# YichengDWu/tinyedm

Measured on AMD Instinct MI355X. Metric: train imgs/sec CIFAR-10 32x32 bf16, higher is better.
Workload: dtype bf16; 1 GPU; CIFAR-10 32x32 unconditional EDM2 U-Net (conf/cifar10.yaml, 35.6M params) full training step: diffuse+embed+denoiser fwd/bwd+loss+grad all-reduce+Adam+EMA; per_gpu_batch=128, global_batch=128, parallelism=dp1, conditional=False, step_launch=hipGraph replay, collective=none

## Files before the change

### include/tinyedm_hip.h

```cpp
#ifndef TINYEDM_HIP_H
#define TINYEDM_HIP_H
#ifdef __cplusplus
extern "C" {
#endif

typedef struct ihipStream_t* edm_stream_t;

int edm_version(void);
const char* edm_last_error(void);
int edm_init(int device);
int edm_graph_replay_safe(void);
typedef struct {
  unsigned step, seed_lo, seed_hi, reserved;
  float lr, ema_beta, grad_scale, bc1, bc2sqrt, pad[3];
} edm_step_params;

int edm_conv_igemm(const void* X, const void* Wp, void* Y, const void* R, float alpha, float beta, int B, int H,
                   int W, int Cin, int Cout, int taps, edm_stream_t stream);
int edm_conv_igemm_v2(const void* X, const void* Wp, void* Y, const void* R, float alpha, float beta, int B, int H,
                      int W, int Cin, int Cout, int taps, edm_stream_t stream);
int edm_conv_igemm_v6(const void* X, const void* Wp, void* Y, const void* R, float alpha, float beta, int B, int H,
                      int W, int Cin, int Cout, int taps, edm_stream_t stream);
int edm_conv_igemm_s(const void* X, const void* Wp, void* Y, const void* R, float alpha, float beta, int B, int H,
                     int W, int Cin, int Cout, int taps, edm_stream_t stream);
int edm_conv_plan(int B, int H, int W, int Cin, int Cout, int taps, int force);
int edm_conv_igemm_o(const void* X, const void* Wp, void* Y, long ldY, void* Ysilu, void* Yb, long ldYb, int split,
                     const void* R, float alpha, float beta, int B, int H, int W, int Cin, int Cout, int taps, int kernel,
                     int wfrag, edm_stream_t stream);
int edm_conv3x3_fold_supported(int B, int H, int W, int Cin, int Cout, int C2);
int edm_conv3x3_fold(const void* X, const void* Wp, const void* X2, long ldX2, const void* W2p, int C2, void* Y, long ldY,
                     void* Ysilu, float alpha3, float alpha1, int B, int H, int W, int Cin, int Cout, edm_stream_t stream);
int edm_conv3x3_mod(const void* X, const void* Wp, void* Y, void* Y2, const float* lin, long lin_stride,
                    const float* gain, float pdrop, unsigned long long seed, unsigned sub, unsigned step, int mark_dropped,
                    int B, int H, int W, int Cin, int Cout, const void* dyn, int wfrag, edm_stream_t stream);
int edm_conv3x3_modbwd(const void* dY, const void* Wd, float alpha, const void* U, const float* lin, long lin_stride,
                       const float* gain, void* GR, float* gm, long gm_stride, float pdrop, unsigned long long seed,
                       unsigned sub, unsigned step, int u_marked, int B, int H, int W, int Cin, int Cout, const void* dyn,
                       int wfrag, edm_stream_t stream);
int edm_conv3x3_silubwd(const void* dY, const void* Wd, const void* Xpre, const void* ADD, float add_scale, void* GX,
                        int B, int H, int W, int Cin, int Cout, int wfrag, edm_stream_t stream);
int edm_mod_finish(const float* gm, const float* lin, long lin_stride, const float* gain, float* glin, long glin_stride,
                   float* ggain, int B, int C, edm_stream_t stream);
int edm_mod_finish_multi(const float* gm_all, const float* lin_all, float* glin_all, long stride, const void* items_dev,
                         int n_items, int B, edm_stream_t stream);
int edm_conv_wgrad_nsplit(int B, int H, int W, int Cin, int Cout, int taps);
int edm_conv_wgrad_v2(const void* X, const void* dY, float* slabs, int B, int H, int W, int Cin, int Cout, int taps,
                      int nsplit, edm_stream_t stream);
int edm_conv_wgrad_1x1_nsplit(long npix, int Cin, int Cout);
int edm_conv_wgrad_1x1(const void* X, const void* dY, float* slabs, long npix, int Cin, int Cout, int nsplit,
                       edm_stream_t stream);
typedef struct {
  const void* X;
  const void* dY;
  float* slabs;
  long npix;
  int Cin, Cout, nsplit, pad;
} edm_wgrad1_item;
int edm_conv_wgrad_1x1_nsplit_grouped(long npix, int Cin, int Cout);
long edm_conv_wgrad_1x1_group_table_bytes(void);
int edm_conv_wgrad_1x1_group(const edm_wgrad1_item* items, int n, void* table_host, void* table_dev, int defer_upload,
                             edm_stream_t stream);
typedef struct {
  const void* X;
  const void* dY;
  const float* w;
  float* grad;
  const int* perm;
  int B, H, W, Cin, Cout, I;
  float scale;
  int accumulate;
} edm_wgrad3_item;
long edm_wgrad3_workspace(const edm_wgrad3_item* items, int n);
long edm_wgrad3_table_bytes(void);
int edm_wgrad3_max_layers(void);
int edm_wgrad3_group(const edm_wgrad3_item* items, int n, void* workspace, long workspace_bytes, void* table_host,
                     void* table_dev, int defer_upload, edm_stream_t stream);

int edm_weight_prep(float* w, int O, int I, int taps, int Ipad, void* wp_fwd, void* wp_dgrad, float* w_hat,
                    const int* perm, int normalize_inplace, edm_stream_t stream);
int edm_weight_prep_multi(const void* descs, const int* groups, int n_groups, int lds_bytes, int normalize_inplace,
                          edm_stream_t stream);
int edm_wgrad_finish(const float* slabs, int S, const float* w, float* grad, const int* perm, int O, int I, int Ipad,
                     int taps, float scale, int accumulate, edm_stream_t stream);

typedef struct {
  const float* slabs;
  const float* w;
  float* grad;
  const int* perm;
  int S, O, I, Ipad, taps;
  float scale;
  int accumulate;
} edm_finish_item;
long edm_wgrad_finish_multi_table_bytes(void);
int edm_wgrad_finish_multi(const edm_finish_item* items, int n, void* table_host, void* table_dev, int defer_upload,
                           edm_stream_t stream);

int edm_attention_fwd(const void* qkv, void* y, int B, int N, int C, int heads, edm_stream_t stream);
int edm_attention_bwd(const void* qkv, const void* y, const void* gy, void* gqkv, int B, int N, int C, int heads,
                      edm_stream_t stream);

int edm_attention_qkv_supported(int N, int C, int heads);
int edm_attention_qkv_fwd(const void* x, const void* Wqkv, void* y, void* stat, int B, int N, int C, int heads,
                          int heads_per_wg, edm_stream_t stream);
int edm_attention_qkv_bwd(const void* x, const void* y, const void* gout, const void* stat, const void* Wqkv,
                          const void* Wd_out, void* gqkv, float alpha, int B, int N, int C, int heads, int heads_per_wg,
                          edm_stream_t stream);

int edm_pixelnorm_silu_fwd(const void* x, void* xn, void* a, float* dsave, long P, int C, edm_stream_t stream);
int edm_pixelnorm_silu_bwd(const void* xn, const float* dsave, const void* gxn, float gxn_scale, const void* ga,
                           const void* gadd, void* gx, long P, int C, edm_stream_t stream);
int edm_pool_pixelnorm_silu_fwd(const void* x, void* xn, void* a, float* dsave, int B, int Hp, int Wp, int C,
                                edm_stream_t stream);
int edm_pool_pixelnorm_silu_bwd(const void* xn, const float* dsave, const void* gxn, float gxn_scale, const void* ga,
                                const void* gadd, void* gx, int B, int Hp, int Wp, int C, edm_stream_t stream);
int edm_silu_fwd(const void* x, void* a, long n, edm_stream_t stream);
int edm_silu_bwd(const void* x, const void* ga, const void* gextra, float extra_scale, void* gx, long n,
                 edm_stream_t stream);
int edm_axpby(const void* a, float alpha, const void* b, float beta, void* out, long n, edm_stream_t stream);
int edm_mod_silu_drop_fwd(const void* r, const float* lin, long lin_stride, const float* gain, void* a, int B, int HW,
                          int C, float pdrop, unsigned long long seed, unsigned sub, unsigned step, const void* dyn,
                          edm_stream_t stream);
int edm_mod_silu_drop_bwd(const void* r, const float* lin, long lin_stride, const float* gain, const void* ga, void* gr,
                          float* gm, float* glin, long glin_stride, float* ggain, int B, int HW, int C, float pdrop,
                          unsigned long long seed, unsigned sub, unsigned step, const void* dyn, edm_stream_t stream);
int edm_mod_silu_drop_bwd_raw(const void* r, const float* lin, long lin_stride, const float* gain, const void* ga, void* gr,
                              float* gm, long gm_stride, int B, int HW, int C, float pdrop, unsigned long long seed,
                              unsigned sub, unsigned step, const void* dyn, edm_stream_t stream);
int edm_dropout_mask(unsigned char* mask, long n, float pdrop, unsigned long long seed, unsigned sub, unsigned step,
                     edm_stream_t stream);
int edm_pool2(const void* x, void* y, int B, int Hout, int Wout, int C, float scale, edm_stream_t stream);
int edm_up2(const void* x, const void* add, void* y, int B, int Hout, int Wout, int C, float scale, edm_stream_t stream);
int edm_up2_silu(const void* x, void* y, void* a, int B, int Hout, int Wout, int C, edm_stream_t stream);
int edm_reduce_hw(const void* x, long x_stride, const void* y, long y_stride, float* out, int B, int HW, int C,
                  float scale, edm_stream_t stream);
int edm_scalelong_fwd(const float* mean, const float* W1h, const float* W2h, float* gate, float* z1save, int B, int C,
                      int R, edm_stream_t stream);
int edm_scalelong_bwd(const float* mean, const float* W1h, const float* W2h, const float* gate, const float* z1save,
                      const float* ggate, float* gmean, float* gW1h, float* gW2h, int B, int C, int R,
                      edm_stream_t stream);
int edm_skip_gate_fwd(const void* skip, const float* W1h, const float* W2h, float* mean, float* gate, float* z1save,
                      int B, int HW, int C, int R, edm_stream_t stream);
int edm_skip_gate_bwd(const void* gcat, long gcat_stride, int c_off, const void* skip, const float* mean,
                      const float* W1h, const float* W2h, const float* gate, const float* z1save, float* gmean,
                      float* gW1h, float* gW2h, float* ws, int B, int HW, int C, int R, edm_stream_t stream);
typedef struct {
  const float* ws;
  const float* mean;
  float* gW1h;
  float* gW2h;
  int B, C, R, pad;
} edm_skip_gate_wgrad_item;
long edm_skip_gate_wgrad_multi_table_bytes(void);
int edm_skip_gate_wgrad_multi(const edm_skip_gate_wgrad_item* items, int n, void* table_host, void* table_dev,
                              int defer_upload, edm_stream_t stream);
typedef struct {
  const void* skip;
  const float* W1h;
  const float* W2h;
  float* mean;
  float* gate;
  float* z1save;
  void* cat;
  void* silu_out;
  int B, HW, C, R, Ci, pad;
} edm_skip_gate_fwd_item;
long edm_skip_gate_fwd_multi_table_bytes(void);
int edm_skip_gate_fwd_multi(const edm_skip_gate_fwd_item* items, int n, void* table_host, void* table_dev, int defer_upload,
                            edm_stream_t stream);
typedef struct {
  const void* gcat;
  long gcat_stride;
  const void* skip;
  const float* W1h;
  const float* W2h;
  const float* gate;
  const float* z1save;
  float* gmean;
  float* ws;
  void* gskip;
  int c_off, B, HW, C, R, pad;
} edm_skip_gate_bwd_item;
typedef struct {
  const void* gcs;
  const float* gate;
  const float* gmean;
  void* gskip;
  int B, HW, Cs, pad;
} edm_skip_half_bwd_item;
long edm_skip_gate_bwd_multi_table_bytes(void);
int edm_skip_gate_bwd_multi(const edm_skip_gate_bwd_item* items, int n, void* table_host, void* table_dev, int defer_upload,
                            edm_stream_t stream);
int edm_skip_half_bwd_multi(const edm_skip_half_bwd_item* items, int n, void* table_host, void* table_dev, int defer_upload,
                            edm_stream_t stream);
int edm_concat_gate_fwd(const void* inp, const void* skip, const float* gate, void* cat, void* silu_out, int B, int HW,
                        int Ci, int Cs, edm_stream_t stream);
int edm_concat_gate_bwd(const void* gcat, const float* gate, const float* gmean, void* ginp, void* gskip, int B,
                        int HW, int Ci, int Cs, edm_stream_t stream);
int edm_skip_half_fwd(const void* skip, const float* gate, void* cat, void* silu_out, int B, int HW, int Ci, int Cs,
                      edm_stream_t stream);
int edm_skip_half_bwd(const void* gcs, const float* gate, const float* gmean, void* gskip, int B, int HW, int Cs,
                      edm_stream_t stream);

int edm_precond_in(const float* noisy, const float* sigma, int sigma_stride, float sigma_data, void* out, int B,
                   int Cimg, int HW, int CP, edm_stream_t stream);
int edm_conv_out_fwd(const void* x, const float* w_hat, const float* gain_out, const float* noisy, const float* sigma,
                     int sigma_stride, float sigma_data, float* D, float* Fraw, int B, int HW, int C, int Co,
                     edm_stream_t stream);
int edm_conv_out_bwd(const void* x, const float* w_hat, const float* gain_out, const float* Fraw, const float* dD,
                     const float* sigma, int sigma_stride, float sigma_data, void* gx, float* gw_hat, float* ggain,
                     int B, int HW, int C, int Co, edm_stream_t stream);

int edm_lowrank_df(const float* dD, const float* Fraw, const float* gain_out, const float* sigma, int sigma_stride,
                   float sigma_data, float* dF, float* aux, int B, int Co, int HW, edm_stream_t stream);
int edm_lowrank_dgrad3x3(const float* dF, const float* Wc, float scale, void* ga2, const void* r1, const float* lin,
                         long lin_stride, const float* gain, void* gr, float* gm, long gm_stride, float pdrop,
                         unsigned long long seed, unsigned sub, unsigned step, int u_marked, int B, int H, int W, int C,
                         int Co, const void* dyn, edm_stream_t stream);
long edm_lowrank_wgrad_workspace(int C, int Co, int taps);
int edm_lowrank_supported(int C, int Co, int W, int taps);
int edm_lowrank_wgrad(const float* dF, const void* X, int taps, const float* aux, float* G, float* aux_out, float* ws,
                      long ws_floats, int B, int H, int W, int C, int Co, edm_stream_t stream);
int edm_lowrank_expand_wc(const float* wout_hat, const void* wd, float* Wc, int Co, int O, int I, int taps,
                          edm_stream_t stream);
int edm_lowrank_expand_slab(const float* wout_hat, const float* G, float* slab, float scale, int Co, int O, int I,
                            int Ipad, int taps, edm_stream_t stream);

int edm_nchw_to_nhwc_bf16(const float* x, void* y, int B, int C, int HW, edm_stream_t stream);
int edm_nhwc_bf16_to_nchw(const void* x, float* y, int B, int C, int HW, edm_stream_t stream);

int edm_linear_fwd(const float* X, const float* W, float* Y, int M, int N, int K, edm_stream_t stream);
int edm_linear_plan(int M, int N, int K, int accumulate, int* tile_rows, int* splits);
int edm_linear_dgrad(const float* dY, const float* W, float* dX, int M, int N, int K, int accumulate,
                     edm_stream_t stream);
int edm_linear_wgrad(const float* dY, const float* X, float* dW, int M, int N, int K, int accumulate,
                     edm_stream_t stream);
int edm_fourier_fwd(const float* sigma, int sigma_stride, const float* freqs, const float* phases, float* out, int B,
                    int Fd, edm_stream_t stream);
int edm_embed_combine_fwd(const float* emb_sigma, const float* wcls_hat, const long long* labels, float add_factor,
                          int K, float* pre, float* out, int B, int E, unsigned long long drop_thr,
                          unsigned long long seed, unsigned step, const void* dyn, const int* drop_in, int* drop_out,
                          edm_stream_t stream);
int edm_embed_combine_bwd(const float* gout, const float* pre, const long long* labels, float add_factor, int K,
                          float* gemb_sigma, float* gwcls_hat, int B, int E, const int* drop, edm_stream_t stream);
int edm_aug_embed_fwd(float* emb_sigma, const float* aug, const float* w_hat, int B, int E, int K, edm_stream_t stream);
int edm_aug_embed_wgrad(const float* gemb_sigma, const float* aug, float* gw_hat, int B, int E, int K,
                        edm_stream_t stream);

int edm_diffuse(const float* clean, float* noisy, float* sigma, float P_mean, float P_std, int B, long CHW,
                unsigned long long seed, unsigned step, const void* dyn, edm_stream_t stream);
int edm_diffuse_given(const float* clean, const float* eps, const float* noise, float* noisy, float* sigma,
                      float P_mean, float P_std, int B, long CHW, edm_stream_t stream);
int edm_weighted_mse(const float* D, const float* clean, const float* sigma, const float* weight_override,
                     float sigma_data, float* loss, float* dD, int B, long CHW, float* acc_sum, long long* acc_total,
                     edm_stream_t stream);
int edm_adam_ema(float* theta, float* grad, float* m, float* v, float* ema, long n, float lr, float b1, float b2,
                 float eps, int step, float ema_beta, float grad_scale, const void* dyn, int zero_grad,
                 unsigned* health, edm_stream_t stream);
int edm_adam_ema_phema(float* theta, float* grad, float* m, float* v, float* ema, float* const* profiles, int K,
                       const float* betas, long n, float lr, float b1, float b2, float eps, int step, float ema_beta,
                       float grad_scale, const void* dyn, int zero_grad, unsigned* health, edm_stream_t stream);
int edm_phema_accumulate(double* acc, const float* snap, const double* w, int L, long n, edm_stream_t stream);
int edm_phema_finish(const double* acc, float* out, long n, edm_stream_t stream);
int edm_heun_euler(const float* x, const float* D, float t0, float t1, float* dx, float* x1, long n, unsigned* health,
                   edm_stream_t stream);
int edm_heun_correct(const float* x, const float* dx, const float* x1, const float* D1, float t0, float t1, float* out,
                     long n, unsigned* health, edm_stream_t stream);
int edm_heun_euler_guided(const float* x, const float* Dm, const float* Dg, const float* w, float t0, float t1,
                          float* dx, float* x1, long n, unsigned* health, edm_stream_t stream);
int edm_heun_correct_guided(const float* x, const float* dx, const float* x1, const float* Dm1, const float* Dg1,
                            const float* w, float t0, float t1, float* out, long n, unsigned* health,
                            edm_stream_t stream);
int edm_heun_churn(const float* x, float c, const void* rec, int step, int B, long CHW, float* x_hat,
                   unsigned* health, edm_stream_t stream);
int edm_dpm_multistep(const float* x, const float* Dm, const float* Dg, const float* w, const float* m1,
                      const float* m2, float a, float c0, float c1, float c2, float* x_out, float* m_out, long n,
                      unsigned* health, edm_stream_t stream);
int edm_state_init(const float* image, const float* x0, float t, float* out, long n, unsigned* health,
                   edm_stream_t stream);
int edm_inpaint_blend(const float* x, const float* image, const unsigned char* mask, float t, const void* rec, int step,
                      int B, int C, long HW, int mask_B, float* out, unsigned* health, edm_stream_t stream);
int edm_degrade(const float* x, float* y, int B, int C, int H, int W, int scale, int gray, edm_stream_t stream);
int edm_project_denoised(const float* Dm, const float* Dg, const float* w, const float* y, float* out, int B, int C,
                         int H, int W, int scale, int gray, unsigned* health, edm_stream_t stream);
#define EDM_NLL_MAX_CHUNKS 64
int edm_nll_probe(const float* x, float h, const void* rec, int step, int ev, int K, int B, long CHW, float* E,
                  unsigned* health, edm_stream_t stream);
int edm_heun_euler_div(const float* E, const float* D, float t0, float t1, float h0, float h1, const void* rec, int step,
                       int K, int B, long CHW, float* dx, float* E1, double* part, double* L, unsigned* health,
                       edm_stream_t stream);
int edm_heun_correct_div(const float* E, const float* dx, const float* E1, const float* D1, float t0, float t1, float h1,
                         float hn, const void* rec, int step, int K, int probes_out, int B, long CHW, float* out,
                         double* part, double* L, unsigned* health, edm_stream_t stream);
int edm_nll_prior(const float* x, float t, int B, long CHW, double* part, double* L, unsigned* health,
                  edm_stream_t stream);
int edm_eval_diffuse(const float* clean, const unsigned* ids, const int* level, const float* sigmas, int L,
                     const void* rec, int B, long CHW, float* noisy, float* sigma_out, unsigned* health,
                     edm_stream_t stream);
int edm_eval_sqerr(const float* D, const float* clean, int B, long CHW, double* part, double* se, unsigned* health,
                   edm_stream_t stream);
int edm_scale_f32(const float* x, float s, float* y, long n, edm_stream_t stream);

int edm_f32_conv(const float* X, const float* w_hat, float* Y, const float* R, float alpha, float beta, const float* lin,
                 long lin_stride, const float* gain, int B, int H, int W, int Cin, int I, int Cout, int taps,
                 edm_stream_t stream);
int edm_f32_to_pairs(const float* x, void* pairs, long rows, int C, edm_stream_t stream);
int edm_split_pack(const float* w_hat, void* pack, int O, int I, int taps, int Ip, edm_stream_t stream);
int edm_split_conv(const void* Xp, const void* Wp3, float* Y, void* Ypairs, const float* R, float alpha, float beta,
                   const float* lin, long lin_stride, const float* gain, int B, int H, int W, int C, int Cout, int taps,
                   edm_stream_t stream);
int edm_split_conv_o(const void* Xp, const void* Wp3, float* Y, void* Ypairs, long ld_pairs, long lo_off, void* Ysilu_pairs,
                     const float* R, float alpha, float beta, const float* lin, long lin_stride, const float* gain, int B,
                     int H, int W, int C, int Cout, int taps, edm_stream_t stream);
int edm_split_conv_fold(const void* Xp, const void* Wp3, const void* X2p, const void* W2p3, int C2, float* Y, void* Ypairs,
                        long ld_pairs, long lo_off, void* Ysilu_pairs, float alpha3, float alpha1, int B, int H, int W, int C,
                        int Cout, edm_stream_t stream);
int edm_f32_skip_half(const float* skip, const float* gate, void* cat_pairs, void* silu_pairs, int B, int HW, int Ci, int Cs,
                      edm_stream_t stream);
int edm_f32_attention(const float* qkv, float* y, int B, int N, int C, int heads, edm_stream_t stream);
int edm_split_attention(const float* qkv, float* y, void* ypairs, int B, int N, int C, int heads, edm_stream_t stream);
int edm_f32_pixelnorm_silu(const float* x, float* xn, float* s, long P, int C, int s_pairs, edm_stream_t stream);
int edm_f32_silu(const float* x, float* s, long n, int pairs_row, edm_stream_t stream);
int edm_f32_pool2(const float* x, float* y, int B, int Hout, int Wout, int C, edm_stream_t stream);
int edm_f32_up2(const float* x, float* y, int B, int Hout, int Wout, int C, edm_stream_t stream);
int edm_f32_pool_pixelnorm_silu(const float* x, float* xn, float* s, int B, int Hout, int Wout, int C, int s_pairs,
                                edm_stream_t stream);
int edm_f32_up2_silu(const float* x, float* y, float* s, int B, int Hout, int Wout, int C, int s_pairs, edm_stream_t stream);
int edm_f32_skip_gate(const float* skip, const float* W1h, const float* W2h, float* gate, int B, int HW, int C, int R,
                      edm_stream_t stream);
int edm_f32_concat_gate(const float* inp, const float* skip, const float* gate, float* cat, float* silu_out, int B,
                        int HW, int Ci, int Cs, int pairs, edm_stream_t stream);
int edm_f32_precond_in(const float* noisy, const float* sigma, int sigma_stride, float sigma_data, float* out, int B,
                       int Cimg, int HW, int CP, edm_stream_t stream);
int edm_f32_conv_out(const float* x, const float* w_hat, const float* gain_out, const float* noisy, const float* sigma,
                     int sigma_stride, float sigma_data, float* D, int B, int HW, int C, int Co, edm_stream_t stream);
int edm_f32_nchw_to_nhwc(const float* x, float* y, int B, int C, int HW, edm_stream_t stream);
int edm_f32_nhwc_to_nchw(const float* x, float* y, int B, int C, int HW, edm_stream_t stream);

int edm_u8_gather_normalize(const void* data, const long* index, float* out, int B, int C, int H, int W, long n_images,
                            float mean, float stdv, int flip, unsigned long long seed, unsigned epoch,
                            edm_stream_t stream);
int edm_u8_gather_augment_normalize(const void* data, const long* index, float* out, int B, int C, int H, int W,
                                    long n_images, float mean, float stdv, int flip, unsigned long long seed,
                                    unsigned epoch, unsigned long long aug_thr, int aug_ops, float* aug,
                                    edm_stream_t stream);
int edm_u8_gather_augment_warp_normalize(const void* data, const long* index, float* out, int B, int C, int H, int W,
                                         long n_images, float mean, float stdv, int flip, unsigned long long seed,
                                         unsigned epoch, unsigned long long aug_thr, int aug_ops, int warp_ops,
                                         float* aug, float* theta, edm_stream_t stream);
int edm_denormalize_u8(const float* x, void* out, long n, float scale, float offset, edm_stream_t stream);
int edm_prediction_to_u8_nhwc(const float* pred, void* out, int B, int C, int H, int W, const float* mean,
                              const float* stdv, edm_stream_t stream);

int edm_u8_knn_splits(long Q, long R);
int edm_u8_norms(const void* x, long n_rows, int D, int* norms, edm_stream_t stream);
int edm_u8_knn_partial(const void* queries, const void* refs, long Q, long R, int D, int k, int exclude_self, long ref_base,
                       int partial, int splits, const int* qnorms, const int* rnorms, unsigned long long* keys,
                       edm_stream_t stream);
int edm_knn_merge(const unsigned long long* keys, int n_lists, long Q, int k, unsigned* dist, int* idx,
                  edm_stream_t stream);

#ifdef __cplusplus
}
#endif
#endif
```

### tinyedm_amd/_lib.py

```python
import ctypes
import os

_HERE = os.path.dirname(os.path.abspath(__file__))
LIB_PATH = os.environ.get("EDM_LIB_PATH") or os.path.join(_HERE, "libtinyedm_hip.so")

P, I, L, F = ctypes.c_void_p, ctypes.c_int, ctypes.c_long, ctypes.c_float
U, U64 = ctypes.c_uint, ctypes.c_ulonglong

SIGNATURES = {
    "edm_version": [],
    "edm_last_error": [],
    "edm_init": [I],
    "edm_graph_replay_safe": [],
    "edm_pixelnorm_silu_fwd": [P, P, P, P, L, I, P],
    "edm_pixelnorm_silu_bwd": [P, P, P, F, P, P, P, L, I, P],
    "edm_pool_pixelnorm_silu_fwd": [P, P, P, P, I, I, I, I, P],
    "edm_pool_pixelnorm_silu_bwd": [P, P, P, F, P, P, P, I, I, I, I, P],
    "edm_up2_silu": [P, P, P, I, I, I, I, P],
    "edm_silu_fwd": [P, P, L, P],
    "edm_silu_bwd": [P, P, P, F, P, L, P],
    "edm_axpby": [P, F, P, F, P, L, P],
    "edm_mod_silu_drop_fwd": [P, P, L, P, P, I, I, I, F, U64, U, U, P, P],
    "edm_mod_silu_drop_bwd": [P, P, L, P, P, P, P, P, L, P, I, I, I, F, U64, U, U, P, P],
    "edm_mod_silu_drop_bwd_raw": [P, P, L, P, P, P, P, L, I, I, I, F, U64, U, U, P, P],
    "edm_dropout_mask": [P, L, F, U64, U, U, P],
    "edm_pool2": [P, P, I, I, I, I, F, P],
    "edm_up2": [P, P, P, I, I, I, I, F, P],
    "edm_reduce_hw": [P, L, P, L, P, I, I, I, F, P],
    "edm_scalelong_fwd": [P, P, P, P, P, I, I, I, P],
    "edm_scalelong_bwd": [P, P, P, P, P, P, P, P, P, I, I, I, P],
    "edm_skip_gate_fwd": [P, P, P, P, P, P, I, I, I, I, P],
    "edm_skip_gate_bwd": [P, L, I, P, P, P, P, P, P, P, P, P, P, I, I, I, I, P],
    "edm_skip_gate_wgrad_multi": [P, I, P, P, I, P],
    "edm_skip_gate_wgrad_multi_table_bytes": [],
    "edm_skip_gate_fwd_multi": [P, I, P, P, I, P],
    "edm_skip_gate_fwd_multi_table_bytes": [],
    "edm_skip_gate_bwd_multi": [P, I, P, P, I, P],
    "edm_skip_half_bwd_multi": [P, I, P, P, I, P],
    "edm_skip_gate_bwd_multi_table_bytes": [],
    "edm_concat_gate_fwd": [P, P, P, P, P, I, I, I, I, P],
    "edm_concat_gate_bwd": [P, P, P, P, P, I, I, I, I, P],
    "edm_skip_half_fwd": [P, P, P, P, I, I, I, I, P],
    "edm_skip_half_bwd": [P, P, P, P, I, I, I, P],
    "edm_precond_in": [P, P, I, F, P, I, I, I, I, P],
    "edm_conv_out_fwd": [P, P, P, P, P, I, F, P, P, I, I, I, I, P],
    "edm_conv_out_bwd": [P, P, P, P, P, P, I, F, P, P, P, I, I, I, I, P],
    "edm_nchw_to_nhwc_bf16": [P, P, I, I, I, P],
    "edm_nhwc_bf16_to_nchw": [P, P, I, I, I, P],
    "edm_lowrank_df": [P, P, P, P, I, F, P, P, I, I, I, P],
    "edm_lowrank_dgrad3x3": [P, P, F, P, P, P, L, P, P, P, L, F, U64, U, U, I, I, I, I, I, I, P, P],
    "edm_lowrank_wgrad_workspace": [I, I, I],
    "edm_lowrank_supported": [I, I, I, I],
    "edm_lowrank_wgrad": [P, P, I, P, P, P, P, L, I, I, I, I, I, P],
    "edm_lowrank_expand_wc": [P, P, P, I, I, I, I, P],
    "edm_lowrank_expand_slab": [P, P, P, F, I, I, I, I, I, P],
    "edm_conv_igemm": [P, P, P, P, F, F, I, I, I, I, I, I, P],
    "edm_conv_igemm_v2": [P, P, P, P, F, F, I, I, I, I, I, I, P],
    "edm_conv_plan": [I, I, I, I, I, I, I],
    "edm_conv_igemm_o": [P, P, P, L, P, P, L, I, P, F, F, I, I, I, I, I, I, I, I, P],
    "edm_conv3x3_fold_supported": [I, I, I, I, I, I],
    "edm_conv3x3_fold": [P, P, P, L, P, I, P, L, P, F, F, I, I, I, I, I, P],
    "edm_conv_igemm_v6": [P, P, P, P, F, F, I, I, I, I, I, I, P],
    "edm_conv_igemm_s": [P, P, P, P, F, F, I, I, I, I, I, I, P],
    "edm_conv3x3_mod": [P, P, P, P, P, L, P, F, U64, U, U, I, I, I, I, I, I, P, I, P],
    "edm_conv3x3_modbwd": [P, P, F, P, P, L, P, P, P, L, F, U64, U, U, I, I, I, I, I, I, P, I, P],
    "edm_mod_finish_multi": [P, P, P, L, P, I, I, P],
    "edm_conv3x3_silubwd": [P, P, P, P, F, P, I, I, I, I, I, I, P],
    "edm_mod_finish": [P, P, L, P, P, L, P, I, I, P],
    "edm_conv_wgrad_nsplit": [I, I, I, I, I, I],
    "edm_conv_wgrad_v2": [P, P, P, I, I, I, I, I, I, I, P],
    "edm_conv_wgrad_1x1_nsplit": [L, I, I],
    "edm_conv_wgrad_1x1_nsplit_grouped": [L, I, I],
    "edm_conv_wgrad_1x1": [P, P, P, L, I, I, I, P],
    "edm_conv_wgrad_1x1_group": [P, I, P, P, I, P],
    "edm_conv_wgrad_1x1_group_table_bytes": [],
    "edm_wgrad3_workspace": [P, I],
    "edm_wgrad3_group": [P, I, P, L, P, P, I, P],
    "edm_wgrad3_table_bytes": [],
    "edm_wgrad3_max_layers": [],
    "edm_attention_fwd": [P, P, I, I, I, I, P],
    "edm_attention_bwd": [P, P, P, P, I, I, I, I, P],
    "edm_attention_qkv_supported": [I, I, I],
    "edm_attention_qkv_fwd": [P, P, P, P, I, I, I, I, I, P],
    "edm_attention_qkv_bwd": [P, P, P, P, P, P, P, F, I, I, I, I, I, P],
    "edm_linear_plan": [I, I, I, I, P, P],
    "edm_linear_fwd": [P, P, P, I, I, I, P],
    "edm_linear_dgrad": [P, P, P, I, I, I, I, P],
    "edm_linear_wgrad": [P, P, P, I, I, I, I, P],
    "edm_fourier_fwd": [P, I, P, P, P, I, I, P],
    "edm_embed_combine_fwd": [P, P, P, F, I, P, P, I, I, U64, U64, U, P, P, P, P],
    "edm_embed_combine_bwd": [P, P, P, F, I, P, P, I, I, P, P],
    "edm_aug_embed_fwd": [P, P, P, I, I, I, P],
    "edm_aug_embed_wgrad": [P, P, P, I, I, I, P],
    "edm_diffuse": [P, P, P, F, F, I, L, U64, U, P, P],
    "edm_diffuse_given": [P, P, P, P, P, F, F, I, L, P],
    "edm_weighted_mse": [P, P, P, P, F, P, P, I, L, P, P, P],
    "edm_adam_ema": [P, P, P, P, P, L, F, F, F, F, I, F, F, P, I, P, P],
    "edm_adam_ema_phema": [P, P, P, P, P, P, I, P, L, F, F, F, F, I, F, F, P, I, P, P],
    "edm_phema_accumulate": [P, P, P, I, L, P],
    "edm_phema_finish": [P, P, L, P],
    "edm_heun_euler": [P, P, F, F, P, P, L, P, P],
    "edm_heun_correct": [P, P, P, P, F, F, P, L, P, P],
    "edm_heun_euler_guided": [P, P, P, P, F, F, P, P, L, P, P],
    "edm_heun_correct_guided": [P, P, P, P, P, P, F, F, P, L, P, P],
    "edm_heun_churn": [P, F, P, I, I, L, P, P, P],
    "edm_dpm_multistep": [P, P, P, P, P, P, F, F, F, F, P, P, L, P, P],
    "edm_state_init": [P, P, F, P, L, P, P],
    "edm_inpaint_blend": [P, P, P, F, P, I, I, I, L, I, P, P, P],
    "edm_nll_probe": [P, F, P, I, I, I, I, L, P, P, P],
    "edm_heun_euler_div": [P, P, F, F, F, F, P, I, I, I, L, P, P, P, P, P, P],
    "edm_heun_correct_div": [P, P, P, P, F, F, F, F, P, I, I, I, I, L, P, P, P, P, P],
    "edm_nll_prior": [P, F, I, L, P, P, P, P],
    "edm_eval_diffuse": [P, P, P, P, I, P, I, L, P, P, P, P],
    "edm_eval_sqerr": [P, P, I, L, P, P, P, P],
    "edm_scale_f32": [P, F, P, L, P],
    "edm_degrade": [P, P, I, I, I, I, I, I, P],
    "edm_project_denoised": [P, P, P, P, P, I, I, I, I, I, I, P, P],
    "edm_weight_prep": [P, I, I, I, I, P, P, P, P, I, P],
    "edm_weight_prep_multi": [P, P, I, I, I, P],
    "edm_wgrad_finish": [P, I, P, P, P, I, I, I, I, F, I, P],
    "edm_wgrad_finish_multi": [P, I, P, P, I, P],
    "edm_wgrad_finish_multi_table_bytes": [],
    "edm_f32_conv": [P, P, P, P, F, F, P, L, P, I, I, I, I, I, I, I, P],
    "edm_f32_attention": [P, P, I, I, I, I, P],
    "edm_split_attention": [P, P, P, I, I, I, I, P],
    "edm_f32_to_pairs": [P, P, L, I, P],
    "edm_split_pack": [P, P, I, I, I, I, P],
    "edm_split_conv": [P, P, P, P, P, F, F, P, L, P, I, I, I, I, I, I, P],
    "edm_split_conv_o": [P, P, P, P, L, L, P, P, F, F, P, L, P, I, I, I, I, I, I, P],
    "edm_split_conv_fold": [P, P, P, P, I, P, P, L, L, P, F, F, I, I, I, I, I, P],
    "edm_f32_skip_half": [P, P, P, P, I, I, I, I, P],
    "edm_f32_pool_pixelnorm_silu": [P, P, P, I, I, I, I, I, P],
    "edm_f32_up2_silu": [P, P, P, I, I, I, I, I, P],
    "edm_f32_pixelnorm_silu": [P, P, P, L, I, I, P],
    "edm_f32_silu": [P, P, L, I, P],
    "edm_f32_pool2": [P, P, I, I, I, I, P],
    "edm_f32_up2": [P, P, I, I, I, I, P],
    "edm_f32_skip_gate": [P, P, P, P, I, I, I, I, P],
    "edm_f32_concat_gate": [P, P, P, P, P, I, I, I, I, I, P],
    "edm_f32_precond_in": [P, P, I, F, P, I, I, I, I, P],
    "edm_f32_conv_out": [P, P, P, P, P, I, F, P, I, I, I, I, P],
    "edm_f32_nchw_to_nhwc": [P, P, I, I, I, P],
    "edm_f32_nhwc_to_nchw": [P, P, I, I, I, P],
    "edm_u8_gather_normalize": [P, P, P, I, I, I, I, L, F, F, I, U64, U, P],
    "edm_u8_gather_augment_normalize": [P, P, P, I, I, I, I, L, F, F, I, U64, U, U64, I, P, P],
    "edm_u8_gather_augment_warp_normalize": [P, P, P, I, I, I, I, L, F, F, I, U64, U, U64, I, I, P, P, P],
    "edm_denormalize_u8": [P, P, L, F, F, P],
    "edm_prediction_to_u8_nhwc": [P, P, I, I, I, I, P, P, P],
    "edm_u8_knn_splits": [L, L],
    "edm_u8_norms": [P, L, I, P, P],
    "edm_u8_knn_partial": [P, P, L, L, I, I, I, L, I, I, P, P, P, P],
    "edm_knn_merge": [P, I, L, I, P, P, P],
}
DIAG_SIGNATURES = {
    "edm_conv_igemm_v2_stamp": [P, P, P, I, I, I, I, I, P, P],
    "edm_conv_igemm_v2_ablate": [P, P, P, I, I, I, I, I, I, P],
    "edm_wgrad3_probe": [P, P],
    "edm_wgrad3_plan_ksplit": [P, I, P],
    "edm_v6_persistent_launches": [],
}
_RET = {"edm_last_error": ctypes.c_char_p, "edm_lowrank_wgrad_workspace": ctypes.c_long, "edm_v6_persistent_launches": ctypes.c_long, "edm_wgrad3_workspace": ctypes.c_long, "edm_wgrad3_table_bytes": ctypes.c_long,
        "edm_skip_gate_wgrad_multi_table_bytes": ctypes.c_long, "edm_skip_gate_fwd_multi_table_bytes": ctypes.c_long, "edm_skip_gate_bwd_multi_table_bytes": ctypes.c_long,
        "edm_conv_wgrad_1x1_group_table_bytes": ctypes.c_long, "edm_wgrad_finish_multi_table_bytes": ctypes.c_long}
_NO_STATUS = {"edm_lowrank_wgrad_workspace", "edm_lowrank_supported", "edm_skip_gate_bwd_multi_table_bytes", "edm_skip_gate_fwd_multi_table_bytes", "edm_v6_persistent_launches", "edm_conv3x3_fold_supported", "edm_conv_plan", "edm_skip_gate_wgrad_multi_table_bytes", "edm_version", "edm_graph_replay_safe", "edm_last_error", "edm_conv_wgrad_nsplit", "edm_conv_wgrad_1x1_nsplit", "edm_conv_wgrad_1x1_nsplit_grouped", "edm_wgrad3_workspace", "edm_wgrad3_table_bytes", "edm_wgrad3_max_layers",
              "edm_conv_wgrad_1x1_group_table_bytes", "edm_wgrad_finish_multi_table_bytes", "edm_attention_qkv_supported",
              "edm_u8_knn_splits"}

_lib = None


class HipKernelError(RuntimeError):
    pass


class FinishItem(ctypes.Structure):
    _fields_ = [("slabs", P), ("w", P), ("grad", P), ("perm", P), ("S", I), ("O", I), ("I", I), ("Ipad", I), ("taps", I),
                ("scale", F), ("accumulate", I)]


class SkipGateWgradItem(ctypes.Structure):
    _fields_ = [("ws", P), ("mean", P), ("gW1h", P), ("gW2h", P), ("B", I), ("C", I), ("R", I), ("pad", I)]


class SkipGateFwdItem(ctypes.Structure):
    _fields_ = [("skip", P), ("W1h", P), ("W2h", P), ("mean", P), ("gate", P), ("z1save", P), ("cat", P), ("silu_out", P),
                ("B", I), ("HW", I), ("C", I), ("R", I), ("Ci", I), ("pad", I)]


class SkipGateBwdItem(ctypes.Structure):
    _fields_ = [("gcat", P), ("gcat_stride", L), ("skip", P), ("W1h", P), ("W2h", P), ("gate", P), ("z1save", P), ("gmean", P),
                ("ws", P), ("gskip", P), ("c_off", I), ("B", I), ("HW", I), ("C", I), ("R", I), ("pad", I)]


class SkipHalfBwdItem(ctypes.Structure):
    _fields_ = [("gcs", P), ("gate", P), ("gmean", P), ("gskip", P), ("B", I), ("HW", I), ("Cs", I), ("pad", I)]


class WGrad1Item(ctypes.Structure):
    _fields_ = [("X", P), ("dY", P), ("slabs", P), ("npix", L), ("Cin", I), ("Cout", I), ("nsplit", I), ("pad", I)]


class WGrad3Item(ctypes.Structure):
    _fields_ = [("X", P), ("dY", P), ("w", P), ("grad", P), ("perm", P), ("B", I), ("H", I), ("W", I), ("Cin", I),
                ("Cout", I), ("I", I), ("scale", F), ("accumulate", I)]


def lib() -> ctypes.CDLL:
    global _lib
    if _lib is None:
        if not os.path.exists(LIB_PATH):
            raise RuntimeError(
                f"tinyedm_amd: {LIB_PATH} is missing -- build it with `python -m tinyedm_amd.build` "
                "(there is no CPU fallback for the HIP hot path)")
        h = ctypes.CDLL(LIB_PATH)
        for name, args in {**SIGNATURES, **DIAG_SIGNATURES}.items():
            fn = getattr(h, name)
            fn.argtypes = args
            fn.restype = _RET.get(name, ctypes.c_int)
        _lib = h
    return _lib


N_CALLS = 0


def call(name: str, *args):
    global N_CALLS
    N_CALLS += 1
    h = lib()
    rc = getattr(h, name)(*args)
    if name in _NO_STATUS:
        return rc
    if rc != 0:
        msg = h.edm_last_error()
        raise HipKernelError(f"{name} failed (status {rc}): {msg.decode() if msg else '?'}")
    return rc


_inited_devices = set()


def init_device(index: int) -> None:
    if index not in _inited_devices:
        call("edm_init", int(index))
        _inited_devices.add(index)
```

### tinyedm_amd/csrc/tail_lowrank.hip

```cpp
#include "common.h"

typedef __attribute__((ext_vector_type(2))) float f32x2;

constexpr size_t LOWRANK_LDS_MAX = 60 * 1024;
static size_t dgrad_lds(int Co, int C, int W, int R, bool fused) {
  const int CL = C / 8, PS = ((256 / CL) * CL) / CL, TP = (W + 3) / 4 * 4 + 4;
  return ((size_t)Co * 9 * C + (size_t)Co * (R + 2) * TP + (fused ? (size_t)PS * C : 0)) * sizeof(float);
}
static size_t wgrad_lds(int Co, int taps, int C, int W, int R) {
  const int halo = taps == 9 ? 1 : 0;
  return ((size_t)Co * taps * C + (size_t)Co * (R + 2 * halo) * (W + 2 * halo)) * sizeof(float);
}
extern "C" int edm_lowrank_supported(int C, int Co, int W, int taps) {
  if (C <= 0 || C % 8 || C > 1024 || Co < 1 || Co > 8 || W <= 0 || (taps != 1 && taps != 9)) return 0;
  if (wgrad_lds(Co, taps, C, W, 1) > LOWRANK_LDS_MAX) return 0;
  return taps == 1 || dgrad_lds(Co, C, W, 1, true) <= LOWRANK_LDS_MAX;
}

__global__ void k_lowrank_df(const float* __restrict__ dD, const float* __restrict__ Fraw,
                             const float* __restrict__ gain_out, const float* __restrict__ sigma, int sstride, float sd,
                             float* __restrict__ dF, float* __restrict__ aux, int CoHW, long n) {
  const float go = *gain_out;
  for (long i = (long)blockIdx.x * blockDim.x + threadIdx.x; i < n; i += (long)gridDim.x * blockDim.x) {
    const int b = (int)(i / CoHW);
// ... 132 lines not shown
    }
  }
}

template <int CO>
static int launch_dgrad(const float* dF, const float* Wc, float scale, void* ga, const void* U, const float* lin,
                        long lin_stride, const float* gain, void* gr, float* gm, long gm_stride, float pdrop,
                        unsigned long long seed, unsigned sub, unsigned step, int u_marked, int B, int H, int W, int C,
                        const void* dyn, hipStream_t st) {
  const int CL = C / 8, block = (256 / CL) * CL, PS = block / CL;
  const int NSX = (W + 3) / 4, TP = NSX * 4 + 4;
  int R = 128 / W;
  R = R < 1 ? 1 : (R > H ? H : R);
  auto lds = [&](int r) { return dgrad_lds(CO, C, W, r, U != nullptr); };
  while (R > 1 && lds(R) > LOWRANK_LDS_MAX) --R;
  EDM_REQUIRE(lds(R) <= LOWRANK_LDS_MAX, "lowrank_dgrad3x3: Co=%d, C=%d, W=%d need %zu bytes of LDS (60 KB at most)", CO, C, W,
              lds(R));
  const dim3 grid((H + R - 1) / R, B);
  if (U)
    hipLaunchKernelGGL((k_lowrank_dgrad3x3<CO, true>), grid, dim3(block), lds(R), st, dF, Wc, scale, (bf16*)ga,
                       (const bf16*)U, lin, lin_stride, gain, (bf16*)gr, gm, gm_stride, pdrop, (uint32_t)seed,
                       (uint32_t)(seed >> 32), sub, step, u_marked, (const StepParams*)dyn, H, W, C, R, TP);
  else
    hipLaunchKernelGGL((k_lowrank_dgrad3x3<CO, false>), grid, dim3(block), lds(R), st, dF, Wc, scale, (bf16*)ga,
                       (const bf16*)nullptr, (const float*)nullptr, 0L, (const float*)nullptr, (bf16*)nullptr,
                       (float*)nullptr, 0L, 0.f, 0u, 0u, 0u, 0u, 0, (const StepParams*)nullptr, H, W, C, R, TP);
  EDM_CHECK_LAUNCH("lowrank_dgrad3x3");
  return EDM_OK;
}

#define EDM_CO_SWITCH(Co, CALL)      \
  switch (Co) {                      \
    case 1: return CALL(1);          \
    case 2: return CALL(2);          \
    case 3: return CALL(3);          \
    case 4: return CALL(4);          \
    case 5: return CALL(5);          \
    case 6: return CALL(6);          \
    case 7: return CALL(7);          \
    default: return CALL(8);         \
  }

extern "C" int edm_lowrank_dgrad3x3(const float* dF, const float* Wc, float scale, void* ga, const void* r1,
                                    const float* lin, long lin_stride, const float* gain, void* gr, float* gm,
                                    long gm_stride, float pdrop, unsigned long long seed, unsigned sub, unsigned step,
                                    int u_marked, int B, int H, int W, int C, int Co, const void* dyn, hipStream_t st) {
  EDM_REQUIRE(dF && Wc && (ga || r1), "lowrank_dgrad3x3: null pointer");
  EDM_REQUIRE(B > 0 && B <= 65535 && H > 0 && W > 0 && C > 0 && C % 8 == 0 && C <= 2048 && Co >= 1 && Co <= 8,
              "lowrank_dgrad3x3: bad args (C %% 8 == 0, Co <= 8 required)");
  EDM_REQUIRE(((uintptr_t)Wc & 15) == 0, "lowrank_dgrad3x3: Wc must be 16-byte aligned");
  if (r1)
    EDM_REQUIRE(lin && gain && gr && gm && lin_stride >= C && gm_stride >= C && pdrop >= 0.f && pdrop < 1.f,
                "lowrank_dgrad3x3: bad modulation-backward args");
#define CALL(CO_) launch_dgrad<CO_>(dF, Wc, scale, ga, r1, lin, lin_stride, gain, gr, gm, gm_stride, pdrop, seed, sub, step, \
                                    u_marked, B, H, W, C, dyn, st)
  EDM_CO_SWITCH(Co, CALL)
#undef CALL
}

template <int CO, int TAPS, int VEC>
__global__ __launch_bounds__(512) void k_lowrank_wgrad(const float* __restrict__ dF, const bf16* __restrict__ X,
                                                       const float* __restrict__ aux, float* __restrict__ ws, int H,
                                                       int W, int C, int R, int upb, int nunits) {
  constexpr int HALO = TAPS == 9 ? 1 : 0, K = TAPS == 9 ? 3 : 1, NB = 8;
  extern __shared__ __attribute__((aligned(16))) float sm[];
  __shared__ float asums[512];
  const int N = CO * TAPS * C, TPW = W + 2 * HALO, TR = R + 2 * HALO;
  float* accl = sm;
  float* tl = sm + N;
  typedef __attribute__((ext_vector_type(VEC / 2))) unsigned int uraw;
  const int CLV = C / VEC;
  const int PS = blockDim.x / CLV;
  const int cv = threadIdx.x % CLV, ps = threadIdx.x / CLV;
  f32x2 acc[CO * TAPS][VEC / 2];
#pragma unroll
  for (int e = 0; e < CO * TAPS; ++e)
#pragma unroll
    for (int h = 0; h < VEC / 2; ++h) acc[e][h] = f32x2{0.f, 0.f};
  float asum = 0.f;
  for (int u = blockIdx.x; u < nunits; u += gridDim.x) {
    const int b = u / upb, y0 = (u - b * upb) * R;
    const int rows = min(R, H - y0);
    __syncthreads();
    for (int i = threadIdx.x; i < CO * TR * TPW; i += blockDim.x) {
      const int o = i / (TR * TPW), rem = i - o * TR * TPW;
      const int ry = rem / TPW, cx = rem - ry * TPW;
      const int y = y0 + ry - HALO, x = cx - HALO;
      float v = 0.f;
      if (y >= 0 && y < H && x >= 0 && x < W)
        v = dF[(((long)b * CO + o) * H + y) * W + x];
      tl[i] = v;
    }
    if (aux) {
      for (int o = 0; o < CO; ++o) {
        const float* ap = aux + (((long)b * CO + o) * H + y0) * W;
        for (int i = threadIdx.x; i < rows * W; i += blockDim.x) asum += ap[i];
      }
    }
    __syncthreads();
    const int np = rows * W;
    const bf16* xp = X + (((long)b * H + y0) * W) * C + cv * VEC;
    int ry = ps / W, x = ps - (ps / W) * W;
    uraw nx[NB];
    auto fetch = [&](int q0) {
#pragma unroll
      for (int i = 0; i < NB; ++i) {
        const int q = q0 + i * PS;
        nx[i] = uraw{};
        if (q < np) nx[i] = *reinterpret_cast<const uraw*>(xp + (long)q * C);
      }
    };
    fetch(ps);
    for (int q0 = ps; q0 < np; q0 += NB * PS) {
      uraw cur[NB];
#pragma unroll
      for (int i = 0; i < NB; ++i) cur[i] = nx[i];
      if (q0 + NB * PS < np) fetch(q0 + NB * PS);
#pragma unroll
      for (int i = 0; i < NB; ++i) {
        if (q0 + i * PS < np) {
          typedef __attribute__((ext_vector_type(VEC))) __bf16 bfv;
          const bfv xv = __builtin_bit_cast(bfv, cur[i]);
          f32x2 xf[VEC / 2];
#pragma unroll
          for (int h = 0; h < VEC / 2; ++h) xf[h] = f32x2{(float)xv[2 * h], (float)xv[2 * h + 1]};
#pragma unroll
          for (int o = 0; o < CO; ++o)
#pragma unroll
            for (int ky = 0; ky < K; ++ky)
#pragma unroll
              for (int kx = 0; kx < K; ++kx) {
                const float d = tl[(o * TR + ry + 2 * HALO - ky) * TPW + x + 2 * HALO - kx];
                const f32x2 d2 = {d, d};
#pragma unroll
                for (int h = 0; h < VEC / 2; ++h) acc[o * TAPS + ky * K + kx][h] += d2 * xf[h];
              }
        }
        x += PS;
        while (x >= W) {
          x -= W;
          ++ry;
        }
      }
    }
  }
  for (int r = 0; r < PS; ++r) {
    __syncthreads();
    if (ps == r) {
#pragma unroll
      for (int e = 0; e < CO * TAPS; ++e) {
#pragma unroll
        for (int h = 0; h < VEC / 2; ++h) {
          f32x2* ap = reinterpret_cast<f32x2*>(accl + e * C + cv * VEC + 2 * h);
          f32x2 v = acc[e][h];
          if (r) v += *ap;
          *ap = v;
        }
      }
    }
  }
  asums[threadIdx.x] = asum;
  __syncthreads();
  float* row = ws + (long)blockIdx.x * (N + 4);
  for (int i = threadIdx.x; i < N; i += blockDim.x) row[i] = accl[i];
  if (threadIdx.x == 0) {
    float s = 0.f;
    for (int i = 0; i < (int)blockDim.x; ++i) s += asums[i];
    row[N] = s;
  }
}

__global__ __launch_bounds__(1024) void k_lowrank_reduce(const float* __restrict__ ws, int nwg, int N, float* __restrict__ G,
                                                         float* __restrict__ aux_out) {
  __shared__ float part[16][64];
  const int l = threadIdx.x & 63, seg = threadIdx.x >> 6;
  const int e = blockIdx.x * 64 + l;
  const int per = (nwg + 15) / 16;
  const int r0 = seg * per;
  float v[16];
#pragma unroll
  for (int k = 0; k < 16; ++k) {
    const int r = r0 + k;
    v[k] = (e <= N && k < per && r < nwg) ? ws[(long)r * (N + 4) + e] : 0.f;
  }
  float s = 0.f;
#pragma unroll
  for (int k = 0; k < 16; ++k) s += v[k];
  part[seg][l] = s;
  __syncthreads();
  if (seg == 0 && e <= N) {
    float t = 0.f;
#pragma unroll
    for (int k = 0; k < 16; ++k) t += part[k][l];
    if (e < N) G[e] = t;
    else if (aux_out) *aux_out += t;
  }
}

template <int CO>
static int launch_wgrad(const float* dF, const void* X, int taps, const float* aux, float* G, float* aux_out, float* ws,
                        long ws_floats, int B, int H, int W, int C, int nwg, hipStream_t st) {
  constexpr int VEC = CO <= 4 ? 4 : 2;
  const int CLV = C / VEC;
  int PS = 512 / CLV;
  PS = PS > 16 ? 16 : PS;
  const int block = PS * CLV, halo = taps == 9 ? 1 : 0;
  const int N = CO * taps * C;
  int R = 512 / W;
  R = R < 1 ? 1 : (R > H ? H : R);
  auto lds = [&](int r) { return wgrad_lds(CO, taps, C, W, r); };
  while (R > 1 && lds(R) > LOWRANK_LDS_MAX) --R;
  EDM_REQUIRE(lds(R) <= LOWRANK_LDS_MAX, "lowrank_wgrad: Co=%d, taps=%d, C=%d, W=%d need %zu bytes of LDS (60 KB at most)", CO,
              taps, C, W, lds(R));
  const int upb = (H + R - 1) / R;
  EDM_REQUIRE((long)B * upb < (1L << 31), "lowrank_wgrad: too many units");
  const int nunits = B * upb;
  const int grid = nunits < nwg ? nunits : nwg;
  EDM_REQUIRE(ws_floats >= (long)grid * (N + 4), "lowrank_wgrad: workspace of %ld floats, %ld needed", ws_floats,
              (long)grid * (N + 4));
  if (taps == 9)
    hipLaunchKernelGGL((k_lowrank_wgrad<CO, 9, VEC>), dim3(grid), dim3(block), lds(R), st, dF, (const bf16*)X, aux, ws, H, W, C,
                       R, upb, nunits);
  else
    hipLaunchKernelGGL((k_lowrank_wgrad<CO, 1, VEC>), dim3(grid), dim3(block), lds(R), st, dF, (const bf16*)X, aux, ws, H, W, C,
                       R, upb, nunits);
  EDM_CHECK_LAUNCH("lowrank_wgrad");
  hipLaunchKernelGGL(k_lowrank_reduce, dim3((N + 1 + 63) / 64), dim3(1024), 0, st, ws, grid, N, G, aux_out);
  EDM_CHECK_LAUNCH("lowrank_reduce");
  return EDM_OK;
}

constexpr int LOWRANK_WGRAD_NWG = 256;
extern "C" long edm_lowrank_wgrad_workspace(int C, int Co, int taps) {
  return (long)LOWRANK_WGRAD_NWG * ((long)Co * taps * C + 4);
}

extern "C" int edm_lowrank_wgrad(const float* dF, const void* X, int taps, const float* aux, float* G, float* aux_out,
                                 float* ws, long ws_floats, int B, int H, int W, int C, int Co, hipStream_t st) {
  EDM_REQUIRE(dF && X && G && ws && (!aux || aux_out), "lowrank_wgrad: null pointer");
  EDM_REQUIRE(B > 0 && H > 0 && W > 0 && C > 0 && C % 8 == 0 && C <= 1024 && Co >= 1 && Co <= 8 && (taps == 1 || taps == 9),
              "lowrank_wgrad: bad args (C %% 8 == 0, Co <= 8, taps 1 or 9 required)");
#define CALL(CO_) launch_wgrad<CO_>(dF, X, taps, aux, G, aux_out, ws, ws_floats, B, H, W, C, LOWRANK_WGRAD_NWG, st)
  EDM_CO_SWITCH(Co, CALL)
#undef CALL
}

__global__ void k_lowrank_expand_wc(const float* __restrict__ wout, const bf16* __restrict__ wd, float* __restrict__ Wc,
                                    int Co, int O, int I, int taps) {
  const int lane = threadIdx.x & 63;
  const int row = blockIdx.x * (blockDim.x >> 6) + (threadIdx.x >> 6);
  if (row >= taps * I) return;
  const int tt = row / I, ci = row - tt * I;
  float acc[8] = {0, 0, 0, 0, 0, 0, 0, 0};
  for (int c = lane * 8; c < O; c += 64 * 8) {
    float v[8];
    load8(wd + (long)row * O + c, v);
#pragma unroll
    for (int o = 0; o < 8; ++o)
      if (o < Co) {
#pragma unroll
        for (int j = 0; j < 8; ++j) acc[o] += wout[(long)o * O + c + j] * v[j];
      }
  }
#pragma unroll
  for (int o = 0; o < 8; ++o)
    if (o < Co) {
      const float s = wave_sum(acc[o]);
      if (lane == 0) Wc[((long)o * taps + (taps - 1 - tt)) * I + ci] = s;
    }
}
extern "C" int edm_lowrank_expand_wc(const float* wout_hat, const void* wd, float* Wc, int Co, int O, int I, int taps,
                                     hipStream_t st) {
  EDM_REQUIRE(wout_hat && wd && Wc, "lowrank_expand_wc: null pointer");
  EDM_REQUIRE(Co >= 1 && Co <= 8 && O > 0 && O % 8 == 0 && I > 0 && taps >= 1, "lowrank_expand_wc: bad args");
  hipLaunchKernelGGL(k_lowrank_expand_wc, dim3((taps * I + 3) / 4), dim3(256), 0, st, wout_hat, (const bf16*)wd, Wc, Co, O,
                     I, taps);
  EDM_CHECK_LAUNCH("lowrank_expand_wc");
  return EDM_OK;
}

__global__ void k_lowrank_expand_slab(const float* __restrict__ wout, const float* __restrict__ G, float* __restrict__ slab,
                                      float scale, int Co, int O, int I, int Ipad, int taps, long n) {
  for (long e = (long)blockIdx.x * blockDim.x + threadIdx.x; e < n; e += (long)gridDim.x * blockDim.x) {
    const int i = (int)(e % Ipad);
    const long tc = e / Ipad;
    const int c = (int)(tc % O), t = (int)(tc / O);
    float s = 0.f;
    if (i < I)
      for (int o = 0; o < Co; ++o) s += wout[(long)o * O + c] * G[((long)o * taps + t) * I + i];
    slab[e] = scale * s;
  }
}
extern "C" int edm_lowrank_expand_slab(const float* wout_hat, const float* G, float* slab, float scale, int Co, int O, int I,
                                       int Ipad, int taps, hipStream_t st) {
  EDM_REQUIRE(wout_hat && G && slab, "lowrank_expand_slab: null pointer");
  EDM_REQUIRE(Co >= 1 && Co <= 8 && O > 0 && I > 0 && Ipad >= I && taps >= 1, "lowrank_expand_slab: bad args");
  const long n = (long)taps * O * Ipad;
  const long blocks = (n + 255) / 256;
  hipLaunchKernelGGL(k_lowrank_expand_slab, dim3((unsigned)(blocks < 4096 ? blocks : 4096)), dim3(256), 0, st, wout_hat, G,
                     slab, scale, Co, O, I, Ipad, taps, n);
  EDM_CHECK_LAUNCH("lowrank_expand_slab");
  return EDM_OK;
}
```

### tinyedm_amd/networks.py

```python
from __future__ import annotations

import math
import os
from typing import Optional

import numpy as np
import torch
import torch.nn as nn
from torch import Tensor

from . import ops

bf16, f32 = torch.bfloat16, torch.float32


class _Rng:
    seed: int = 42
    step: int = 0
    dyn = None


rng = _Rng()


def manual_seed(seed: int) -> None:
    rng.seed = int(seed) & 0xFFFFFFFFFFFFFFFF
    rng.step = 0


_WEIGHT_EPOCH = 0


_IN_DENOISER = [False]
FORWARD_EPOCH = 0


def bump_weight_epoch() -> None:
    global _WEIGHT_EPOCH
    _WEIGHT_EPOCH += 1


def _mp_coeffs(t: float):
    c = math.sqrt((1 - t) ** 2 + t ** 2)
    return (1 - t) / c, t / c


class _WNBase(nn.Module):

    weight: nn.Parameter

    def _init_cache(self):
        self._cache = None
        self._cache_key = None
        self._perm: Optional[Tensor] = None
        self._ipad: Optional[int] = None
        self._want = ("fwd", "dgrad")
        self._split_pack = None
        self._split_key = None
        self._plain = None

    def _taps(self) -> int:
        return self.weight[0, 0].numel() if self.weight.dim() == 4 else 1

    def packs(self):
        w = self.weight
        if not w.is_cuda:
            raise RuntimeError("tinyedm_amd: parameters must live on the GPU (there is no CPU path)")
        if self.training and getattr(self, "_fresh", False):
            self._fresh = False
            return self._cache
        key = (w.data_ptr(), w._version, _WEIGHT_EPOCH)
        if not self.training and not _IN_DENOISER[0] and self._cache is not None and self._cache_key == key and any(
                getattr(t, "_edm_frag", False) for t in self._cache[:2] if t is not None):
            if self._plain is None or self._plain[0] != key:
                with torch.no_grad():
                    self._plain = (key, ops.weight_prep(w.data, self._taps(), Ipad=self._ipad, want_fwd="fwd" in self._want,
                                                        want_dgrad="dgrad" in self._want, want_hat="hat" in self._want,
                                                        perm=self._perm, normalize_inplace=False))
            return self._plain[1]
        if self.training or self._cache is None or self._cache_key != key:
            perm = self._perm
            if perm is not None and perm.device != w.device:
                perm = self._perm = perm.to(w.device)
            with torch.no_grad():
                self._cache = ops.weight_prep(
                    w.data, self._taps(), Ipad=self._ipad, want_fwd="fwd" in self._want,
                    want_dgrad="dgrad" in self._want, want_hat="hat" in self._want, perm=perm,
                    normalize_inplace=self.training)
            self._cache_key = (w.data_ptr(), w._version, _WEIGHT_EPOCH)
        return self._cache

    def finish_grad(self, slabs: Tensor, scale: float = 1.0) -> Tensor:
        w = self.weight
        I = w.shape[1]
        if w.grad is not None and getattr(w, "_edm_direct", False):
            key = w.device.index
            pend = _fin_pending.setdefault(key, [])
            pend.append((slabs, w, self._perm, self._taps(), I, scale))
            w._edm_deferred = True
            if len(pend) >= FIN_GROUP:
                _flush_fin(key)
            _queue_backward_end(w.device)
            return None
        g = ops.wgrad_finish(slabs, w.data, self._taps(), I, perm=self._perm, scale=scale)
        return g.view_as(w)


WGRAD_STREAM = os.environ.get("EDM_WGRAD_STREAM", "1") != "0"
W3_GROUP = max(0, min(ops.W3_MAX_LAYERS, int(os.environ.get("EDM_W3_GROUP", "16"))))
W3_TAIL = max(0, int(os.environ.get("EDM_W3_TAIL", "0")))
_w3_seen = {}
_w3_total = {}
W3_MAXPIX = int(os.environ.get("EDM_W3_MAXPIX", str(1 << 18)))
FIN_GROUP = 40
W1_GROUP = max(0, min(16, int(os.environ.get("EDM_W1_GROUP", "16"))))
_w1_pending = {}
_bwd_end_queued = set()
MOD_DEFER_UNFUSED = os.environ.get("EDM_MOD_DEFER_UNFUSED", "1") != "0"
SG_MULTI = os.environ.get("EDM_SG_MULTI", "1") != "0"
SG_HALVES = os.environ.get("EDM_SG_HALVES", "1") != "0"
SG_BWD_MULTI = os.environ.get("EDM_SG_BWD_MULTI", "1") != "0"
SG_DEFER = os.environ.get("EDM_SG_DEFER", "1") != "0"
_sg_pending = {}
_w3_pending = {}
TAIL_LOWRANK = os.environ.get("EDM_TAIL_LOWRANK", "1") != "0"
_tail_slot = {}
_fin_pending = {}


def _run_on_side(device, fn, tensors=()):
    if WGRAD_STREAM:
        side = ops.side_stream(device)
        side.wait_stream(torch.cuda.current_stream())
        with torch.cuda.stream(side):
            fn()
        for t in tensors:
            t.record_stream(side)
    else:
        fn()


def _flush_w3(key):
    items = _w3_pending.pop(key, None)
    if not items:
        return
    dev = items[0][0].weight.device
    args = [(x, dy, m.weight.data, m.weight.grad, m._perm, scale, True) for m, x, dy, scale in items]
    keep = [t for _, x, dy, _ in items for t in (x, dy)]
    _run_on_side(dev, lambda: ops.wgrad3_group(args), keep)
    _flush_fin(key)
    for m, _, _, _ in items:
        m.weight._edm_deferred = False
        for hook in getattr(m.weight, "_edm_hooks", ()):
            hook(m.weight)


def _flush_w1(key):
    items = _w1_pending.pop(key, None)
    if not items:
        return
    dev = items[0][0].weight.device
    box = []
    _run_on_side(dev, lambda: box.extend(ops.conv_wgrad_1x1_group([(x, dy) for _, x, dy, _ in items])),
                 [t for _, x, dy, _ in items for t in (x, dy)])
    pend = _fin_pending.setdefault(key, [])
    for (m, _, _, scale), slabs in zip(items, box):
        w = m.weight
        pend.append((slabs, w, m._perm, 1, w.shape[1], scale))


def _flush_fin(key):
    _flush_w1(key)
    items = _fin_pending.pop(key, None)
    if not items:
        return
    dev = items[0][1].device
    args = [(slabs, w.data, w.grad, perm, taps, I, scale, True) for slabs, w, perm, taps, I, scale in items]
    _run_on_side(dev, lambda: ops.wgrad_finish_multi(args), [a[0] for a in args])
    for _, w, *_rest in items:
        w._edm_deferred = False
        for hook in getattr(w, "_edm_hooks", ()):
            hook(w)


def _flush_sg(key):
    items = _sg_pending.pop(key, None)
    if not items:
        return
    outs = ops.skip_gate_wgrad_multi([(ws, mean, R) for _, ws, mean, R in items])
    for (sl, _, _, _), (gw1h, gw2h) in zip(items, outs):
        sl.layer1.finish_grad(gw1h.view(1, 1, *gw1h.shape))
        sl.layer2.finish_grad(gw2h.view(1, 1, *gw2h.shape))


def _backward_end(key):
    _bwd_end_queued.discard(key)
    _tail_slot.pop(key, None)
    if key in _w3_seen:
        _w3_total[key] = _w3_seen.pop(key)
    _flush_sg(key)
    _flush_w3(key)
    _flush_fin(key)
    if WGRAD_STREAM:
        torch.cuda.current_stream(key).wait_stream(ops.side_stream(key))


def _queue_backward_end(device):
    key = torch.device(device).index
    if key in _bwd_end_queued:
        return
    try:
        torch.autograd.Variable._execution_engine.queue_callback(lambda: _backward_end(key))
        _bwd_end_queued.add(key)
    except RuntimeError:
        _backward_end(key)


def reset_backward_state():
    _tail_slot.clear()
    if _bwd_end_queued or _w3_pending or _fin_pending or _w1_pending or _sg_pending:
        _bwd_end_queued.clear()
        for items in _sg_pending.values():
            for sl, *_rest in items:
                sl.layer1.weight._edm_deferred = sl.layer2.weight._edm_deferred = False
        _sg_pending.clear()
        for items in _w1_pending.values():
            for m, _, _, _ in items:
                m.weight._edm_deferred = False
        _w1_pending.clear()
        for items in _fin_pending.values():
            for _, w, *_rest in items:
                w._edm_deferred = False
        _fin_pending.clear()
        for items in _w3_pending.values():
            for m, _, _, _ in items:
                m.weight._edm_deferred = False
        _w3_pending.clear()
        _w3_seen.clear()
        if WGRAD_STREAM:
            for s in ops.side_streams():
                torch.cuda.current_stream(s.device).wait_stream(s)


def _wgrad(mod, x, dy, taps, scale=1.0):
    w = mod.weight
    direct = w.grad is not None and getattr(w, "_edm_direct", False)
    if (taps == 9 and W3_GROUP and w.dim() == 4 and ops.wgrad3_supported(x, dy, w.shape[1])
            and (not WGRAD_STREAM or x.shape[0] * x.shape[1] * x.shape[2] <= W3_MAXPIX)):
        if direct:
            key = w.device.index
            pend = _w3_pending.setdefault(key, [])
            if pend and (pend[0][1].shape[2] + 2 > 64) != (x.shape[2] + 2 > 64):
                _flush_w3(key)
                pend = _w3_pending.setdefault(key, [])
            pend.append((mod, x, dy, scale))
            w._edm_deferred = True
            seen = _w3_seen[key] = _w3_seen.get(key, 0) + 1
            if len(pend) >= W3_GROUP or (W3_TAIL and seen == _w3_total.get(key, 0) - W3_TAIL):
                _flush_w3(key)
            _queue_backward_end(w.device)
            return None
        g = torch.empty_like(w.data)
        ops.wgrad3_group([(x, dy, w.data, g, mod._perm, scale, False)])
        return g
    if direct and taps == 1 and W1_GROUP and w.dim() == 4 and ops.wgrad1x1_group_supported(x, dy):
        key = w.device.index
        pend = _w1_pending.setdefault(key, [])
        pend.append((mod, x, dy, scale))
        w._edm_deferred = True
        if len(pend) >= W1_GROUP:
            _flush_fin(key)
        _queue_backward_end(w.device)
        return None
    if direct:
        _run_on_side(w.device, lambda: mod.finish_grad(ops.conv_wgrad(x, dy, taps), scale=scale), (x, dy))
        _queue_backward_end(w.device)
        return None
    return mod.finish_grad(ops.conv_wgrad(x, dy, taps), scale=scale)


def _wgrad_lowrank(mod, x, dF, wout_hat, scale):
    w = mod.weight
    box = []
    _run_on_side(w.device, lambda: box.append(ops.lowrank_expand_slab(wout_hat, ops.lowrank_wgrad(dF, x, 9)[0], scale)),
                 (x, dF, wout_hat))
    return mod.finish_grad(box[0])


PREP_TILE_BYTES = int(os.environ.get("EDM_PREP_TILE_KB", "96")) * 1024


class _PrepPlan:

    def __init__(self, mods, frag=None, wants=None, cat=None):
        self.mods = mods
        frag = frag or {}
        wants = [tuple(m._want) for m in mods] if wants is None else list(wants)
        self.wants = wants
        self.pins = 0
        self._pinned_forever = False
        self.splits = []
        dev = mods[0].weight.device
        self.ptr_key = tuple(m.weight.data_ptr() for m in mods)
        desc = np.zeros(len(mods), dtype=np.dtype([
            ("w", "<u8"), ("fwd", "<u8"), ("dgrad", "<u8"), ("hat", "<u8"), ("perm", "<u8"),
            ("O", "<i4"), ("I", "<i4"), ("taps", "<i4"), ("Ipad", "<i4"), ("row0", "<i4"), ("pad", "<i4")]))
        assert desc.dtype.itemsize == 64
        groups, row0, lds = [], 0, 0
        self.caches = []
        self.wcat, cat_rows = None, {}
        if cat:
            kin = cat[0].weight.shape[1]
            if all(c.weight.dim() == 2 and c.weight.shape[1] == kin for c in cat):
                self.wcat = torch.empty(sum(c.weight.shape[0] for c in cat), kin, device=dev, dtype=f32)
                r = 0
                for c in cat:
                    cat_rows[c] = r
                    r += c.weight.shape[0]
        for k, m in enumerate(mods):
            w = m.weight
            O, I, taps = w.shape[0], w.shape[1], m._taps()
            ipad = I if m._ipad is None else m._ipad
            want = wants[k]
            wf = torch.empty(taps, O, ipad, device=dev, dtype=bf16) if "fwd" in want else None
            wd = torch.empty(taps, I, O, device=dev, dtype=bf16) if "dgrad" in want else None
            if m in cat_rows:
                wh = self.wcat[cat_rows[m]:cat_rows[m] + O]
            else:
                wh = torch.empty(O, I * taps, device=dev, dtype=f32) if ("hat" in want or "split" in want) else None
            self.splits.append(torch.empty(taps, O, 3 * ((I + 31) // 32 * 32), device=dev, dtype=bf16)
                               if "split" in want else None)
            if m._perm is not None and m._perm.device != dev:
                m._perm = m._perm.to(dev)
            rb = 32
            while rb > 1 and (rb * I * taps * 2 > PREP_TILE_BYTES or rb > O):
                rb //= 2
            lds = max(lds, rb * I * taps * 2)
            ff, fd = frag.get(m, (False, False))
            if not (taps == 9 and I % 32 == 0 and O % 32 == 0 and ipad == I and rb % 8 == 0 and m._perm is None):
                ff = fd = False
            if ff and wf is not None:
                wf._edm_frag = True
            if fd and wd is not None:
                wd._edm_frag = True
            desc[k] = (w.data_ptr(), wf.data_ptr() if wf is not None else 0, wd.data_ptr() if wd is not None else 0,
                       wh.data_ptr() if wh is not None else 0, m._perm.data_ptr() if m._perm is not None else 0,
                       O, I, taps | (0x100 if ff and wf is not None else 0) | (0x200 if fd and wd is not None else 0), ipad,
                       row0, rb)
            groups += [(k, r) for r in range(0, O, rb)]
            row0 += O
            self.caches.append((wf, wd, wh))
        self.total_rows = row0
        self.desc = torch.from_numpy(desc.view(np.uint8).copy()).to(dev)
        self.groups = torch.tensor(groups, dtype=torch.int32).to(dev)
        self.lds_bytes = lds
        self.eval_key = None

    @property
    def pinned(self) -> bool:
        return self.pins > 0 or self._pinned_forever

    def valid_for(self, mods):
        return tuple(m.weight.data_ptr() for m in mods) == self.ptr_key

    def run(self, training: bool):
        key = (tuple(m.weight._version for m in self.mods), _WEIGHT_EPOCH)
        if training or key != self.eval_key:
            ops.weight_prep_multi(self.desc, self.groups, self.lds_bytes, training)
            for m, c, sp in zip(self.mods, self.caches, self.splits):
                if sp is not None:
                    ops.split_pack(c[2], m._taps(), out=sp)
            self.eval_key = None if training else key
        if torch.cuda.is_current_stream_capturing() and not ops.note_capture_pin(self):
            self._pinned_forever = True
        for m, c, sp in zip(self.mods, self.caches, self.splits):
            m._cache = c
            m._cache_key = (m.weight.data_ptr(), m.weight._version, _WEIGHT_EPOCH)
            m._fresh = training
            m._split_pack = sp
            m._split_key = m._cache_key if sp is not None else None


class Conv2d(_WNBase):

    def __init__(self, in_channels, out_channels, kernel_size):
        super().__init__()
        self.in_channels = in_channels
        self.out_channels = out_channels
        self.kernel_size = kernel_size
        self.weight = nn.Parameter(torch.randn(out_channels, in_channels, kernel_size, kernel_size))
        self._init_cache()

    def forward(self, x: Tensor) -> Tensor:
        xh = ops.nchw_to_nhwc_bf16(x.float().contiguous())
        y = _ConvFn.apply(xh, self.weight, self)
        return ops.nhwc_bf16_to_nchw(y).to(x.dtype)

    def extra_repr(self) -> str:
        return f"{self.in_channels}, {self.out_channels}, kernel_size={self.kernel_size}"


class Linear(_WNBase):

    def __init__(self, in_features: int, out_features: int):
        super().__init__()
        self.in_features = in_features
        self.out_features = out_features
        self.weight = nn.Parameter(torch.randn(out_features, in_features))
        self._init_cache()
        self._want = ("hat",)

    def forward(self, x: Tensor) -> Tensor:
        return _LinearFn.apply(x.float().contiguous(), self.weight, self)

    def extra_repr(self) -> str:
        return f"{self.in_features}, {self.out_features}"


class _ConvFn(torch.autograd.Function):
    @staticmethod
    def forward(ctx, x, weight, mod: Conv2d):
        wf, wd, _ = mod.packs()
        ctx.mod, ctx.wd = mod, wd
        ctx.save_for_backward(x)
        return ops.conv_igemm(x, wf, mod._taps())

    @staticmethod
    def backward(ctx, gy):
        (x,) = ctx.saved_tensors
        gy = gy.contiguous()
        taps = ctx.mod._taps()
        gx = ops.conv_igemm(gy, ctx.wd, taps) if ctx.needs_input_grad[0] else None
        gw = _wgrad(ctx.mod, x, gy, taps) if ctx.needs_input_grad[1] else None
        return gx, gw, None


class _LinearFn(torch.autograd.Function):
    @staticmethod
    def forward(ctx, x, weight, mod: Linear):
        _, _, wh = mod.packs()
        ctx.mod, ctx.wh = mod, wh
        ctx.save_for_backward(x)
        return ops.linear_fwd(x, wh)

    @staticmethod
    def backward(ctx, gy):
        (x,) = ctx.saved_tensors
        gy = gy.contiguous()
        gx = ops.linear_dgrad(gy, ctx.wh) if ctx.needs_input_grad[0] else None
        gw = None
        if ctx.needs_input_grad[1]:
            dwh = ops.linear_wgrad(gy, x)
            gw = ctx.mod.finish_grad(dwh.view(1, 1, *dwh.shape))
        return gx, gw, None


def pixel_norm(x: Tensor, eps: float = 1e-4, dim=1) -> Tensor:
    if dim != 1 or x.dim() != 4 or eps != 1e-4:
        raise NotImplementedError("tinyedm_amd.pixel_norm implements the (B,C,H,W), dim=1, eps=1e-4 hot-path case")
    xn, _, _ = ops.pixelnorm_silu_fwd(ops.nchw_to_nhwc_bf16(x.float().contiguous()))
    return ops.nhwc_bf16_to_nchw(xn).to(x.dtype)


def mp_silu(x: Tensor) -> Tensor:
    return torch.nn.functional.silu(x) / 0.596


def mp_add(a: Tensor, b: Tensor, t: float = 0.5) -> Tensor:
    return a.lerp(b, t) / np.sqrt((1 - t) ** 2 + t ** 2)


class UpSample(nn.Module):

    def forward(self, x):
        return ops.nhwc_bf16_to_nchw(ops.up2(ops.nchw_to_nhwc_bf16(x.float().contiguous()))).to(x.dtype)


class DownSample(nn.Module):

    def forward(self, x):
        return ops.nhwc_bf16_to_nchw(ops.pool2(ops.nchw_to_nhwc_bf16(x.float().contiguous()))).to(x.dtype)


class _ResampleFn(torch.autograd.Function):

    @staticmethod
    def forward(ctx, x, up: bool, alias: bool = False, want_silu: bool = False):
        ctx.up = up
        ctx.set_materialize_grads(False)
        if up and want_silu:
            y, s = ops.up2_silu(x)
            ctx.mark_non_differentiable(s)
            return y, s
        y = ops.up2(x) if up else ops.pool2(x, 0.25)
        return (y, x) if alias else y

    @staticmethod
    def backward(ctx, g, g_alias=None):
        if g is None:
            return g_alias, None, None, None
        g = g.contiguous()
        if ctx.up:
            gx = ops.pool2(g, 1.0)
            if g_alias is not None:
                gx = ops.axpby(gx, 1.0, g_alias.contiguous(), 1.0)
            return gx, None, None, None
        return ops.up2(g, 0.25, add=None if g_alias is None else g_alias.contiguous()), None, None, None


class UncertaintyNet(nn.Module):

    def __init__(self, in_features: int, hidden_features: int):
        super().__init__()
        self.linear1 = Linear(in_features + 1, hidden_features)
        self.linear2 = Linear(hidden_features, 1)
        self.gain = nn.Parameter(torch.zeros(()))

    def forward(self, x: Tensor):
        x = torch.cat((x, torch.ones_like(x[:, 0:1])), dim=1)
        x = mp_silu(self.linear1(x))
        return self.gain * self.linear2(x)


class ScaleLong(nn.Module):
    def __init__(self, dim, r=16):
        super().__init__()
        self.layer1 = Conv2d(dim + 1, int(dim // r), 1)
        self.layer2 = Conv2d(int(dim // r), dim, 1)
        self.layer1._want = ("hat",)
        self.layer2._want = ("hat",)
        if SG_DEFER:
            self.layer1.weight._edm_late = True
            self.layer2.weight._edm_late = True

    def forward(self, inp: Tensor) -> Tensor:
        xh = ops.nchw_to_nhwc_bf16(inp.float().contiguous())
        B, H, W, C = xh.shape
        w1h, w2h = self.layer1.packs()[2], self.layer2.packs()[2]
        _, gate, _ = ops.skip_gate_fwd(xh, w1h, w2h)
        return gate.view(B, C, 1, 1)


SKIP_GATE_FUSED = os.environ.get("EDM_SKIP_GATE_FUSED", "1") != "0"
U_MARKS = os.environ.get("EDM_U_MARKS", "1") != "0"


FUSE_CAT = os.environ.get("EDM_FUSE_CAT", "1") != "0"
FUSE_RESAMPLE = os.environ.get("EDM_FUSE_RESAMPLE", "1") != "0"
FRAG_PACKS = os.environ.get("EDM_FRAG_PACKS", "1") != "0"


def _col_block(buf: Tensor, C: int) -> Tensor:
    B, H, W, Ct = buf.shape
    return torch.empty(0, device=buf.device, dtype=buf.dtype).set_(buf.untyped_storage(), buf.storage_offset(),
                                                                   (B, H, W, C), (H * W * Ct, W * Ct, Ct, 1))


def _dest_ok(dest, x: Tensor) -> bool:
    return dest is not None and dest[0].shape[:3] == x.shape[:3]


class _ConcatGateFn(torch.autograd.Function):
    @staticmethod
    def forward(ctx, inp, skip, w1, w2, sl: ScaleLong, want_silu: bool = False):
        ctx.set_materialize_grads(False)
        B, H, W, Cs = skip.shape
        w1h, w2h = sl.layer1.packs()[2], sl.layer2.packs()[2]
        if SKIP_GATE_FUSED:
            mean, gate, z1 = ops.skip_gate_fwd(skip, w1h, w2h)
        else:
            mean = ops.reduce_hw(skip, scale=1.0 / (H * W))
            gate, z1 = ops.scalelong_fwd(mean, w1h, w2h)
        cat, sil = ops.concat_gate_fwd(inp, skip, gate, want_silu)
        ctx.sl, ctx.Ci = sl, inp.shape[-1]
        ctx.save_for_backward(skip, mean, gate, z1, w1h, w2h)
        if want_silu:
            ctx.mark_non_differentiable(sil)
            return cat, sil
        return cat

    @staticmethod
    def backward(ctx, gcat, _gsil=None):
        skip, mean, gate, z1, w1h, w2h = ctx.saved_tensors
        gcat = gcat.contiguous()
        Ci, Cs = ctx.Ci, skip.shape[-1]
        if SKIP_GATE_FUSED:
            gmean, gw1h, gw2h = ops.skip_gate_bwd(gcat, Ci, skip, mean, w1h, w2h, gate, z1)
        else:
            ggate = ops.reduce_hw(gcat, C=Cs, c_off=Ci, y=skip)
            gmean, gw1h, gw2h = ops.scalelong_bwd(mean, w1h, w2h, gate, z1, ggate)
        ginp, gskip = ops.concat_gate_bwd(gcat, gate, gmean, Ci)
        gw1 = ctx.sl.layer1.finish_grad(gw1h.view(1, 1, *gw1h.shape))
        gw2 = ctx.sl.layer2.finish_grad(gw2h.view(1, 1, *gw2h.shape))
        return ginp, gskip, gw1, gw2, None, None


class ClassEmbedding(nn.Module):
    def __init__(self, num_embeddings, embedding_dim):
        super().__init__()
        self.num_embeddings = num_embeddings
        self.linear = Linear(num_embeddings, embedding_dim)

    def forward(self, class_labels: Tensor):
        onehot = torch.nn.functional.one_hot(class_labels.flatten(), self.num_embeddings).float()
        return self.linear(onehot * np.sqrt(self.num_embeddings, dtype=np.float32))


class FourierEmbedding(nn.Module):
    def __init__(self, embedding_dim: int):
        super().__init__()
        self.register_buffer("freqs", 2 * np.pi * torch.randn(embedding_dim))
        self.register_buffer("phases", 2 * np.pi * torch.rand(embedding_dim))

    def forward(self, x):
        s = (x.float() * 4).exp().flatten().contiguous()
        return ops.fourier_fwd(s, self.freqs, self.phases, s.numel())


class _EmbeddingFn(torch.autograd.Function):
    @staticmethod
    def forward(ctx, sigma, labels, w_sigma, w_cls, mod: "Embedding", aug=None, w_aug=None):
        ctx.set_materialize_grads(False)
        B = max(sigma.numel(), labels.numel() if labels is not None else 1, aug.shape[0] if aug is not None else 1)
        four = ops.fourier_fwd(sigma, mod.fourier_embed.freqs, mod.fourier_embed.phases, B)
        wsh = mod.sigma_embed.packs()[2]
        wch = mod.class_embed.linear.packs()[2] if labels is not None else None
        es = ops.linear_fwd(four, wsh)
        if aug is not None:
            ops.aug_embed_fwd(es, aug, mod.aug_embed.packs()[2])
        drop = None
        if labels is not None and mod.training and mod.label_dropout > 0:
            pre, out, drop = ops.embed_combine_fwd(es, wch, labels, mod.add_factor, drop_p=mod.label_dropout,
                                                   seed=rng.seed, step=rng.step, dyn=rng.dyn)
        else:
            pre, out = ops.embed_combine_fwd(es, wch, labels, mod.add_factor)
        ctx.mod, ctx.labels, ctx.drop, ctx.aug = mod, labels, drop, aug
        mod.last_label_drop = drop
        ctx.save_for_backward(four, pre)
        ctx.mark_non_differentiable(four)
        return four, out

    @staticmethod
    def backward(ctx, _gfour, gout):
        four, pre = ctx.saved_tensors
        mod = ctx.mod
        wshape = tuple(mod.class_embed.linear.weight.shape) if ctx.labels is not None else None
        ges, gwch = ops.embed_combine_bwd(gout.contiguous(), pre, ctx.labels, mod.add_factor, wshape, drop=ctx.drop)
        dws = ops.linear_wgrad(ges, four)
        gws = mod.sigma_embed.finish_grad(dws.view(1, 1, *dws.shape))
        gwc = mod.class_embed.linear.finish_grad(gwch.view(1, 1, *gwch.shape)) if gwch is not None else None
        gwa = None
        if ctx.aug is not None and ctx.needs_input_grad[6]:
            dwa = ops.aug_embed_wgrad(ges, ctx.aug)
            gwa = mod.aug_embed.finish_grad(dwa.view(1, 1, *dwa.shape))
        return None, None, gws, gwc, None, None, gwa


class Embedding(nn.Module):

    _local_extensions = ("label_dropout", "augment_dim")

    def __init__(self, fourier_dim: int, embedding_dim: int, num_classes: int | None = None, add_factor: float = 0.5,
                 label_dropout: float = 0.0, augment_dim: int = 0):
        super().__init__()
        augment_dim = int(augment_dim)
        if augment_dim < 0:
            raise ValueError(f"Embedding: augment_dim must be >= 0, got {augment_dim}")
        self.augment_dim = augment_dim
        label_dropout = float(label_dropout)
        if not 0.0 <= label_dropout <= 1.0:
            raise ValueError(f"Embedding: label_dropout must be in [0, 1], got {label_dropout}")
        if label_dropout > 0 and (num_classes is None or num_classes == -1):
            raise ValueError("Embedding: label_dropout > 0 needs a class-conditional embedding (num_classes)")
        self.label_dropout = label_dropout
        self.last_label_drop = None
        self.fourier_dim = fourier_dim
        self.add_factor = add_factor
        self.embedding_dim = embedding_dim
        self.num_classes = num_classes
        self.fourier_embed = FourierEmbedding(fourier_dim)
        self.sigma_embed = Linear(fourier_dim, embedding_dim)
        self.sigma_embed.weight._edm_late = True
        self.class_embed = None
        if num_classes is not None and num_classes != -1:
            self.class_embed = ClassEmbedding(num_classes, embedding_dim)
            self.class_embed.linear.weight._edm_late = True
        self.aug_embed = None
        if augment_dim > 0:
            self.aug_embed = Linear(augment_dim, embedding_dim)
            self.aug_embed.weight._edm_late = True

    def forward(self, sigmas: Tensor, class_labels: Tensor | None = None, augment_labels: Tensor | None = None):
        if augment_labels is not None and self.aug_embed is None:
            raise ValueError("augment_labels is not None, but augment_dim is 0. ")
        if class_labels is not None and self.class_embed is None:
            raise ValueError("class_labels is not None, but num_classes is None. ")
        if not sigmas.is_cuda:
            raise RuntimeError("tinyedm_amd.Embedding: sigma must be a GPU tensor (there is no CPU path)")
        sigma = sigmas.detach().float().flatten().contiguous()
        labels = None
        if class_labels is not None:
            labels = class_labels.detach().to(sigma.device).flatten().to(torch.int64).contiguous()
            if sigma.numel() not in (1, labels.numel()):
                raise ValueError("sigma and class_labels batch sizes differ")
        w_cls = self.class_embed.linear.weight if labels is not None else None
        aug = w_aug = None
        if augment_labels is not None:
            aug = augment_labels.detach().to(sigma.device).float().contiguous()
            if aug.dim() != 2 or aug.shape[1] != self.augment_dim:
                raise ValueError(f"augment_labels must have shape (B, {self.augment_dim}), got {tuple(aug.shape)}")
            if sigma.numel() not in (1, aug.shape[0]) or (labels is not None and labels.numel() != aug.shape[0]):
                raise ValueError("sigma / class_labels and augment_labels batch sizes differ")
            w_aug = self.aug_embed.weight
        four, out = _EmbeddingFn.apply(sigma, labels, self.sigma_embed.weight, w_cls, self, aug, w_aug)
        if sigmas.numel() == 1:
            four = four[:1]
        return four, out


def _qkv_perm(C: int, heads: int) -> Tensor:
    d = C // heads
    h = torch.arange(heads).view(heads, 1, 1)
    w = torch.arange(3).view(1, 3, 1)
    dd = torch.arange(d).view(1, 1, d)
    return (h * 3 * d + dd * 3 + w).reshape(-1).to(torch.int32)


class CosineAttention(nn.Module):
    def __init__(self, embedding_dim: int, num_heads):
        super().__init__()
        assert embedding_dim % num_heads == 0
        self.num_heads = num_heads
        self.head_dim = embedding_dim // num_heads
        self.embedding_dim = embedding_dim
        self.qkv_conv = Conv2d(embedding_dim, 3 * embedding_dim, 1)
        self.out_conv = Conv2d(embedding_dim, embedding_dim, 1)
        self.qkv_conv._perm = _qkv_perm(embedding_dim, num_heads)

    def forward_nhwc(self, x: Tensor, dest=None) -> Tensor:
        out = _AttnFn.apply(x, self.qkv_conv.weight, self.out_conv.weight, self, dest, torch.is_grad_enabled())
        if dest is not None and out.data_ptr() == dest[0].data_ptr():
            out._edm_cat = dest
        return out

    def forward(self, x: Tensor) -> Tensor:
        y = self.forward_nhwc(ops.nchw_to_nhwc_bf16(x.float().contiguous()))
        return ops.nhwc_bf16_to_nchw(y).to(x.dtype)

    def forward_f32(self, x: Tensor, xp: Tensor | None = None, want=None):
        qkv = _conv_f32(self.qkv_conv, xp if (xp is not None and _split_ok(self.qkv_conv)) else x, 1)
        B, H, W, _ = qkv.shape
        if _split_ok(self.out_conv) and ops.split_attention_ok(self.embedding_dim, self.num_heads, H * W):
            y = ops.split_attention(qkv, self.num_heads, pairs=True)
        else:
            y = ops.f32_attention(qkv, self.num_heads)
        a, b = _mp_coeffs(0.5)
        return _conv_f32(self.out_conv, y, 1, residual=x, alpha=b, beta=a, want=want)


class _AttnFn(torch.autograd.Function):

    @staticmethod
    def forward(ctx, x, w_qkv, w_out, mod: CosineAttention, dest=None, grad_mode: bool = True):
        wf_qkv, wd_qkv, _ = mod.qkv_conv.packs()
        wf_out, wd_out, _ = mod.out_conv.packs()
        fused = ops.attention_qkv_supported(x, mod.num_heads)
        stat = qkv = None
        if fused:
            y, stat = ops.attention_qkv_fwd(x, wf_qkv, mod.num_heads, want_stat=grad_mode and any(ctx.needs_input_grad[:3]))
        else:
            qkv = ops.conv_igemm(x, wf_qkv, 1)
            y = ops.attention_fwd(qkv, mod.num_heads)
        a, b = _mp_coeffs(0.5)
        C = wf_out.shape[1]
        if _dest_ok(dest, y):
            out = ops.conv_igemm(y, wf_out, 1, residual=x, alpha=b, beta=a, out=_col_block(dest[0], C),
                                 silu_out=_col_block(dest[1], C))
            out._edm_cat = dest
        else:
            out = ops.conv_igemm(y, wf_out, 1, residual=x, alpha=b, beta=a)
        ctx.mod, ctx.fused = mod, fused
        if fused:
            ctx.save_for_backward(x, stat, y, wd_qkv, wd_out, wf_qkv)
        else:
            ctx.save_for_backward(x, qkv, y, wd_qkv, wd_out)
        return out

    @staticmethod
    def backward(ctx, gout):
        mod = ctx.mod
        gout = gout.contiguous()
        a, b = _mp_coeffs(0.5)
        if ctx.fused:
            x, stat, y, wd_qkv, wd_out, wf_qkv = ctx.saved_tensors
            if stat is None:
                raise RuntimeError("tinyedm_amd: attention backward without the forward's softmax statistics (the forward ran "
                                   "under torch.no_grad())")
            gqkv = ops.attention_qkv_bwd(x, y, gout, stat, wf_qkv, wd_out, mod.num_heads, alpha=b)
        else:
            x, qkv, y, wd_qkv, wd_out = ctx.saved_tensors
            gy = ops.conv_igemm(gout, wd_out, 1, alpha=b)
            gqkv = ops.attention_bwd(qkv, y, gy, mod.num_heads)
        gw_out = _wgrad(mod.out_conv, y, gout, 1, b)
        gx = ops.conv_igemm(gqkv, wd_qkv, 1, residual=gout, alpha=1.0, beta=a)
        gw_qkv = _wgrad(mod.qkv_conv, x, gqkv, 1)
        return gx, gw_qkv, gw_out, None, None, None


class _ResBlockFn(torch.autograd.Function):

    @staticmethod
    def forward(ctx, u, emb, w1x1, w1, w2, wemb, gain, blk, lin_view, glin_view, token, s_pre=None, alias=False,
                gm_view=None, skip=None, w_sl1=None, w_sl2=None, pre=None, dest=None, pool=False, gate_pre=None):
        enc = blk.is_encoder
        ctx.set_materialize_grads(False)
        has1 = w1x1 is not None
        taps = 9
        wf1, wd1, _ = blk.conv_3x3_1.packs()
        wf2, wd2, _ = blk.conv_3x3_2.packs()
        batched = lin_view is not None
        weh = None if batched else blk.embed.packs()[2]
        wd11 = None
        ctx.has_skip = skip is not None
        if skip is not None:
            sl = blk.cat_factor
            ctx.sgb = None
            if gate_pre is not None:
                mean, gate, z1, w1h, w2h, ctx.sgb, halves = gate_pre
            else:
                w1h, w2h = sl.layer1.packs()[2], sl.layer2.packs()[2]
                mean, gate, z1 = ops.skip_gate_fwd(skip, w1h, w2h)
            ctx.Ci = u.shape[-1]
            if pre is not None and pre[0].shape[-1] == u.shape[-1] + skip.shape[-1] and pre[0].data_ptr() == u.data_ptr():
                cat, s_pre = pre
                if not (gate_pre is not None and halves == cat.data_ptr()):
                    ops.skip_half_fwd(skip, gate, cat, s_pre)
            else:
                cat, s_pre = ops.concat_gate_fwd(u.contiguous(), skip, gate, True)
            u = cat
            ctx.skip_saved = (skip, mean, gate, z1, w1h, w2h)
        ctx.pool = bool(pool)
        if enc and pool:
            assert not has1
            xres, s, dsave = ops.pool_pixelnorm_silu_fwd(u)
        elif enc:
            x = u
            if has1:
                wf11, wd11, _ = blk.conv_1x1.packs()
                x = ops.conv_igemm(u, wf11, 1)
            xres, s, dsave = ops.pixelnorm_silu_fwd(x)
        else:
            xres = u
            fold = False
            if has1:
                wf11, wd11, _ = blk.conv_1x1.packs()
                fold = u.is_contiguous() and ops.conv3x3_fold_supported((*u.shape[:3], wf1.shape[1]), wf2.shape[1], u.shape[-1])
                if not fold:
                    xres = ops.conv_igemm(u, wf11, 1)
            s = s_pre if s_pre is not None else ops.silu_fwd(u)
            dsave = None
        lin = lin_view if batched else ops.linear_fwd(emb, weh)
        pdrop = blk.dropout_rate if blk.training else 0.0
        seed, sub, step = rng.seed, blk.rng_sub, rng.step
        if ops.FUSE_MOD and ops.IGEMM_VERSION == 0:
            r1, a2 = ops.conv3x3_mod(s, wf1, lin, gain, pdrop, seed, sub, step, want_u=any(ctx.needs_input_grad),
                                     dyn=rng.dyn, mark_dropped=U_MARKS)
        else:
            r1 = ops.conv_igemm(s, wf1, taps)
            a2 = ops.mod_silu_drop_fwd(r1, lin, gain, pdrop, seed, sub, step, dyn=rng.dyn)
        a, b = _mp_coeffs(blk.add_factor)
        Co = wf2.shape[1]
        if (not enc) and fold:
            if _dest_ok(dest, a2):
                out = ops.conv3x3_fold(a2, wf2, u, wf11, b, a, out=_col_block(dest[0], Co), silu_out=_col_block(dest[1], Co))
                out._edm_cat = dest
            else:
                out = ops.conv3x3_fold(a2, wf2, u, wf11, b, a)
        elif _dest_ok(dest, a2):
            out = ops.conv_igemm(a2, wf2, taps, residual=xres, alpha=b, beta=a, out=_col_block(dest[0], Co),
                                 silu_out=_col_block(dest[1], Co))
            out._edm_cat = dest
        else:
            out = ops.conv_igemm(a2, wf2, taps, residual=xres, alpha=b, beta=a)
        ctx.blk, ctx.enc, ctx.has1 = blk, enc, has1
        ctx.drop = (pdrop, seed, sub, step, rng.dyn)
        ctx.u_marked = U_MARKS and ops.FUSE_MOD and ops.IGEMM_VERSION == 0
        ctx.batched, ctx.glin_view, ctx.gm_view = batched, glin_view, gm_view
        ctx.has_token = token is not None
        ctx.save_for_backward(u if (not enc or has1) else None, xres if enc else None, dsave, s, r1, lin, a2,
                              None if batched else emb, gain, wd1, wd2, wd11, weh)
        return (out, u) if alias else out

    @staticmethod
    def backward(ctx, gout, g_alias=None):
        u, xn, dsave, s, r1, lin, a2, emb, gain, wd1, wd2, wd11, weh = ctx.saved_tensors
        if g_alias is not None:
            g_alias = g_alias.contiguous()
        blk, enc, has1 = ctx.blk, ctx.enc, ctx.has1
        pdrop, seed, sub, step, dyn = ctx.drop
        gout = gout.contiguous()
        a, b = _mp_coeffs(blk.add_factor)
        glin_out = ctx.glin_view if ctx.batched else None
        gp = blk.gain
        gdirect = gp.grad is not None and getattr(gp, "_edm_direct", False) and gp.grad.is_contiguous()
        ggain_out = gp.grad if gdirect else None
        deferred = False
        fused = ops.FUSE_MOD and ops.IGEMM_VERSION == 0 and (gout.shape[1] * gout.shape[2]) % 32 == 0
        tail = None
        if blk._tail_last:
            slot = _tail_slot.pop(gout.device.index, None)
            w2 = blk.conv_3x3_2.weight
            if (slot is not None and slot[2].data_ptr() == gout.data_ptr() and slot[2].shape == gout.shape
                    and w2.grad is not None and getattr(w2, "_edm_direct", False) and r1 is not None
                    and wd2.dim() == 3 and not getattr(wd2, "_edm_frag", False)
                    and ops.lowrank_supported(r1.shape[-1], slot[0].shape[1], r1.shape[2], 9)):
                tail = slot[:2]
        if tail is not None:
            deferred = ctx.gm_view is not None and gdirect and (fused or MOD_DEFER_UNFUSED)
            gr1, glin, ggain = ops.lowrank_dgrad3x3_modbwd(tail[0], ops.lowrank_expand_wc(tail[1], wd2), b, r1, lin, gain, pdrop,
                                                             seed, sub, step, glin_out=glin_out, ggain_out=ggain_out, dyn=dyn,
                                                             gm_out=ctx.gm_view if deferred else None, u_marked=ctx.u_marked)
            if deferred:
                gp._edm_deferred = True
        elif fused:
            deferred = ctx.gm_view is not None and gdirect
            gr1, glin, ggain = ops.conv3x3_modbwd(gout, wd2, b, r1, lin, gain, pdrop, seed, sub, step, glin_out=glin_out,
                                                     ggain_out=ggain_out, dyn=dyn, gm_out=ctx.gm_view if deferred else None,
                                                     u_marked=ctx.u_marked)
            if deferred:
                gp._edm_deferred = True
        else:
            deferred = MOD_DEFER_UNFUSED and ctx.gm_view is not None and gdirect
            ga2 = ops.conv_igemm(gout, wd2, 9, alpha=b)
            gr1, glin, ggain = ops.mod_silu_drop_bwd(r1, lin, gain, ga2, pdrop, seed, sub, step, glin_out=glin_out,
                                                        ggain_out=ggain_out, dyn=dyn, gm_out=ctx.gm_view if deferred else None)
            if deferred:
                gp._edm_deferred = True
        if gdirect:
            ggain = None
            if not deferred:
                for hook in getattr(gp, "_edm_hooks", ()):
                    hook(gp)
        if tail is not None:
            gw2 = _wgrad_lowrank(blk.conv_3x3_2, a2, tail[0], tail[1], b)
        else:
            gw2 = _wgrad(blk.conv_3x3_2, a2, gout, 9, b)
        gwemb = gemb = gtoken = None
        if ctx.batched:
            gtoken = ops.zeros_f32((1,), gout.device) if ctx.has_token else None
        else:
            dweh = ops.linear_wgrad(glin, emb)
            gwemb = blk.embed.finish_grad(dweh.view(1, 1, *dweh.shape))
            gemb = ops.linear_dgrad(glin, weh) if ctx.needs_input_grad[1] else None
        fuse = ops.FUSE_MOD and ops.IGEMM_VERSION == 0 and not enc
        gs = None if fuse else ops.conv_igemm(gr1, wd1, 9)
        gw1 = _wgrad(blk.conv_3x3_1, s, gr1, 9)
        gw11 = None
        if enc and ctx.pool:
            gu = ops.pool_pixelnorm_silu_bwd(xn, dsave, gout, a, gs, gadd=g_alias)
            g_alias = None
        elif enc:
            gx = ops.pixelnorm_silu_bwd(xn, dsave, gout, a, gs, gadd=None if has1 else g_alias)
            if has1:
                gw11 = _wgrad(blk.conv_1x1, u, gx, 1)
                gu = ops.conv_igemm(gx, wd11, 1, residual=g_alias, alpha=1.0, beta=1.0 if g_alias is not None else 0.0)
            else:
                gu = gx
            g_alias = None
        else:
            if has1:
                t = ops.conv3x3_silubwd(gr1, wd1, u) if fuse else ops.silu_bwd(u, gs)
                if ctx.has_skip:
                    Ci = ctx.Ci
                    B_, H_, W_, Ct = u.shape
                    gu = torch.empty(B_, H_, W_, Ci, device=u.device, dtype=bf16)
                    gcs = torch.empty(B_, H_, W_, Ct - Ci, device=u.device, dtype=bf16)
                    ops.conv_igemm(gout, wd11, 1, residual=t, alpha=a, beta=1.0, split=(Ci, gu, gcs))
                else:
                    gu = ops.conv_igemm(gout, wd11, 1, residual=t, alpha=a, beta=1.0)
                    gcs = None
                gw11 = _wgrad(blk.conv_1x1, u, gout, 1, a)
            else:
                gu = ops.conv3x3_silubwd(gr1, wd1, u, gout, a) if fuse else ops.silu_bwd(u, gs, gout, a)
                gcs = None
        gskip = gwsl1 = gwsl2 = None
        if ctx.has_skip:
            skip, mean, gate, z1, w1h, w2h = ctx.skip_saved
            Ci = ctx.Ci
            sl = blk.cat_factor
            wsl = (sl.layer1.weight, sl.layer2.weight)
            defer = SG_DEFER and all(w.grad is not None and getattr(w, "_edm_direct", False) for w in wsl)
            sgb = getattr(ctx, "sgb", None)
            queued = False
            if gcs is None:
                gmean, *gws = ops.skip_gate_bwd(gu, Ci, skip, mean, w1h, w2h, gate, z1, defer_wgrad=defer)
                gu, gskip = ops.concat_gate_bwd(gu, gate, gmean, Ci)
            elif defer and sgb is not None and SG_BWD_MULTI:
                gskip = torch.empty_like(gcs)
                sgb.pending.append((gcs, skip, w1h, w2h, gate, z1, gskip, sl, mean))
                queued = True
            else:
                gmean, *gws = ops.skip_gate_bwd(gcs, 0, skip, mean, w1h, w2h, gate, z1, defer_wgrad=defer)
                gskip = ops.skip_half_bwd(gcs, gate, gmean)
            if defer:
                if not queued:
                    _sg_pending.setdefault(wsl[0].device.index, []).append((sl, gws[0], mean, w1h.shape[0]))
                wsl[0]._edm_deferred = wsl[1]._edm_deferred = True
                _queue_backward_end(wsl[0].device)
            else:
                gw1h, gw2h = gws
                gwsl1 = sl.layer1.finish_grad(gw1h.view(1, 1, *gw1h.shape))
                gwsl2 = sl.layer2.finish_grad(gw2h.view(1, 1, *gw2h.shape))
            if sgb is not None:
                sgb.arrived += 1
                if sgb.arrived == sgb.expected:
                    sgb.flush()
        if g_alias is not None:
            gu = ops.axpby(gu, 1.0, g_alias, 1.0)
        return (gu, gemb, gw11, gw1, gw2, gwemb, ggain, None, None, None, gtoken, None, None, None, gskip, gwsl1, gwsl2,
                None, None, None, None)


_rng_sub_counter = [0]


class _BlockBase(nn.Module):
    is_encoder = True

    def _common(self, out_channels, embedding_dim, attention, num_heads, dropout_rate):
        self.conv_3x3_2 = Conv2d(out_channels, out_channels, 3)
        self.dropout = nn.Dropout(dropout_rate)
        self.attention = CosineAttention(out_channels, num_heads) if attention else nn.Identity()
        self.embed = Linear(embedding_dim, out_channels)
        self.embed.weight._edm_late = True
        self.gain = nn.Parameter(torch.ones(()))
        self._tail_last = False
        _rng_sub_counter[0] += 1
        self.rng_sub = _rng_sub_counter[0]

    def _res(self, u: Tensor, embedding: Tensor, lin=None, s_pre=None, alias=False, skip=None, dest=None, pool=False,
             gate=None):
        w11 = self.conv_1x1.weight if isinstance(self.conv_1x1, Conv2d) else None
        has_attn = isinstance(self.attention, CosineAttention)
        sk = ()
        if skip is not None or dest is not None or pool:
            cf = self.cat_factor if skip is not None else None
            sk = (skip, cf.layer1.weight if cf is not None else None, cf.layer2.weight if cf is not None else None,
                  getattr(u, "_edm_cat", None) if skip is not None else None, None if has_attn else dest, bool(pool),
                  gate if skip is not None else None)
        if lin is None:
            out = _ResBlockFn.apply(u, embedding, w11, self.conv_3x3_1.weight, self.conv_3x3_2.weight,
                                    self.embed.weight, self.gain, self, None, None, None, s_pre, alias, None, *sk)
        else:
            lin_view, glin_view, token, gm_view = lin
            out = _ResBlockFn.apply(u, None, w11, self.conv_3x3_1.weight, self.conv_3x3_2.weight, None, self.gain,
                                    self, lin_view, glin_view, token, s_pre, alias, gm_view, *sk)
        ualias = None
        if alias:
            out, ualias = out
        if has_attn:
            out = self.attention.forward_nhwc(out, dest)
        elif dest is not None and out.data_ptr() == dest[0].data_ptr():
            out._edm_cat = dest
        return (out, ualias) if alias else out


_SPLIT_EVAL = [False]
F32_FUSE_OUT = os.environ.get("EDM_F32_FUSE_OUT", "1") != "0"


def _split_ok(mod) -> bool:
    return bool(_SPLIT_EVAL[0]) and isinstance(mod, _WNBase) and mod.weight.shape[1] % 32 == 0 and mod.weight.shape[0] % 8 == 0


class _CatPre:
    __slots__ = ("cat", "sil")

    def __init__(self, cat, sil):
        self.cat, self.sil = cat, sil


def _conv_f32(mod: "_WNBase", x: Tensor, taps: int, pairs_out: bool = False, want=None, **kw):
    w_hat = mod.packs()[2]
    if _split_ok(mod):
        key = (mod.weight.data_ptr(), mod.weight._version, _WEIGHT_EPOCH)
        if mod._split_pack is None or mod._split_key != key:
            if torch.cuda.is_current_stream_capturing():
                raise RuntimeError("tinyedm_amd: split-bf16 weight pack is stale under stream capture (the plan refreshes "
                                   "it before the capture: Denoiser._prep_all)")
            mod._split_pack, mod._split_key = ops.split_pack(w_hat, taps), key
        xp = x if x.dtype == bf16 else ops.f32_to_pairs(x)
        if want == "pairs":
            return ops.split_conv(xp, mod._split_pack, taps, also_pairs=True, **kw)
        if want == "silu":
            return ops.split_conv(xp, mod._split_pack, taps, silu_pairs=True, **kw)
        if want is not None:
            _, cat, sil = want
            ops.split_conv(xp, mod._split_pack, taps, dest=(cat, sil), **kw)
            return _CatPre(cat, sil)
        return ops.split_conv(xp, mod._split_pack, taps, pairs_out=pairs_out, **kw)
    if x.dtype == bf16 or pairs_out or want is not None:
        raise RuntimeError("tinyedm_amd: split-bf16 pairs reached a conv that runs on the exact-fp32 kernel")
    return ops.f32_conv(x, w_hat, taps, **kw)


def _res_f32(blk, xres, s: Tensor, lin: Tensor, want=None):
    a2 = _conv_f32(blk.conv_3x3_1, s, 9, lin=lin, gain=blk.gain.detach(),
                   pairs_out=_split_ok(blk.conv_3x3_1) and _split_ok(blk.conv_3x3_2))
    a, b = _mp_coeffs(blk.add_factor)
    kw = dict(residual=xres)
    if isinstance(xres, tuple):
        m1 = blk.conv_1x1
        kw = dict(fold=(xres[1], m1._split_pack))
    if isinstance(blk.attention, CosineAttention):
        both = _split_ok(blk.conv_3x3_2) and _split_ok(blk.attention.qkv_conv)
        out = _conv_f32(blk.conv_3x3_2, a2, 9, alpha=b, beta=a, want="pairs" if both else None, **kw)
        out, outp = out if both else (out, None)
        return blk.attention.forward_f32(out, outp, want)
    return _conv_f32(blk.conv_3x3_2, a2, 9, alpha=b, beta=a, want=want, **kw)


def _out_conv_split(blk) -> bool:
    return _split_ok(blk.attention.out_conv if isinstance(blk.attention, CosineAttention) else blk.conv_3x3_2)


def _as_nhwc(x: Tensor):
    if x.dtype == bf16 and getattr(x, "_edm_nhwc", False):
        return x, False
    return ops.nchw_to_nhwc_bf16(x.float().contiguous()), True


def _tag(x: Tensor) -> Tensor:
    x._edm_nhwc = True
    return x


class EncoderBlock(_BlockBase):
    is_encoder = True

    def __init__(self, in_channels: int, out_channels: int, embedding_dim: int, down: bool, attention: bool,
                 num_heads: int = 4, dropout_rate: float = 0.0, add_factor: float = 0.3):
        super().__init__()
        self.dropout_rate = dropout_rate
        self.add_factor = add_factor
        self.resample = DownSample() if down else nn.Identity()
        self.conv_1x1 = Conv2d(in_channels, out_channels, 1) if in_channels != out_channels else nn.Identity()
        self.conv_3x3_1 = Conv2d(out_channels, out_channels, 3)
        self._common(out_channels, embedding_dim, attention, num_heads, dropout_rate)

    def forward(self, input: Tensor, embedding: Tensor, _lin=None, _alias: bool = False, _dest=None):
        x, conv = _as_nhwc(input)
        ualias = None
        emb = None if _lin is not None else _emb32(embedding, x.shape[0])
        if (isinstance(self.resample, DownSample) and FUSE_RESAMPLE and not isinstance(self.conv_1x1, Conv2d)
                and x.shape[-1] <= 1024 and x.shape[1] % 2 == 0 and x.shape[2] % 2 == 0):
            out = self._res(x, emb, _lin, alias=_alias, pool=True, dest=_dest)
            if _alias:
                out, ualias = out
        else:
            if isinstance(self.resample, DownSample):
                if _alias:
                    x, ualias = _ResampleFn.apply(x, False, True)
                else:
                    x = _ResampleFn.apply(x, False)
            if _alias and ualias is None:
                out, ualias = self._res(x, emb, _lin, alias=True, dest=_dest)
            else:
                out = self._res(x, emb, _lin, dest=_dest)
        if conv:
            out = ops.nhwc_bf16_to_nchw(out).to(input.dtype)
        else:
            cat_pre = getattr(out, "_edm_cat", None)
            out = _tag(out)
            if cat_pre is not None:
                out._edm_cat = cat_pre
        return (out, _tag(ualias)) if _alias else out

    def forward_f32(self, x: Tensor, lin: Tensor, want=None):
        pairs = _split_ok(self.conv_3x3_1)
        if (F32_FUSE_OUT and isinstance(self.resample, DownSample) and not isinstance(self.conv_1x1, Conv2d)
                and x.shape[-1] <= 1024):
            xn, s = ops.f32_pool_pixelnorm_silu(x, pairs=pairs)
        else:
            if isinstance(self.resample, DownSample):
                x = ops.f32_pool2(x)
            if isinstance(self.conv_1x1, Conv2d):
                x = _conv_f32(self.conv_1x1, x, 1)
            xn, s = ops.f32_pixelnorm_silu(x, pairs=pairs)
        return _res_f32(self, xn, s, lin, want)


class DecoderBlock(_BlockBase):
    is_encoder = False

    def __init__(self, in_channels: int, out_channels: int, embedding_dim: int, up: bool, attention: bool,
                 num_heads: int = 4, skip_channels: int = 0, dropout_rate: float = 0.0, add_factor: float = 0.3):
        super().__init__()
        self.add_factor = add_factor
        self.dropout_rate = dropout_rate
        self.cat_factor = ScaleLong(skip_channels) if skip_channels > 0 else None
        self.resample = UpSample() if up else nn.Identity()
        total = in_channels + skip_channels
        self.conv_1x1 = Conv2d(total, out_channels, 1) if total != out_channels else nn.Identity()
        self.conv_3x3_1 = Conv2d(total, out_channels, 3)
        self._common(out_channels, embedding_dim, attention, num_heads, dropout_rate)

    def _gate_in_block(self) -> bool:
        return (FUSE_CAT and SKIP_GATE_FUSED and not isinstance(self.resample, UpSample)
                and isinstance(self.conv_1x1, Conv2d) and self.cat_factor is not None)

    def forward(self, input: Tensor, embedding: Tensor, skip: Tensor | None = None, _lin=None, _dest=None, _gate=None) -> Tensor:
        x, conv = _as_nhwc(input)
        s_pre = None
        if skip is not None and FUSE_CAT and SKIP_GATE_FUSED and not isinstance(self.resample, UpSample) \
                and isinstance(self.conv_1x1, Conv2d):
            assert self.cat_factor is not None
            sk, _ = _as_nhwc(skip)
            out = self._res(x, None if _lin is not None else _emb32(embedding, x.shape[0]), _lin, skip=sk, dest=_dest,
                            gate=_gate)
            return ops.nhwc_bf16_to_nchw(out).to(input.dtype) if conv else _tag(out)
        if skip is not None:
            assert self.cat_factor is not None
            sk, _ = _as_nhwc(skip)
            fuse_silu = not isinstance(self.resample, UpSample)
            x = _ConcatGateFn.apply(x, sk, self.cat_factor.layer1.weight, self.cat_factor.layer2.weight, self.cat_factor,
                                    fuse_silu)
            if fuse_silu:
                x, s_pre = x
        if skip is None and not isinstance(self.resample, UpSample):
            pre = getattr(x, "_edm_cat", None)
            if pre is not None and pre[0].data_ptr() == x.data_ptr() and pre[0].shape == x.shape:
                s_pre = pre[1]
        if isinstance(self.resample, UpSample):
            if FUSE_RESAMPLE:
                x, s_pre = _ResampleFn.apply(x, True, False, True)
            else:
                x = _ResampleFn.apply(x, True)
                s_pre = None
        out = self._res(x, None if _lin is not None else _emb32(embedding, x.shape[0]), _lin, s_pre, dest=_dest)
        return ops.nhwc_bf16_to_nchw(out).to(input.dtype) if conv else _tag(out)

    @staticmethod
    def _split_pack_ready(mod) -> bool:
        key = (mod.weight.data_ptr(), mod.weight._version, _WEIGHT_EPOCH)
        return mod._split_pack is not None and mod._split_key == key

    def forward_f32(self, x, lin: Tensor, skip: Tensor | None = None, want=None):
        s = silp = pre = None
        if isinstance(x, _CatPre):
            pre = x
        elif isinstance(x, tuple):
            x, silp = x
        up = isinstance(self.resample, UpSample)
        if skip is not None:
            cf = self.cat_factor
            gate = ops.f32_skip_gate(skip, cf.layer1.packs()[2], cf.layer2.packs()[2])
            if pre is not None:
                ops.f32_skip_half(skip, gate, pre.cat, pre.sil)
                x, s = pre.cat, pre.sil
            else:
                pairs = (not up) and isinstance(self.conv_1x1, Conv2d) and _split_ok(self.conv_1x1) and _split_ok(self.conv_3x3_1)
                x, s = ops.f32_concat_gate(x, skip, gate, not up, pairs=pairs)
        elif pre is not None:
            raise RuntimeError("tinyedm_amd: a pre-concatenated input reached a decoder block without a skip")
        if up and F32_FUSE_OUT:
            x, s = ops.f32_up2_silu(x, pairs=_split_ok(self.conv_3x3_1))
        elif up:
            x, s = ops.f32_up2(x), None
        if (isinstance(self.conv_1x1, Conv2d) and F32_FUSE_OUT and x.dtype == bf16 and _split_ok(self.conv_1x1)
                and _split_ok(self.conv_3x3_1) and _split_ok(self.conv_3x3_2) and self._split_pack_ready(self.conv_1x1)
                and ops.split_conv_fold_supported((*x.shape[:3], 2 * self.conv_3x3_2.weight.shape[1]),
                                                  self.conv_3x3_2.weight.shape[0], x.shape[-1] // 2)):
            xres = ("fold", x)
        else:
            xres = _conv_f32(self.conv_1x1, x, 1) if isinstance(self.conv_1x1, Conv2d) else x
        if s is None:
            s = silp if (silp is not None and _split_ok(self.conv_3x3_1)) else ops.f32_silu(x, pairs=_split_ok(self.conv_3x3_1))
        return _res_f32(self, xres, s, lin, want)


def _emb32(embedding: Tensor, B: int) -> Tensor:
    e = embedding.float()
    if e.dim() != 2:
        raise ValueError("embedding must be (B, E)")
    if e.shape[0] != B:
        if e.shape[0] != 1:
            raise ValueError(f"embedding batch {e.shape[0]} does not match input batch {B}")
        e = e.expand(B, -1)
    return e.contiguous()


def get_encoder_blocks_types() -> tuple[str, ...]:
    return ("Enc",) * 3 + ("EncD",) + ("Enc",) * 3 + ("EncD",) + ("EncA",) * 3 + ("EncD",) + ("EncA",) * 3


def get_decoder_blocks_types() -> tuple[str, ...]:
    return (("DecA", "Dec") + ("DecA",) * 4 + ("DecU",) + ("DecA",) * 4 + ("DecU",) + ("Dec",) * 4 + ("DecU",)
            + ("Dec",) * 4)


def get_encoder_out_channels() -> tuple[int, ...]:
    return (192,) * 4 + (384,) * 4 + (576,) * 4 + (768,) * 3


def get_decoder_out_channels() -> tuple[int, ...]:
    return (768,) * 6 + (576,) * 5 + (384,) * 6 + (192,) * 4


def get_skip_connections() -> tuple[bool, ...]:
    return (False, False) + (True,) * 4 + ((False,) + (True,) * 4) * 3


def get_skip_channels(encoder_out_channels, decoder_out_channels, skip_connections) -> tuple[int, ...]:
    pool = iter(list(encoder_out_channels[::-1]) + [encoder_out_channels[0]])
    return tuple(int(next(pool)) if flag else 0 for flag in skip_connections)


def build_encoder_blocks(block_types, out_channels, **kwargs):
    blocks = nn.ModuleList()
    cin = out_channels[0]
    for t, cout in zip(block_types, out_channels):
        blocks.append(EncoderBlock(in_channels=cin, out_channels=cout, down=t.endswith("D"), attention=t.endswith("A"),
                                   **kwargs))
        cin = cout
    return blocks


def build_decoder_blocks(block_types, out_channels, skip_channels, **kwargs):
    blocks = nn.ModuleList()
    cin = out_channels[0]
    for t, cout, sc in zip(block_types, out_channels, skip_channels):
        blocks.append(DecoderBlock(in_channels=cin, out_channels=cout, skip_channels=sc, up=t.endswith("U"),
                                   attention=t.endswith("A"), **kwargs))
        cin = cout
    return blocks


class _EmbedAllFn(torch.autograd.Function):

    @staticmethod
    def forward(ctx, emb, den, *weights):
        ctx.set_materialize_grads(False)
        blocks = den._res_blocks()
        wcat = den._wcat(blocks)
        lin_all = ops.linear_fwd(emb, wcat)
        glin_all = ops.zeros_f32(lin_all.shape, lin_all.device)
        table = den._modfin_table(blocks) if any(ctx.needs_input_grad) else None
        gm_all = ops.zeros_f32(lin_all.shape, lin_all.device) if table is not None else None
        ctx.den, ctx.glin_all, ctx.gm_all, ctx.lin_all, ctx.table = den, glin_all, gm_all, lin_all, table
        ctx.save_for_backward(emb, wcat)
        token = ops.zeros_f32((1,), emb.device)
        if gm_all is not None:
            ctx.mark_non_differentiable(lin_all, glin_all, gm_all)
        else:
            ctx.mark_non_differentiable(lin_all, glin_all)
        return lin_all, glin_all, token, gm_all

    @staticmethod
    def backward(ctx, _g1, _g2, _gtoken, _g4=None):
        emb, wcat = ctx.saved_tensors
        glin_all = ctx.glin_all
        if ctx.gm_all is not None:
            ops.mod_finish_multi(ctx.gm_all, ctx.lin_all, glin_all, ctx.table, len(ctx.den._res_blocks()))
            for b in ctx.den._res_blocks():
                gp = b.gain
                if getattr(gp, "_edm_deferred", False):
                    gp._edm_deferred = False
                    for hook in getattr(gp, "_edm_hooks", ()):
                        hook(gp)
        dw = ops.linear_wgrad(glin_all, emb)
        gemb = ops.linear_dgrad(glin_all, wcat) if ctx.needs_input_grad[0] else None
        gws, off = [], 0
        for b in ctx.den._res_blocks():
            C = b.embed.weight.shape[0]
            gws.append(b.embed.finish_grad(dw[off:off + C].view(1, 1, C, -1)))
            off += C
        return (gemb, None, *gws)


class _ConvInFn(torch.autograd.Function):

    @staticmethod
    def forward(ctx, noisy, sigma, w, den: "Denoiser"):
        wf, _, _ = den.conv_in.packs()
        xin = ops.precond_in(noisy, sigma, den.sigma_data, den.conv_in._ipad)
        ctx.den = den
        ctx.save_for_backward(xin)
        return ops.conv_igemm(xin, wf, 9)

    @staticmethod
    def backward(ctx, gy):
        (xin,) = ctx.saved_tensors
        gw = _wgrad(ctx.den.conv_in, xin, gy.contiguous(), 9)
        return None, None, gw, None


class _ConvOutFn(torch.autograd.Function):

    @staticmethod
    def forward(ctx, x, w, gain_out, noisy, sigma, den: "Denoiser"):
        wh = den.conv_out.packs()[2]
        D, Fraw = ops.conv_out_fwd(x, wh, gain_out, noisy, sigma, den.sigma_data, want_fraw=True)
        ctx.den = den
        ctx.save_for_backward(x, wh, gain_out, Fraw, sigma)
        return D

    @staticmethod
    def backward(ctx, gD):
        x, wh, gain_out, Fraw, sigma = ctx.saved_tensors
        gp = ctx.den.gain_out
        gdirect = gp.grad is not None and getattr(gp, "_edm_direct", False) and gp.grad.is_contiguous()
        w = ctx.den.conv_out.weight
        dD = gD.contiguous().float()
        if (TAIL_LOWRANK and w.grad is not None and getattr(w, "_edm_direct", False)
                and ops.lowrank_supported(x.shape[-1], wh.shape[0], x.shape[2], 1)):
            dF, aux = ops.lowrank_df(dD, Fraw, gain_out, sigma, ctx.den.sigma_data)
            gx = ops.conv_out_bwd_x(wh, gain_out, dD, sigma, ctx.den.sigma_data, x.shape[-1])
            G, gg = ops.lowrank_wgrad(dF, x, 1, aux=aux, aux_out=gp.grad if gdirect else None)
            gwh = G.view(G.shape[0], G.shape[2])
            _tail_slot[gx.device.index] = (dF, wh, gx)
            _queue_backward_end(gx.device)
        else:
            gx, gwh, gg = ops.conv_out_bwd(x, wh, gain_out, Fraw, dD, sigma, ctx.den.sigma_data,
                                           gg_out=gp.grad if gdirect else None)
        if gdirect:
            gg = None
            for hook in getattr(gp, "_edm_hooks", ()):
                hook(gp)
        gw = ctx.den.conv_out.finish_grad(gwh.view(1, 1, *gwh.shape))
        return gx, gw, gg, None, None, None


class Denoiser(nn.Module):
    def __init__(
        self,
        in_channels: int = 3,
        out_channels: int = 3,
        encoder_block_types: tuple[str, ...] = get_encoder_blocks_types(),
        decoder_block_types: tuple[str, ...] = get_decoder_blocks_types(),
        encoder_out_channels: tuple[int, ...] = get_encoder_out_channels(),
        decoder_out_channels: tuple[int, ...] = get_decoder_out_channels(),
        skip_connections: tuple[bool, ...] = get_skip_connections(),
        dropout_rate: float = 0.0,
        sigma_data: float = 0.5,
        encoder_add_factor: float = 0.3,
        decoder_add_factor: float = 0.3,
        embedding_dim: int = 768,
        num_heads: int = 4,
    ):
        super().__init__()
        assert len(encoder_block_types) == len(encoder_out_channels), (
            f"encoder_block_types and encoder_out_channels must have the same length, got "
            f"{len(encoder_block_types)} and {len(encoder_out_channels)}")
        assert len(decoder_block_types) == len(decoder_out_channels), (
            f"decoder_block_types and decoder_out_channels must have the same length, got "
            f"{len(decoder_block_types)} and {len(decoder_out_channels)}")
        assert len(skip_connections) == len(decoder_out_channels), (
            f"skip_connections must have the same length as decoder_out_channels, got "
            f"{len(skip_connections)} and {len(decoder_out_channels)}")
        encoder_block_types, decoder_block_types = tuple(encoder_block_types), tuple(decoder_block_types)
        encoder_out_channels, decoder_out_channels = tuple(encoder_out_channels), tuple(decoder_out_channels)
        skip_connections = tuple(bool(s) for s in skip_connections)

        self.conv_in = Conv2d(in_channels + 1, encoder_out_channels[0], 3)
        self.conv_in._ipad = 32 * ((in_channels + 1 + 31) // 32)
        self.conv_in._want = ("fwd",)
        self.conv_out = Conv2d(decoder_out_channels[-1], out_channels, 1)
        self.conv_out._want = ("hat",)
        self.gain_out = nn.Parameter(torch.zeros(()))

        self.encoder_blocks = build_encoder_blocks(
            encoder_block_types, encoder_out_channels, embedding_dim=embedding_dim, dropout_rate=dropout_rate,
            add_factor=encoder_add_factor, num_heads=num_heads)
        skip_channels = get_skip_channels(encoder_out_channels, decoder_out_channels, skip_connections)
        self.decoder_blocks = build_decoder_blocks(
            decoder_block_types, decoder_out_channels, skip_channels, embedding_dim=embedding_dim,
            dropout_rate=dropout_rate, add_factor=decoder_add_factor, num_heads=num_heads)
        if len(self.decoder_blocks):
            self.decoder_blocks[-1]._tail_last = True

        self.in_channels = in_channels
        self.out_channels = out_channels
        self.encoder_block_types = encoder_block_types
        self.decoder_block_types = decoder_block_types
        self.encoder_out_channels = encoder_out_channels
        self.decoder_out_channels = decoder_out_channels
        self.skip_connections = skip_connections
        self.dropout_rate = dropout_rate
        self.sigma_data = sigma_data
        self.encoder_add_factor = encoder_add_factor
        self.decoder_add_factor = decoder_add_factor
        self.embedding_dim = embedding_dim
        self.num_heads = num_heads

    def _res_blocks(self):
        return list(self.encoder_blocks) + list(self.decoder_blocks)

    def _modfin_table(self, blocks):
        gains = [b.gain for b in blocks]
        if not all(g.grad is not None and getattr(g, "_edm_direct", False) and g.grad.is_contiguous() for g in gains):
            return None
        key = tuple((g.data_ptr(), g.grad.data_ptr()) for g in gains)
        cached = getattr(self, "_modfin", None)
        if cached is None or cached[0] != key:
            rec = np.zeros(len(blocks), dtype=np.dtype([("gain", "<u8"), ("ggain", "<u8"), ("col0", "<i4"), ("C", "<i4")]))
            assert rec.dtype.itemsize == 24
            off = 0
            for k, (b, g) in enumerate(zip(blocks, gains)):
                C = b.embed.weight.shape[0]
                rec[k] = (g.data_ptr(), g.grad.data_ptr(), off, C)
                off += C
            cached = self._modfin = (key, torch.from_numpy(rec.view(np.uint8).copy()).to(gains[0].device))
        return cached[1]

    @staticmethod
    def _decoder_gates(dec, skips, dests=None):
        return _decoder_gates_impl(dec, skips, dests)

    @staticmethod
    def _silu_dest(block, nxt, x, up, down=False):
        if not FUSE_CAT or isinstance(nxt.resample, UpSample) or nxt.cat_factor is not None:
            return None
        Bx, Hx, Wx, _ = x.shape
        if down:
            Hx, Wx = Hx // 2, Wx // 2
        Co = block.conv_3x3_2.weight.shape[0]
        return (torch.empty(Bx, Hx * up, Wx * up, Co, device=x.device, dtype=bf16),
                torch.empty(Bx, Hx * up, Wx * up, Co, device=x.device, dtype=bf16))

    def _frag_flags(self, B: int, H: int, W: int):
        cache = self.__dict__.setdefault("_fragcache", {})
        key = (B, H, W, ops.IGEMM_VERSION)
        if key not in cache:
            flags = {}
            h, w = H, W

            def mark(conv, hh, ww):
                O, I = conv.weight.shape[:2]
                f = (ops.uses_s_kernel(B, hh, ww, I, O), ops.uses_s_kernel(B, hh, ww, O, I))
                if f[0] or f[1]:
                    flags[conv] = f
            for blk in self.encoder_blocks:
                if isinstance(blk.resample, DownSample):
                    h, w = h // 2, w // 2
                mark(blk.conv_3x3_1, h, w)
                mark(blk.conv_3x3_2, h, w)
            for blk in self.decoder_blocks:
                if isinstance(blk.resample, UpSample):
                    h, w = h * 2, w * 2
                mark(blk.conv_3x3_1, h, w)
                mark(blk.conv_3x3_2, h, w)
            cache[key] = flags
        return cache[key]

    MAX_PLANS = 6

    def _eff_wants(self, mods):
        hat = (not self.training) and self.eval_dtype != "bf16"
        split = (not self.training) and self.eval_dtype == "f32x3"
        out = []
        for m in mods:
            w = tuple(m._want)
            if hat and "hat" not in w:
                w += ("hat",)
            if split and m.weight.dim() == 4 and m.weight.shape[1] % 32 == 0 and m.weight.shape[0] % 8 == 0:
                w += ("split",)
            out.append(w)
        return tuple(out)

    def _prep_all(self, shape=None):
        mods = [m for m in self.modules() if isinstance(m, _WNBase)]
        frag = self._frag_flags(*shape) if (shape is not None and FRAG_PACKS) else {}
        ptrs = tuple(m.weight.data_ptr() for m in mods)
        base = (ptrs, self._eff_wants(mods))
        key = base + (tuple((k, v) for k, v in enumerate(frag.get(m) for m in mods) if v),)
        plans = self.__dict__.setdefault("_plans", {})
        if shape is None and not self.training:
            for k, plan in plans.items():
                if k[:2] == base and k != key:
                    plan.run(False)
        plan = plans.pop(key, None)
        if plan is None:
            plan = _PrepPlan(mods, frag, base[1], cat=[b.embed for b in self._res_blocks()])
            for k in [k for k, p in plans.items() if k[0] != ptrs and not p.pinned]:
                del plans[k]
            live = [k for k, p in plans.items() if not p.pinned]
            for k in live[:max(0, len(live) + 1 - self.MAX_PLANS)]:
                del plans[k]
        plans[key] = plan
        plan.run(self.training)
        self.__dict__["_embed_wcat"] = plan.wcat

    def _wcat(self, blocks) -> Tensor:
        whs = [b.embed.packs()[2] for b in blocks]
        w = self.__dict__.get("_embed_wcat")
        if w is not None and all(wh._base is w for wh in whs) and sum(wh.shape[0] for wh in whs) == w.shape[0]:
            return w
        return torch.cat(whs, 0)

    eval_dtype = "bf16"

    def set_eval_dtype(self, dtype: str) -> "Denoiser":
        dtype = {"float32": "f32", "fp32": "f32", "bfloat16": "bf16", "split": "f32x3"}.get(str(dtype).replace("torch.", ""), str(dtype))
        if dtype not in ("bf16", "f32", "f32x3"):
            raise ValueError("Denoiser.set_eval_dtype: 'bf16', 'f32' (exact fp32 products) or 'f32x3' (split-bf16, fp32-accurate)")
        self.eval_dtype = dtype
        return self

    def _forward_f32(self, noisy: Tensor, sig: Tensor, emb: Tensor) -> Tensor:
        blocks = self._res_blocks()
        lin_all = ops.linear_fwd(emb, self._wcat(blocks))
        lins, off = {}, 0
        for b in blocks:
            C = b.embed.weight.shape[0]
            lins[b] = lin_all[:, off:off + C]
            off += C
        cp = 8 * ((self.in_channels + 1 + 7) // 8)
        x = ops.f32_conv(ops.f32_precond_in(noisy, sig, self.sigma_data, cp), self.conv_in.packs()[2], 9)
        skips = [x]
        dec = list(zip(self.decoder_blocks, self.skip_connections))
        split = bool(_SPLIT_EVAL[0]) and F32_FUSE_OUT

        def want_of(block, nxt, n_skip, hw, skip_c):
            if not split or nxt is None or isinstance(nxt.resample, UpSample) or not _out_conv_split(block):
                return None
            if not _split_ok(nxt.conv_3x3_1):
                return None
            if n_skip:
                if not (isinstance(nxt.conv_1x1, Conv2d) and _split_ok(nxt.conv_1x1)):
                    return None
                Ct = block.conv_3x3_2.weight.shape[0] + skip_c
                shape = (noisy.shape[0], hw[0], hw[1], 2 * Ct)
                return ("dest", torch.empty(shape, device=noisy.device, dtype=bf16),
                        torch.empty(shape, device=noisy.device, dtype=bf16))
            return None if isinstance(nxt.conv_1x1, Conv2d) else "silu"

        enc = list(self.encoder_blocks)
        h, w = x.shape[1], x.shape[2]
        for i, block in enumerate(enc):
            if isinstance(block.resample, DownSample):
                h, w = h // 2, w // 2
            want = want_of(block, dec[0][0], dec[0][1], (h, w), 0) if (i + 1 == len(enc) and dec and not dec[0][1]) else None
            x = block.forward_f32(x, lins[block], want)
            skips.append(x[0] if isinstance(x, tuple) else x)
        for i, (block, has_skip) in enumerate(dec):
            skip = skips.pop() if has_skip else None
            if isinstance(block.resample, UpSample):
                h, w = 2 * h, 2 * w
            nxt, n_skip = dec[i + 1] if i + 1 < len(dec) else (None, False)
            want = want_of(block, nxt, n_skip, (h, w), skips[-1].shape[-1] if (n_skip and skips) else 0)
            x = block.forward_f32(x, lins[block], skip, want)
        return ops.f32_conv_out(x, self.conv_out.packs()[2], self.gain_out.detach(), noisy, sig, self.sigma_data)

    def forward(self, noisy_image: Tensor, sigma: Tensor, embedding: Tensor):
        prev, _IN_DENOISER[0] = _IN_DENOISER[0], True
        try:
            return self._forward(noisy_image, sigma, embedding)
        finally:
            _IN_DENOISER[0] = prev

    def _forward(self, noisy_image: Tensor, sigma: Tensor, embedding: Tensor):
        if not noisy_image.is_cuda:
            raise RuntimeError("tinyedm_amd.Denoiser: inputs must be GPU tensors (there is no CPU path)")
        if self.eval_dtype != "bf16" and not self.training:
            if torch.is_grad_enabled() and (noisy_image.requires_grad or embedding.requires_grad):
                raise RuntimeError("tinyedm_amd.Denoiser: the fp32 evaluation path is forward-only (use torch.no_grad())")
            with torch.no_grad():
                self._prep_all()
                noisy = noisy_image.float().contiguous()
                _SPLIT_EVAL[0] = self.eval_dtype == "f32x3"
                try:
                    D = self._forward_f32(noisy, sigma.detach().float().flatten().contiguous(),
                                          _emb32(embedding.detach(), noisy.shape[0]))
                finally:
                    _SPLIT_EVAL[0] = False
            return D.to(noisy_image.dtype)
        reset_backward_state()
        if torch.is_grad_enabled():
            global FORWARD_EPOCH
            FORWARD_EPOCH += 1
        with torch.no_grad():
            self._prep_all((noisy_image.shape[0], noisy_image.shape[2], noisy_image.shape[3]))
        noisy = noisy_image.float().contiguous()
        B = noisy.shape[0]
        sig = sigma.detach().float().flatten().contiguous()
        emb = _emb32(embedding, B)

        blocks = self._res_blocks()
        lin_all, glin_all, token, gm_all = _EmbedAllFn.apply(emb, self, *[b.embed.weight for b in blocks])
        lins, off = {}, 0
        for k, b in enumerate(blocks):
            C = b.embed.weight.shape[0]
            lins[b] = (lin_all[:, off:off + C], glin_all[:, off:off + C], token if k == 0 else None,
                       None if gm_all is None else gm_all[:, off:off + C])
            off += C

        x = _ConvInFn.apply(noisy, sig, self.conv_in.weight, self)
        skips = []
        dec = list(zip(self.decoder_blocks, self.skip_connections))
        enc = list(self.encoder_blocks)
        for k, block in enumerate(enc):
            dest = None
            if k + 1 == len(enc) and dec and not dec[0][1]:
                dest = self._silu_dest(block, dec[0][0], x, 1, down=isinstance(block.resample, DownSample))
            x, x_in = block(_tag(x), None, _lin=lins[block], _alias=True, _dest=dest)
            skips.append(x_in)
        skips.append(x)
        dests = _decoder_dests_impl(dec, skips, x) if FUSE_CAT and SKIP_GATE_FUSED else {}
        gates = self._decoder_gates(dec, skips, dests) if SG_MULTI else {}
        for i, (block, has_skip) in enumerate(dec):
            skip = skips.pop() if has_skip else None
            dest = dests.get(i)
            if dest is not None:
                pass
            elif i + 1 < len(dec):
                dest = self._silu_dest(block, dec[i + 1][0], x, 2 if isinstance(block.resample, UpSample) else 1)
            xin = _tag(x)
            cat_pre = getattr(x, "_edm_cat", None)
            if cat_pre is not None:
                xin._edm_cat = cat_pre
            x = block(xin, None, _tag(skip) if has_skip else None, _lin=lins[block], _dest=dest, _gate=gates.get(block))
        D = _ConvOutFn.apply(x, self.conv_out.weight, self.gain_out, noisy, sig, self)
        if self.training:
            rng.step += 1
        return D.to(noisy_image.dtype)


class _SgbPass:

    def __init__(self, expected: int):
        self.expected, self.arrived, self.pending = expected, 0, []

    def flush(self):
        items, self.pending = self.pending, []
        self.arrived = 0
        if not items:
            return
        by_c = {}
        for it in items:
            by_c.setdefault(it[1].shape[-1], []).append(it)
        halves = []
        for group in by_c.values():
            for k0 in range(0, len(group), 32):
                part = group[k0:k0 + 32]
                res = ops.skip_gate_bwd_multi([(gcs, 0, skip, w1h, w2h, gate, z1) + ((gskip,) if SG_HALVES else ())
                                               for gcs, skip, w1h, w2h, gate, z1, gskip, _, _ in part])
                for (gcs, skip, w1h, w2h, gate, z1, gskip, sl, mean), (gmean, ws) in zip(part, res):
                    if not SG_HALVES:
                        halves.append((gcs, gate, gmean, gskip))
                    _sg_pending.setdefault(sl.layer1.weight.device.index, []).append((sl, ws, mean, w1h.shape[0]))
        for k0 in range(0, len(halves), 32):
            ops.skip_half_bwd_multi(halves[k0:k0 + 32])


def _decoder_dests_impl(dec, skips, x):
    out = {}
    st = list(skips)
    h, w = x.shape[1], x.shape[2]
    for i, (block, has_skip) in enumerate(dec):
        if has_skip:
            st.pop()
        if isinstance(block.resample, UpSample):
            h, w = 2 * h, 2 * w
        if i + 1 < len(dec) and dec[i + 1][1]:
            nxt = dec[i + 1][0]
            if not isinstance(nxt.resample, UpSample) and isinstance(nxt.conv_1x1, Conv2d):
                Ct = block.conv_3x3_2.weight.shape[0] + st[-1].shape[-1]
                out[i] = (torch.empty(x.shape[0], h, w, Ct, device=x.device, dtype=bf16),
                          torch.empty(x.shape[0], h, w, Ct, device=x.device, dtype=bf16))
    return out


def _decoder_gates_impl(dec, skips, dests=None):
    st = list(skips)
    todo = {}
    for i, (block, has_skip) in enumerate(dec):
        if not has_skip:
            continue
        skip = st.pop()
        if not (isinstance(block, DecoderBlock) and block._gate_in_block() and skip.dim() == 4 and skip.dtype == bf16):
            continue
        sl = block.cat_factor
        pre = dests.get(i - 1) if dests and SG_HALVES else None
        if pre is not None and not (pre[0].shape[:3] == skip.shape[:3] and pre[0].shape[-1] > skip.shape[-1]):
            pre = None
        todo.setdefault(skip.shape[-1], []).append((block, skip, sl.layer1.packs()[2], sl.layer2.packs()[2], pre))
    out = {}
    tok = _SgbPass(sum(len(v) for v in todo.values())) if torch.is_grad_enabled() else None
    for items in todo.values():
        for k0 in range(0, len(items), 32):
            part = items[k0:k0 + 32]
            res = ops.skip_gate_fwd_multi([(skip, w1h, w2h) + (pre if pre is not None else ()) for _, skip, w1h, w2h, pre in part])
            for (block, _, w1h, w2h, pre), (mean, gate, z1) in zip(part, res):
                out[block] = (mean, gate, z1, w1h, w2h, tok, None if pre is None else pre[0].data_ptr())
    return out


class DenoiserWrapper(nn.Module):

    def __init__(self, net: nn.Module, sigma_data: float):
        super().__init__()
        self.net = net
        self._sigma_data = sigma_data

    @property
    def sigma_data(self) -> float:
        return self._sigma_data

    def forward(self, noisy_image: Tensor, sigma: Tensor, embedding: Tensor | None = None) -> Tensor:
        sigma = sigma.view(-1, 1, 1, 1)
        sd = self.sigma_data
        c_skip = sd ** 2 / (sigma ** 2 + sd ** 2)
        c_out = sigma * sd / (sigma ** 2 + sd ** 2).sqrt()
        c_in = 1 / (sd ** 2 + sigma ** 2).sqrt()
        c_noise = sigma.log() / 4
        F_ = self.net(c_in * noisy_image, c_noise.flatten(), embedding)
        return c_skip * noisy_image + c_out * F_
```

### tinyedm_amd/ops.py

```python
import contextlib
import ctypes
import functools
import math
import os
import types
from typing import Optional

import torch

from . import _lib

bf16, f32 = torch.bfloat16, torch.float32

PROFILE = None


class _prof:
    def __init__(self, name, flops, nbytes):
        self.name, self.flops, self.nbytes = name, flops, nbytes

    def __enter__(self):
        if PROFILE is not None:
            self.s = torch.cuda.Event(enable_timing=True)
            self.e = torch.cuda.Event(enable_timing=True)
# ... 521 lines not shown
    th, td, defer, release = _tables.take(items[0][0].device)
    _lib.call("edm_skip_gate_fwd_multi", ctypes.byref(arr), n, ctypes.c_void_p(th), ctypes.c_void_p(td), defer, _stream())
    release()
    return out


def skip_gate_bwd_multi(items):
    n = len(items)
    if not 0 < n <= 32:
        raise ValueError("skip_gate_bwd_multi: 1..32 gates per launch")
    arr = (_lib.SkipGateBwdItem * n)()
    out = []
    C0 = items[0][2].shape[-1]
    for k, item in enumerate(items):
        gcat, Ci, skip, w1h, w2h, gate, z1 = item[:7]
        gskip = item[7] if len(item) > 7 else None
        B, H, W, Ct = _nhwc(gcat, "gcat")
        Bs, Hs, Ws, C = _nhwc(skip, "skip")
        if (Bs, Hs, Ws) != (B, H, W) or Ct != Ci + C or C != C0:
            raise ValueError("skip_gate_bwd_multi: gcat/skip shape mismatch, or mixed channel counts in one launch")
        R = w1h.shape[0]
        _chk(w1h, f32, "w1h", (R, C + 1))
        _chk(w2h, f32, "w2h", (C, R))
        _chk(gate, f32, "gate", (B, C))
        _chk(z1, f32, "z1", (B, R))
        gmean = torch.empty(B, C, device=skip.device, dtype=f32)
        ws = torch.empty(B, C + 2 * R, device=skip.device, dtype=f32)
        if gskip is not None:
            _chk(gskip, bf16, "gskip", (B, H, W, C))
        arr[k] = _lib.SkipGateBwdItem(gcat.data_ptr(), Ct, skip.data_ptr(), w1h.data_ptr(), w2h.data_ptr(), gate.data_ptr(),
                                      z1.data_ptr(), gmean.data_ptr(), ws.data_ptr(), _p(gskip), Ci, B, H * W, C, R, 0)
        out.append((gmean, ws))
    th, td, defer, release = _tables.take(items[0][2].device)
    _lib.call("edm_skip_gate_bwd_multi", ctypes.byref(arr), n, ctypes.c_void_p(th), ctypes.c_void_p(td), defer, _stream())
    release()
    return out


def skip_half_bwd_multi(items):
    n = len(items)
    if not 0 < n <= 32:
        raise ValueError("skip_half_bwd_multi: 1..32 tensors per launch")
    arr = (_lib.SkipHalfBwdItem * n)()
    for k, (gcs, gate, gmean, gskip) in enumerate(items):
        B, H, W, Cs = _nhwc(gcs, "gcs")
        _chk(gate, f32, "gate", (B, Cs))
        _chk(gmean, f32, "gmean", (B, Cs))
        _chk(gskip, bf16, "gskip", (B, H, W, Cs))
        arr[k] = _lib.SkipHalfBwdItem(gcs.data_ptr(), gate.data_ptr(), gmean.data_ptr(), gskip.data_ptr(), B, H * W, Cs, 0)
    th, td, defer, release = _tables.take(items[0][0].device)
    _lib.call("edm_skip_half_bwd_multi", ctypes.byref(arr), n, ctypes.c_void_p(th), ctypes.c_void_p(td), defer, _stream())
    release()


def skip_gate_bwd(gcat, Ci, skip, mean, w1h, w2h, gate, z1, defer_wgrad=False):
    B, H, W, Ct = _nhwc(gcat, "gcat")
    Bs, Hs, Ws, C = _nhwc(skip, "skip")
    if (Bs, Hs, Ws) != (B, H, W) or Ci + C != Ct or Ci % 8:
        raise ValueError("skip_gate_bwd: gcat / skip shape mismatch")
    R = w1h.shape[0]
    _chk(mean, f32, "mean", (B, C))
    _chk(gate, f32, "gate", (B, C))
    _chk(z1, f32, "z1", (B, R))
    _chk(w1h, f32, "w1h", (R, C + 1))
    _chk(w2h, f32, "w2h", (C, R))
    gmean = torch.empty(B, C, device=skip.device, dtype=f32)
    gw1 = None if defer_wgrad else torch.empty(w1h.shape, device=w1h.device, dtype=f32)
    gw2 = None if defer_wgrad else torch.empty(w2h.shape, device=w2h.device, dtype=f32)
    ws = torch.empty(B, C + 2 * R, device=skip.device, dtype=f32)
    _lib.call("edm_skip_gate_bwd", _p(gcat), Ct, Ci, _p(skip), _p(mean), _p(w1h), _p(w2h), _p(gate), _p(z1), _p(gmean),
              _p(gw1), _p(gw2), _p(ws), B, H * W, C, R, _stream())
    return (gmean, ws) if defer_wgrad else (gmean, gw1, gw2)


def skip_gate_wgrad_multi(items):
    n = len(items)
    if not 0 < n <= 32:
        raise ValueError("skip_gate_wgrad_multi: 1..32 gates per launch")
    arr = (_lib.SkipGateWgradItem * n)()
    out = []
    for k, (ws, mean, R) in enumerate(items):
        _chk(mean, f32, "mean")
        B, C = mean.shape
        _chk(ws, f32, "ws", (B, C + 2 * R))
        gw1 = torch.empty(R, C + 1, device=ws.device, dtype=f32)
        gw2 = torch.empty(C, R, device=ws.device, dtype=f32)
        arr[k] = _lib.SkipGateWgradItem(ws.data_ptr(), mean.data_ptr(), gw1.data_ptr(), gw2.data_ptr(), B, C, R, 0)
        out.append((gw1, gw2))
    th, td, defer, release = _tables.take(items[0][0].device)
    _lib.call("edm_skip_gate_wgrad_multi", ctypes.byref(arr), n, ctypes.c_void_p(th), ctypes.c_void_p(td), defer, _stream())
    release()
    return out


def concat_gate_fwd(inp, skip, gate, want_silu):
    B, H, W, Ci = _nhwc(inp, "inp")
    Bs, Hs, Ws, Cs = _nhwc(skip, "skip")
    if (Bs, Hs, Ws) != (B, H, W):
        raise ValueError("concat_gate_fwd: inp/skip spatial mismatch")
    _chk(gate, f32, "gate", (B, Cs))
    cat = torch.empty(B, H, W, Ci + Cs, device=inp.device, dtype=bf16)
    sil = torch.empty_like(cat) if want_silu else None
    _lib.call("edm_concat_gate_fwd", _p(inp), _p(skip), _p(gate), _p(cat), _p(sil), B, H * W, Ci, Cs, _stream())
    return cat, sil


def concat_gate_bwd(gcat, gate, gmean, Ci):
    B, H, W, Ct = _nhwc(gcat, "gcat")
    Cs = Ct - Ci
    _chk(gate, f32, "gate", (B, Cs))
    _chk(gmean, f32, "gmean", (B, Cs))
    ginp = torch.empty(B, H, W, Ci, device=gcat.device, dtype=bf16)
    gskip = torch.empty(B, H, W, Cs, device=gcat.device, dtype=bf16)
    _lib.call("edm_concat_gate_bwd", _p(gcat), _p(gate), _p(gmean), _p(ginp), _p(gskip), B, H * W, Ci, Cs, _stream())
    return ginp, gskip


def skip_half_fwd(skip, gate, cat, sil=None):
    B, H, W, Cs = _nhwc(skip, "skip")
    _chk(gate, f32, "gate", (B, Cs))
    Ct = cat.shape[-1]
    _chk(cat, bf16, "cat", (B, H, W, Ct))
    if sil is not None:
        _chk(sil, bf16, "sil", (B, H, W, Ct))
    if Ct <= Cs:
        raise ValueError("skip_half_fwd: cat must be wider than the skip")
    _lib.call("edm_skip_half_fwd", _p(skip), _p(gate), _p(cat), _p(sil), B, H * W, Ct - Cs, Cs, _stream())


def skip_half_bwd(gcs, gate, gmean):
    B, H, W, Cs = _nhwc(gcs, "gcs")
    _chk(gate, f32, "gate", (B, Cs))
    _chk(gmean, f32, "gmean", (B, Cs))
    gskip = torch.empty_like(gcs)
    _lib.call("edm_skip_half_bwd", _p(gcs), _p(gate), _p(gmean), _p(gskip), B, H * W, Cs, _stream())
    return gskip


def _sigma_arg(sigma, B):
    _chk(sigma, f32, "sigma")
    if sigma.numel() == 1:
        return 0
    if sigma.numel() != B:
        raise ValueError(f"sigma must have 1 or {B} elements, got {sigma.numel()}")
    return 1


def precond_in(noisy, sigma, sigma_data, CP):
    _chk(noisy, f32, "noisy")
    B, Cimg, H, W = noisy.shape
    ss = _sigma_arg(sigma, B)
    out = torch.empty(B, H, W, CP, device=noisy.device, dtype=bf16)
    _lib.call("edm_precond_in", _p(noisy), _p(sigma), ss, float(sigma_data), _p(out), B, Cimg, H * W, CP, _stream())
    return out


def conv_out_fwd(x, w_hat, gain_out, noisy, sigma, sigma_data, want_fraw=True):
    B, H, W, C = _nhwc(x, "x")
    Co = w_hat.shape[0]
    _chk(w_hat, f32, "w_hat", (Co, C))
    _chk(noisy, f32, "noisy", (B, Co, H, W))
    _chk(gain_out, f32, "gain_out")
    ss = _sigma_arg(sigma, B)
    D = torch.empty(B, Co, H, W, device=x.device, dtype=f32)
    Fraw = torch.empty(B, Co, H, W, device=x.device, dtype=f32) if want_fraw else None
    _lib.call("edm_conv_out_fwd", _p(x), _p(w_hat), _p(gain_out), _p(noisy), _p(sigma), ss, float(sigma_data), _p(D),
              _p(Fraw), B, H * W, C, Co, _stream())
    return D, Fraw


def conv_out_bwd(x, w_hat, gain_out, Fraw, dD, sigma, sigma_data, gg_out=None):
    B, H, W, C = _nhwc(x, "x")
    Co = w_hat.shape[0]
    _chk(dD, f32, "dD", (B, Co, H, W))
    _chk(Fraw, f32, "Fraw", (B, Co, H, W))
    ss = _sigma_arg(sigma, B)
    gx = torch.empty_like(x)
    gw = zeros_f32(w_hat.shape, w_hat.device)
    gg = zeros_f32((), x.device) if gg_out is None else _chk(gg_out, f32, "gg_out", ())
    _lib.call("edm_conv_out_bwd", _p(x), _p(w_hat), _p(gain_out), _p(Fraw), _p(dD), _p(sigma), ss, float(sigma_data),
              _p(gx), _p(gw), _p(gg), B, H * W, C, Co, _stream())
    return gx, gw, gg


def conv_out_bwd_x(w_hat, gain_out, dD, sigma, sigma_data, C):
    Co = w_hat.shape[0]
    _chk(w_hat, f32, "w_hat", (Co, C))
    _chk(dD, f32, "dD")
    B, _, H, W = dD.shape
    ss = _sigma_arg(sigma, B)
    gx = torch.empty(B, H, W, C, device=dD.device, dtype=bf16)
    _lib.call("edm_conv_out_bwd", None, _p(w_hat), _p(gain_out), None, _p(dD), _p(sigma), ss, float(sigma_data),
              _p(gx), None, None, B, H * W, C, Co, _stream())
    return gx


LOWRANK_MAX_CO = 8


@functools.lru_cache(maxsize=None)
def lowrank_supported(C, Co, W, taps):
    return bool(_lib.lib().edm_lowrank_supported(int(C), int(Co), int(W), int(taps)))


def lowrank_df(dD, Fraw, gain_out, sigma, sigma_data, want_aux=True):
    _chk(dD, f32, "dD")
    B, Co, H, W = dD.shape
    ss = _sigma_arg(sigma, B)
    _chk(gain_out, f32, "gain_out")
    dF = torch.empty_like(dD)
    aux = None
    if want_aux:
        _chk(Fraw, f32, "Fraw", dD.shape)
        aux = torch.empty_like(dD)
    _lib.call("edm_lowrank_df", _p(dD), _p(Fraw), _p(gain_out), _p(sigma), ss, float(sigma_data), _p(dF), _p(aux), B, Co,
              H * W, _stream())
    return dF, aux


def _lowrank_args(dF, Wc, C):
    _chk(dF, f32, "dF")
    if dF.dim() != 4 or not 1 <= dF.shape[1] <= LOWRANK_MAX_CO:
        raise ValueError(f"dF: expected (B, Co <= {LOWRANK_MAX_CO}, H, W)")
    B, Co, H, W = dF.shape
    _chk(Wc, f32, "Wc", (Co, 9, C))
    return B, Co, H, W


def lowrank_dgrad3x3(dF, Wc, scale=1.0):
    C = Wc.shape[-1]
    B, Co, H, W = _lowrank_args(dF, Wc, C)
    ga = torch.empty(B, H, W, C, device=dF.device, dtype=bf16)
    _lib.call("edm_lowrank_dgrad3x3", _p(dF), _p(Wc), float(scale), _p(ga), None, None, 0, None, None, None, 0, 0.0, 0, 0, 0,
              0, B, H, W, C, Co, None, _stream())
    return ga


def lowrank_dgrad3x3_modbwd(dF, Wc, alpha, r1, lin, gain, pdrop, seed, sub, step, glin_out=None, ggain_out=None, dyn=None,
                            gm_out=None, u_marked=False):
    B, H, W, C = _nhwc(r1, "r1")
    if tuple(dF.shape[0:1] + dF.shape[2:]) != (B, H, W):
        raise ValueError(f"lowrank_dgrad3x3_modbwd: dF {tuple(dF.shape)} does not match r1 {tuple(r1.shape)}")
    _, Co, _, _ = _lowrank_args(dF, Wc, C)
    ls = _lin_view(lin, B, C, "lin")
    _chk(gain, f32, "gain")
    gr = torch.empty_like(r1)
    if gm_out is not None:
        gms = _lin_view(gm_out, B, C, "gm_out")
        gm = gm_out
    else:
        gms = C
        gm = zeros_f32((B, C), r1.device)
        glin = torch.empty(B, C, device=r1.device, dtype=f32) if glin_out is None else glin_out
        gs = _lin_view(glin, B, C, "glin")
        ggain = zeros_f32((), r1.device) if ggain_out is None else _chk(ggain_out, f32, "ggain_out", ())
    _lib.call("edm_lowrank_dgrad3x3", _p(dF), _p(Wc), float(alpha), None, _p(r1), _p(lin), ls, _p(gain), _p(gr), _p(gm),
              gms, float(pdrop), int(seed), int(sub), int(step), int(bool(u_marked)), B, H, W, C, Co, _dyn(dyn), _stream())
    if gm_out is not None:
        return gr, None, None
    _lib.call("edm_mod_finish", _p(gm), _p(lin), ls, _p(gain), _p(glin), gs, _p(ggain), B, C, _stream())
    return gr, glin, ggain


def lowrank_wgrad(dF, X, taps, aux=None, aux_out=None):
    B, H, W, C = _nhwc(X, "X")
    _chk(dF, f32, "dF")
    if dF.dim() != 4 or tuple(dF.shape[0:1] + dF.shape[2:]) != (B, H, W) or not 1 <= dF.shape[1] <= LOWRANK_MAX_CO:
        raise ValueError(f"lowrank_wgrad: dF {tuple(dF.shape)} does not match X {tuple(X.shape)}")
    if taps not in (1, 9):
        raise ValueError("lowrank_wgrad: taps must be 1 or 9")
    Co = dF.shape[1]
    asum = None
    if aux is not None:
        _chk(aux, f32, "aux", dF.shape)
        asum = zeros_f32((), X.device) if aux_out is None else _chk(aux_out, f32, "aux_out", ())
    G = torch.empty(Co, taps, C, device=X.device, dtype=f32)
    nws = int(_lib.call("edm_lowrank_wgrad_workspace", C, Co, taps))
    ws = torch.empty(nws, device=X.device, dtype=f32)
    _lib.call("edm_lowrank_wgrad", _p(dF), _p(X), int(taps), _p(aux), _p(G), _p(asum), _p(ws), nws, B, H, W, C, Co, _stream())
    return G, asum


def lowrank_expand_wc(wout_hat, wd):
    _chk(wd, bf16, "wd")
    if wd.dim() != 3 or getattr(wd, "_edm_frag", False):
        raise ValueError("lowrank_expand_wc: expected a plain (taps, I, O) dgrad pack")
    taps, I, O = wd.shape
    Co = wout_hat.shape[0]
    _chk(wout_hat, f32, "wout_hat", (Co, O))
    Wc = torch.empty(Co, taps, I, device=wd.device, dtype=f32)
    _lib.call("edm_lowrank_expand_wc", _p(wout_hat), _p(wd), _p(Wc), Co, O, I, taps, _stream())
    return Wc


def lowrank_expand_slab(wout_hat, G, scale=1.0, Ipad=None):
    _chk(G, f32, "G")
    Co, taps, I = G.shape
    O = wout_hat.shape[1]
    _chk(wout_hat, f32, "wout_hat", (Co, O))
    Ipad = I if Ipad is None else Ipad
    slab = torch.empty(1, taps, O, Ipad, device=G.device, dtype=f32)
    _lib.call("edm_lowrank_expand_slab", _p(wout_hat), _p(G), _p(slab), float(scale), Co, O, I, Ipad, taps, _stream())
    return slab


def nchw_to_nhwc_bf16(x):
    _chk(x, f32, "x")
    B, C, H, W = x.shape
    y = torch.empty(B, H, W, C, device=x.device, dtype=bf16)
    _lib.call("edm_nchw_to_nhwc_bf16", _p(x), _p(y), B, C, H * W, _stream())
    return y


def nhwc_bf16_to_nchw(x):
    B, H, W, C = _nhwc(x, "x")
    y = torch.empty(B, C, H, W, device=x.device, dtype=f32)
    _lib.call("edm_nhwc_bf16_to_nchw", _p(x), _p(y), B, C, H * W, _stream())
    return y


IGEMM_VERSION = int(os.environ.get("EDM_IGEMM", "0"))


_KERNEL_ID = {"edm_conv_igemm": 1, "edm_conv_igemm_v2": 2, "edm_conv_igemm_s": 5, "edm_conv_igemm_v6": 6}
_ENTRY = {kid: entry for entry, kid in _KERNEL_ID.items()}


@functools.lru_cache(maxsize=None)
def _conv_plan(B, H, W, Cin, Cout, taps, force):
    return _lib.lib().edm_conv_plan(B, H, W, Cin, Cout, taps, force)


def _igemm_entry(npix, W, Cout, taps, Cin):
    return _ENTRY[_conv_plan(1, npix // W, W, Cin, Cout, taps, IGEMM_VERSION) & 0xff]


def uses_s_kernel(B, H, W, Cin, Cout):
    return (IGEMM_VERSION == 0 and Cout % 64 == 0 and Cin % 32 == 0
            and _conv_plan(B, H, W, Cin, Cout, 9, 0) & 0xff == 5)


def _wfrag(wp, plan, who):
    if not getattr(wp, "_edm_frag", False):
        return 0
    if plan & 0xff != 5:
        raise ValueError(f"{who}: a fragment-major weight pack reached a shape that does not run on k_conv3x3_s ({_ENTRY[plan & 0xff]})")
    return 1


V46 = "_v6"


def _conv_key(plan, taps=9, tail=""):
    suffix = {1: "", 2: "_v2", 5: "_s", 6: V46 if plan >> 8 == 128 else V46 + "s"}[plan & 0xff]
    return ("conv3x3_igemm" if taps == 9 else "conv1x1_igemm") + suffix + tail


def conv_igemm(x, wp, taps, residual=None, alpha=1.0, beta=0.0, out=None, silu_out=None, split=None):
    B, H, W, Cin = _nhwc(x, "x")
    _chk(wp, bf16, "wp")
    if wp.dim() != 3 or wp.shape[0] != taps or wp.shape[2] != Cin:
        raise ValueError(f"conv_igemm: packed weight {tuple(wp.shape)} does not match taps={taps}, Cin={Cin}")
    Cout = wp.shape[1]
    if residual is not None:
        _chk(residual, bf16, "residual", (B, H, W, Cout))
    npix = B * H * W
    plan = _conv_plan(B, H, W, Cin, Cout, taps, IGEMM_VERSION)
    pname = _conv_key(plan, taps)
    nbytes = 2.0 * (npix * (Cin + Cout * ((2 if residual is not None else 1) + (1 if silu_out is not None else 0))) + wp.numel())
    wfrag = _wfrag(wp, plan, "conv_igemm")
    if out is None and silu_out is None and split is None and not wfrag:
        y = torch.empty(B, H, W, Cout, device=x.device, dtype=bf16)
        with _prof(pname, 2.0 * npix * Cin * Cout * taps, nbytes):
            _lib.call(_ENTRY[plan & 0xff], _p(x), _p(wp), _p(y), _p(residual), float(alpha), float(beta), B, H, W, Cin, Cout, taps, _stream())
        return y
    ld, ya, yb, ldb, c = 0, None, None, 0, 0
    if split is not None:
        if out is not None or silu_out is not None:
            raise ValueError("conv_igemm: split excludes out / silu_out")
        c, ya, yb = split
        _chk(ya, bf16, "split[1]", (B, H, W, c))
        _chk(yb, bf16, "split[2]", (B, H, W, Cout - c))
        if c % 8 or not (0 < c < Cout):
            raise ValueError("conv_igemm: split channel must be a multiple of 8 inside (0, Cout)")
        ld, ldb = c, Cout - c
    else:
        if out is None:
            out = torch.empty(B, H, W, Cout, device=x.device, dtype=bf16)
        ld = _row_view(out, B, H, W, Cout, "out")
        if silu_out is not None and _row_view(silu_out, B, H, W, Cout, "silu_out") != ld:
            raise ValueError("conv_igemm: out and silu_out must have the same row stride")
        ya = out
    with _prof(pname, 2.0 * npix * Cin * Cout * taps, nbytes):
        _lib.call("edm_conv_igemm_o", _p(x), _p(wp), _p(ya), ld, _p(silu_out), _p(yb), ldb, c, _p(residual), float(alpha),
                  float(beta), B, H, W, Cin, Cout, taps, plan & 0xff, wfrag, _stream())
    return (ya, yb) if split is not None else out


FOLD_PROJ = os.environ.get("EDM_FOLD_PROJ", "1") != "0"


def conv3x3_fold_supported(xshape, Cout, C2):
    B, H, W, Cin = xshape
    return bool(FOLD_PROJ and IGEMM_VERSION == 0 and _lib.call("edm_conv3x3_fold_supported", B, H, W, Cin, Cout, C2))


def conv3x3_fold(x, wp, x2, w2p, alpha3, alpha1, out=None, silu_out=None):
    B, H, W, Cin = _nhwc(x, "x")
    _chk(wp, bf16, "wp")
    _chk(w2p, bf16, "w2p")
    B2, H2, W2, C2 = _nhwc(x2, "x2")
    Cout = wp.shape[1]
    if wp.dim() != 3 or wp.shape[0] != 9 or wp.shape[2] != Cin or tuple(w2p.shape) != (1, Cout, C2) or (B2, H2, W2) != (B, H, W):
        raise ValueError(f"conv3x3_fold: operands do not match (x {tuple(x.shape)}, wp {tuple(wp.shape)}, x2 {tuple(x2.shape)}, "
                         f"w2p {tuple(w2p.shape)})")
    if getattr(wp, "_edm_frag", False):
        raise ValueError("conv3x3_fold: a fragment-major weight pack belongs to k_conv3x3_s")
    if out is None:
        out = torch.empty(B, H, W, Cout, device=x.device, dtype=bf16)
    ld = _row_view(out, B, H, W, Cout, "out")
    if silu_out is not None and _row_view(silu_out, B, H, W, Cout, "silu_out") != ld:
        raise ValueError("conv3x3_fold: out and silu_out must have the same row stride")
    npix = B * H * W
    with _prof(_conv_key(_conv_plan(B, H, W, Cin, Cout, 9, 6), tail="_fold"), 2.0 * npix * Cout * (9 * Cin + C2),
               2.0 * (npix * (Cin + C2 + Cout * (2 if silu_out is not None else 1)) + wp.numel() + w2p.numel())):
        _lib.call("edm_conv3x3_fold", _p(x), _p(wp), _p(x2), C2, _p(w2p), C2, _p(out), ld, _p(silu_out), float(alpha3),
                  float(alpha1), B, H, W, Cin, Cout, _stream())
    return out


def _row_view(t, B, H, W, C, name):
    if t.dtype != bf16 or not t.is_cuda or tuple(t.shape) != (B, H, W, C):
        raise ValueError(f"{name}: expected a cuda bf16 tensor of shape {(B, H, W, C)}, got {t.dtype} {tuple(t.shape)}")
    sb, sh, sw, sc = t.stride()
    if sc != 1 or sw < C or sw % 8 or sh != W * sw or sb != H * sh or (t.data_ptr() % 16):
        raise ValueError(f"{name}: strides {t.stride()} are not those of a column block of an NHWC buffer")
    return sw


FUSE_MOD = os.environ.get("EDM_FUSE_MOD", "1") != "0"


def conv3x3_mod(x, wp, lin, gain, pdrop, seed, sub, step, want_u=True, dyn=None, mark_dropped=False):
    B, H, W, Cin = _nhwc(x, "x")
    _chk(wp, bf16, "wp")
    if wp.dim() != 3 or wp.shape[0] != 9 or wp.shape[2] != Cin:
        raise ValueError(f"conv3x3_mod: pack shape {tuple(wp.shape)} does not match taps=9, Cin={Cin}")
    Cout = wp.shape[1]
    ls = _lin_view(lin, B, Cout, "lin")
    _chk(gain, f32, "gain")
    u = torch.empty(B, H, W, Cout, device=x.device, dtype=bf16) if want_u else None
    a2 = torch.empty(B, H, W, Cout, device=x.device, dtype=bf16)
    npix = B * H * W
    plan = _conv_plan(B, H, W, Cin, Cout, 9, 0)
    with _prof(_conv_key(plan), 2.0 * npix * Cin * Cout * 9, 2.0 * (npix * (Cin + Cout * (2 if want_u else 1)) + wp.numel())):
        _lib.call("edm_conv3x3_mod", _p(x), _p(wp), _p(u), _p(a2), _p(lin), ls, _p(gain), float(pdrop), int(seed),
                  int(sub), int(step), int(bool(mark_dropped)), B, H, W, Cin, Cout, _dyn(dyn), _wfrag(wp, plan, "conv3x3_mod"),
                  _stream())
    return u, a2


def conv3x3_modbwd(gout, wd, alpha, r1, lin, gain, pdrop, seed, sub, step, glin_out=None, ggain_out=None, dyn=None,
                   gm_out=None, u_marked=False):
    B, H, W, Cin = _nhwc(gout, "gout")
    _chk(wd, bf16, "wd")
    if wd.dim() != 3 or wd.shape[0] != 9 or wd.shape[2] != Cin:
        raise ValueError(f"conv3x3_modbwd: pack shape {tuple(wd.shape)} does not match taps=9, Cin={Cin}")
    Cout = wd.shape[1]
    _chk(r1, bf16, "r1", (B, H, W, Cout))
    if (H * W) % 32:
        raise ValueError("conv3x3_modbwd: H*W must be a multiple of 32")
    ls = _lin_view(lin, B, Cout, "lin")
    _chk(gain, f32, "gain")
    gr = torch.empty_like(r1)
    if gm_out is not None:
        gms = _lin_view(gm_out, B, Cout, "gm_out")
        gm = gm_out
    else:
        gms = 0
        gm = zeros_f32((B, Cout), r1.device)
        glin = torch.empty(B, Cout, device=r1.device, dtype=f32) if glin_out is None else glin_out
        gs = _lin_view(glin, B, Cout, "glin")
        ggain = zeros_f32((), r1.device) if ggain_out is None else _chk(ggain_out, f32, "ggain_out", ())
    npix = B * H * W
    plan = _conv_plan(B, H, W, Cin, Cout, 9, 0)
    with _prof(_conv_key(plan, tail="_modbwd"), 2.0 * npix * Cin * Cout * 9, 2.0 * (npix * (Cin + 2 * Cout) + wd.numel())):
        _lib.call("edm_conv3x3_modbwd", _p(gout), _p(wd), float(alpha), _p(r1), _p(lin), ls, _p(gain), _p(gr), _p(gm), gms,
                  float(pdrop), int(seed), int(sub), int(step), int(bool(u_marked)), B, H, W, Cin, Cout, _dyn(dyn),
                  _wfrag(wd, plan, "conv3x3_modbwd"), _stream())
    if gm_out is not None:
        return gr, None, None
    _lib.call("edm_mod_finish", _p(gm), _p(lin), ls, _p(gain), _p(glin), gs, _p(ggain), B, Cout, _stream())
    return gr, glin, ggain


def mod_finish_multi(gm_all, lin_all, glin_all, items, n_items):
    _chk(gm_all, f32, "gm_all")
    _chk(lin_all, f32, "lin_all", gm_all.shape)
    _chk(glin_all, f32, "glin_all", gm_all.shape)
    _chk(items, torch.uint8, "items")
    if gm_all.dim() != 2 or items.numel() != 24 * n_items:
        raise ValueError("mod_finish_multi: bad buffers")
    _lib.call("edm_mod_finish_multi", _p(gm_all), _p(lin_all), _p(glin_all), gm_all.shape[1], _p(items), int(n_items),
              gm_all.shape[0], _stream())


def conv3x3_silubwd(g, wd, xpre, gextra=None, extra_scale=1.0):
    B, H, W, Cin = _nhwc(g, "g")
    _chk(wd, bf16, "wd")
    if wd.dim() != 3 or wd.shape[0] != 9 or wd.shape[2] != Cin:
        raise ValueError(f"conv3x3_silubwd: pack shape {tuple(wd.shape)} does not match taps=9, Cin={Cin}")
    Cout = wd.shape[1]
    _chk(xpre, bf16, "xpre", (B, H, W, Cout))
    if gextra is not None:
        _chk(gextra, bf16, "gextra", xpre.shape)
    gx = torch.empty_like(xpre)
    npix = B * H * W
    plan = _conv_plan(B, H, W, Cin, Cout, 9, 0)
    with _prof(_conv_key(plan, tail="_silubwd"), 2.0 * npix * Cin * Cout * 9,
               2.0 * (npix * (Cin + Cout * (3 if gextra is not None else 2)) + wd.numel())):
        _lib.call("edm_conv3x3_silubwd", _p(g), _p(wd), _p(xpre), _p(gextra), float(extra_scale), _p(gx), B, H, W, Cin,
                  Cout, _wfrag(wd, plan, "conv3x3_silubwd"), _stream())
    return gx


WGRAD_1X1 = os.environ.get("EDM_WGRAD_1X1", "1") != "0"
WGRAD_VERSION = 2


def conv_wgrad(x, dy, taps):
    B, H, W, Cin = _nhwc(x, "x")
    Bd, Hd, Wd, Cout = _nhwc(dy, "dy")
    if (Bd, Hd, Wd) != (B, H, W):
        raise ValueError("conv_wgrad: x/dy spatial mismatch")
    npix = B * H * W
    if taps == 1 and WGRAD_1X1 and Cin % 32 == 0 and Cout % 32 == 0:
        S = _lib.call("edm_conv_wgrad_1x1_nsplit", npix, Cin, Cout)
        slabs = torch.empty(S, 1, Cout, Cin, device=x.device, dtype=f32)
        with _prof("conv1x1_wgrad", 2.0 * npix * Cin * Cout, 2.0 * npix * (Cin + Cout) + 4.0 * slabs.numel()):
            _lib.call("edm_conv_wgrad_1x1", _p(x), _p(dy), _p(slabs), npix, Cin, Cout, S, _stream())
        return slabs
    S = _lib.call("edm_conv_wgrad_nsplit", B, H, W, Cin, Cout, taps)
    slabs = torch.empty(S, taps, Cout, Cin, device=x.device, dtype=f32)
    with _prof("conv3x3_wgrad" if taps == 9 else "conv1x1_wgrad", 2.0 * npix * Cin * Cout * taps,
               2.0 * npix * (Cin + Cout) + 4.0 * slabs.numel()):
        _lib.call("edm_conv_wgrad_v2", _p(x), _p(dy), _p(slabs), B, H, W, Cin, Cout, taps, S, _stream())
    return slabs


def wgrad1x1_group_supported(x, dy):
    return WGRAD_1X1 and x.shape[-1] % 32 == 0 and dy.shape[-1] % 32 == 0


def conv_wgrad_1x1_group(pairs):
    n = len(pairs)
    if not 0 < n <= 16:
        raise ValueError("conv_wgrad_1x1_group: 1..16 layers per group")
    arr = (_lib.WGrad1Item * n)()
    out = []
    flops = nbytes = 0.0
    for k, (x, dy) in enumerate(pairs):
        B, H, W, Cin = _nhwc(x, "x")
        Bd, Hd, Wd, Cout = _nhwc(dy, "dy")
        if (Bd, Hd, Wd) != (B, H, W) or Cin % 32 or Cout % 32:
            raise ValueError("conv_wgrad_1x1_group: x/dy mismatch or channels not multiples of 32")
        npix = B * H * W
        S = _lib.call("edm_conv_wgrad_1x1_nsplit_grouped", npix, Cin, Cout)
        slabs = torch.empty(S, 1, Cout, Cin, device=x.device, dtype=f32)
        arr[k] = _lib.WGrad1Item(x.data_ptr(), dy.data_ptr(), slabs.data_ptr(), npix, Cin, Cout, S, 0)
        out.append(slabs)
        flops += 2.0 * npix * Cin * Cout
        nbytes += 2.0 * npix * (Cin + Cout) + 4.0 * slabs.numel()
    th, td, defer, release = _tables.take(pairs[0][0].device)
    with _prof("conv1x1_wgrad", flops, nbytes):
        _lib.call("edm_conv_wgrad_1x1_group", ctypes.byref(arr), n, ctypes.c_void_p(th), ctypes.c_void_p(td), defer, _stream())
    release()
    return out


W3_MAX_LAYERS = 48


def wgrad3_supported(x, dy, I):
    B, H, W, Cin = x.shape
    Cout = dy.shape[-1]
    return Cin % 32 == 0 and Cout % 32 == 0 and W <= 126 and I * 9 * 4 <= 64 * 1024 and B * (H + 1) * (W + 1) < (1 << 30)


def wgrad3_plan_ksplit(shapes):
    n = len(shapes)
    arr = (_lib.WGrad3Item * n)()
    for k, (B, H, W, Cin, Cout) in enumerate(shapes):
        arr[k] = _lib.WGrad3Item(1, 1, 1, 1, None, B, H, W, Cin, Cout, Cin, 1.0, 0)
    out = (ctypes.c_int * n)()
    _lib.call("edm_wgrad3_plan_ksplit", ctypes.byref(arr), n, out)
    return list(out)


def wgrad3_group(items):
    n = len(items)
    if not 0 < n <= W3_MAX_LAYERS:
        raise ValueError(f"wgrad3_group: 1..{W3_MAX_LAYERS} layers per group")
    arr = (_lib.WGrad3Item * n)()
    flops = nbytes = 0.0
    halo = None
    for k, (x, dy, w, grad, perm, scale, accumulate) in enumerate(items):
# ... 1250 lines not shown
```

Measured before the change: 10290 img/s.

## Fuse last decoder block's 3x3 conv, skip 1x1 and conv_out into low-rank tail

Adds a low-rank tail path that folds the final conv_out projection (few output channels) into the last decoder block's 3x3 conv and 1x1 skip. The forward computes D directly from the block's activations with small expanded weights, so the full-width block output is never materialised. The backward contracts the weight gradients and the concat input gradient through the rank-Co factor. The aim is to remove the full-width conv and conv_out GEMMs and their memory traffic at 32x32. In exchange it adds expand, wgrad and contraction kernels plus new side-stream scheduling, and it only runs when the direct-grad conditions hold.

```diff
diff --git a/include/tinyedm_hip.h b/include/tinyedm_hip.h
--- a/include/tinyedm_hip.h
+++ b/include/tinyedm_hip.h
@@ -225,6 +225,16 @@
                           edm_stream_t stream);
 int edm_lowrank_expand_slab(const float* wout_hat, const float* G, float* slab, float scale, int Co, int O, int I,
                             int Ipad, int taps, edm_stream_t stream);
+int edm_lowrank_tail_supported(int C, int Cc, int Co, int W);
+int edm_lowrank_tail_fwd(const void* a2, const void* cat, const float* Wc, const float* Wp, float sb, float sa,
+                         const float* gain_out, const float* noisy, const float* sigma, int sigma_stride, float sigma_data,
+                         float* D, float* Fraw, int B, int H, int W, int C, int Cc, int Co, edm_stream_t stream);
+int edm_lowrank_tail_dwout_supported(int C, int Cc, int Co, int has_1x1);
+int edm_lowrank_tail_dwout(const float* G, const void* wf2, const float* G1, const void* wf1, float sb, float sa,
+                           float* gw_hat, int Co, int C, int Cc, edm_stream_t stream);
+int edm_lowrank_gcat_supported(int Cc, int Ci, int Co);
+int edm_lowrank_gcat_add(const float* dF, const float* Wp, float sa, const void* t, void* gu, void* gcs, int B, int HW,
+                         int Cc, int Ci, int Co, edm_stream_t stream);
 
 int edm_nchw_to_nhwc_bf16(const float* x, void* y, int B, int C, int HW, edm_stream_t stream);
 int edm_nhwc_bf16_to_nchw(const void* x, float* y, int B, int C, int HW, edm_stream_t stream);
diff --git a/tinyedm_amd/_lib.py b/tinyedm_amd/_lib.py
--- a/tinyedm_amd/_lib.py
+++ b/tinyedm_amd/_lib.py
@@ -54,6 +54,12 @@
     "edm_lowrank_wgrad": [P, P, I, P, P, P, P, L, I, I, I, I, I, P],
     "edm_lowrank_expand_wc": [P, P, P, I, I, I, I, P],
     "edm_lowrank_expand_slab": [P, P, P, F, I, I, I, I, I, P],
+    "edm_lowrank_tail_supported": [I, I, I, I],
+    "edm_lowrank_tail_fwd": [P, P, P, P, F, F, P, P, P, I, F, P, P, I, I, I, I, I, I, P],
+    "edm_lowrank_tail_dwout_supported": [I, I, I, I],
+    "edm_lowrank_tail_dwout": [P, P, P, P, F, F, P, I, I, I, P],
+    "edm_lowrank_gcat_supported": [I, I, I],
+    "edm_lowrank_gcat_add": [P, P, F, P, P, P, I, I, I, I, I, P],
     "edm_conv_igemm": [P, P, P, P, F, F, I, I, I, I, I, I, P],
     "edm_conv_igemm_v2": [P, P, P, P, F, F, I, I, I, I, I, I, P],
     "edm_conv_plan": [I, I, I, I, I, I, I],
@@ -162,7 +168,7 @@
 _RET = {"edm_last_error": ctypes.c_char_p, "edm_lowrank_wgrad_workspace": ctypes.c_long, "edm_v6_persistent_launches": ctypes.c_long, "edm_wgrad3_workspace": ctypes.c_long, "edm_wgrad3_table_bytes": ctypes.c_long,
         "edm_skip_gate_wgrad_multi_table_bytes": ctypes.c_long, "edm_skip_gate_fwd_multi_table_bytes": ctypes.c_long, "edm_skip_gate_bwd_multi_table_bytes": ctypes.c_long,
         "edm_conv_wgrad_1x1_group_table_bytes": ctypes.c_long, "edm_wgrad_finish_multi_table_bytes": ctypes.c_long}
-_NO_STATUS = {"edm_lowrank_wgrad_workspace", "edm_lowrank_supported", "edm_skip_gate_bwd_multi_table_bytes", "edm_skip_gate_fwd_multi_table_bytes", "edm_v6_persistent_launches", "edm_conv3x3_fold_supported", "edm_conv_plan", "edm_skip_gate_wgrad_multi_table_bytes", "edm_version", "edm_graph_replay_safe", "edm_last_error", "edm_conv_wgrad_nsplit", "edm_conv_wgrad_1x1_nsplit", "edm_conv_wgrad_1x1_nsplit_grouped", "edm_wgrad3_workspace", "edm_wgrad3_table_bytes", "edm_wgrad3_max_layers",
+_NO_STATUS = {"edm_lowrank_wgrad_workspace", "edm_lowrank_supported", "edm_lowrank_tail_supported", "edm_lowrank_tail_dwout_supported", "edm_lowrank_gcat_supported", "edm_skip_gate_bwd_multi_table_bytes", "edm_skip_gate_fwd_multi_table_bytes", "edm_v6_persistent_launches", "edm_conv3x3_fold_supported", "edm_conv_plan", "edm_skip_gate_wgrad_multi_table_bytes", "edm_version", "edm_graph_replay_safe", "edm_last_error", "edm_conv_wgrad_nsplit", "edm_conv_wgrad_1x1_nsplit", "edm_conv_wgrad_1x1_nsplit_grouped", "edm_wgrad3_workspace", "edm_wgrad3_table_bytes", "edm_wgrad3_max_layers",
               "edm_conv_wgrad_1x1_group_table_bytes", "edm_wgrad_finish_multi_table_bytes", "edm_attention_qkv_supported",
               "edm_u8_knn_splits"}
 
diff --git a/tinyedm_amd/csrc/tail_lowrank.hip b/tinyedm_amd/csrc/tail_lowrank.hip
--- a/tinyedm_amd/csrc/tail_lowrank.hip
+++ b/tinyedm_amd/csrc/tail_lowrank.hip
@@ -458,3 +458,266 @@
   EDM_CHECK_LAUNCH("lowrank_expand_slab");
   return EDM_OK;
 }
+
+constexpr int TAIL_LPP = 8;
+static size_t tail_fwd_lds(int Co, int C, int Cc, int W, int R) {
+  return ((size_t)Co * 9 * C + (size_t)Co * Cc + (size_t)R * W * 10 * Co) * sizeof(float);
+}
+extern "C" int edm_lowrank_tail_supported(int C, int Cc, int Co, int W) {
+  if (C <= 0 || C % 8 || C > 1024 || Cc <= 0 || Cc % 8 || Cc > 2048 || Co < 1 || Co > 8 || W <= 0) return 0;
+  return tail_fwd_lds(Co, C, Cc, W, 1) <= LOWRANK_LDS_MAX;
+}
+
+template <int CO, int NK, int PX>
+__device__ __forceinline__ void tail_dots(const bf16* const (&xp)[PX], int Cx, const float* __restrict__ w, int wso, int lig,
+                                          float (&s)[PX][NK * CO]) {
+  f32x2 acc[PX][NK * CO];
+#pragma unroll
+  for (int k = 0; k < PX; ++k)
+#pragma unroll
+    for (int v = 0; v < NK * CO; ++v) acc[k][v] = f32x2{0.f, 0.f};
+  const int CL = Cx >> 3;
+  for (int c8 = lig; c8 < CL; c8 += TAIL_LPP) {
+    f32x2 xf[PX][4];
+#pragma unroll
+    for (int k = 0; k < PX; ++k) {
+      u32x4 raw = u32x4{0u, 0u, 0u, 0u};
+      if (xp[k]) raw = *reinterpret_cast<const u32x4*>(xp[k] + c8 * 8);
+      const bf16x8 xv = __builtin_bit_cast(bf16x8, raw);
+#pragma unroll
+      for (int h = 0; h < 4; ++h) xf[k][h] = f32x2{(float)xv[2 * h], (float)xv[2 * h + 1]};
+    }
+#pragma unroll
+    for (int o = 0; o < CO; ++o)
+#pragma unroll
+      for (int kk = 0; kk < NK; ++kk) {
+        const float* wp = w + (long)(o * wso + kk) * Cx + c8 * 8;
+        const f32x4 w0 = *reinterpret_cast<const f32x4*>(wp), w1 = *reinterpret_cast<const f32x4*>(wp + 4);
+        const f32x2 wv[4] = {f32x2{w0[0], w0[1]}, f32x2{w0[2], w0[3]}, f32x2{w1[0], w1[1]}, f32x2{w1[2], w1[3]}};
+#pragma unroll
+        for (int k = 0; k < PX; ++k)
+#pragma unroll
+          for (int h = 0; h < 4; ++h) acc[k][kk * CO + o] += xf[k][h] * wv[h];
+      }
+  }
+#pragma unroll
+  for (int k = 0; k < PX; ++k)
+#pragma unroll
+    for (int v = 0; v < NK * CO; ++v) s[k][v] = group_sum<TAIL_LPP>(acc[k][v][0] + acc[k][v][1]);
+}
+
+template <int CO, int PX>
+__global__ __launch_bounds__(512) void k_lowrank_tail_fwd(const bf16* __restrict__ a2, const bf16* __restrict__ cat,
+                                                          const float* __restrict__ Wc, const float* __restrict__ Wp,
+                                                          float sb, float sa, const float* __restrict__ gain_out,
+                                                          const float* __restrict__ noisy, const float* __restrict__ sigma,
+                                                          int sstride, float sd, float* __restrict__ D,
+                                                          float* __restrict__ Fraw, int H, int W, int C, int Cc, int R) {
+  extern __shared__ __attribute__((aligned(16))) float sm[];
+  float* wl = sm;
+  float* wpl = wl + CO * 9 * C;
+  float* pt = wpl + CO * Cc;
+  const int RW = R * W;
+  float* qt = pt + 3 * RW * 3 * CO;
+  const int b = blockIdx.y, y0 = blockIdx.x * R;
+  const int rows = min(R, H - y0);
+  for (int i = threadIdx.x; i < CO * 9 * C / 4; i += blockDim.x)
+    reinterpret_cast<f32x4*>(wl)[i] = reinterpret_cast<const f32x4*>(Wc)[i];
+  for (int i = threadIdx.x; i < CO * Cc / 4; i += blockDim.x)
+    reinterpret_cast<f32x4*>(wpl)[i] = reinterpret_cast<const f32x4*>(Wp)[i];
+  __syncthreads();
+  const int lig = threadIdx.x % TAIL_LPP, grp = threadIdx.x / TAIL_LPP, NG = blockDim.x / TAIL_LPP;
+#pragma unroll 1
+  for (int ky = 0; ky < 3; ++ky) {
+    const int r_lo = max(y0 + ky - 1, 0), r_hi = min(y0 + rows - 1 + ky - 1, H - 1);
+    const int np = (r_hi - r_lo + 1) * W;
+    const int slot0 = (r_lo - (y0 + ky - 1)) * W;
+    const bf16* base = a2 + (((long)b * H + r_lo) * W) * C;
+    float* po = pt + (long)ky * RW * 3 * CO;
+    for (int n0 = grp * PX; n0 < np; n0 += NG * PX) {
+      const bf16* xp[PX];
+#pragma unroll
+      for (int k = 0; k < PX; ++k) xp[k] = n0 + k < np ? base + (long)(n0 + k) * C : nullptr;
+      float s[PX][3 * CO];
+      tail_dots<CO, 3, PX>(xp, C, wl + ky * 3 * C, 9, lig, s);
+#pragma unroll
+      for (int k = 0; k < PX; ++k)
+        if (n0 + k < np) {
+#pragma unroll
+          for (int v = 0; v < 3 * CO; ++v)
+            if ((v % TAIL_LPP) == lig) po[(long)(slot0 + n0 + k) * 3 * CO + v] = s[k][v];
+        }
+    }
+  }
+  {
+    const int np = rows * W;
+    const bf16* base = cat + (((long)b * H + y0) * W) * Cc;
+    for (int n0 = grp * PX; n0 < np; n0 += NG * PX) {
+      const bf16* xp[PX];
+#pragma unroll
+      for (int k = 0; k < PX; ++k) xp[k] = n0 + k < np ? base + (long)(n0 + k) * Cc : nullptr;
+      float s[PX][CO];
+      tail_dots<CO, 1, PX>(xp, Cc, wpl, 1, lig, s);
+#pragma unroll
+      for (int k = 0; k < PX; ++k)
+        if (n0 + k < np) {
+#pragma unroll
+          for (int v = 0; v < CO; ++v)
+            if ((v % TAIL_LPP) == lig) qt[(long)(n0 + k) * CO + v] = s[k][v];
+        }
+    }
+  }
+  __syncthreads();
+  const float go = *gain_out;
+  const float sg = sigma[b * sstride];
+  const float den = sg * sg + sd * sd;
+  const float cskip = sd * sd / den, cout = sg * sd * rsqrtf(den);
+  for (int i = threadIdx.x; i < CO * rows * W; i += blockDim.x) {
+    const int o = i / (rows * W), n = i - o * rows * W;
+    const int ry = n / W, x = n - ry * W;
+    float s = 0.f;
+#pragma unroll
+    for (int ky = 0; ky < 3; ++ky) {
+      const int iy = y0 + ry + ky - 1;
+      if (iy < 0 || iy >= H) continue;
+#pragma unroll
+      for (int kx = 0; kx < 3; ++kx) {
+        const int ix = x + kx - 1;
+        if (ix < 0 || ix >= W) continue;
+        s += pt[((long)ky * RW + ry * W + ix) * 3 * CO + kx * CO + o];
+      }
+    }
+    const float f = sb * s + sa * qt[(long)n * CO + o];
+    const long idx = (((long)b * CO + o) * H + y0 + ry) * W + x;
+    if (Fraw) Fraw[idx] = f;
+    D[idx] = f * go * cout + noisy[idx] * cskip;
+  }
+}
+
+template <int CO>
+static int launch_tail_fwd(const void* a2, const void* cat, const float* Wc, const float* Wp, float sb, float sa,
+                           const float* gain_out, const float* noisy, const float* sigma, int sstride, float sd, float* D,
+                           float* Fraw, int B, int H, int W, int C, int Cc, hipStream_t st) {
+  constexpr int PX = CO <= 4 ? 2 : 1;
+  int R = 128 / W;
+  R = R < 1 ? 1 : (R > H ? H : R);
+  auto lds = [&](int r) { return tail_fwd_lds(CO, C, Cc, W, r); };
+  while (R > 1 && lds(R) > LOWRANK_LDS_MAX) --R;
+  EDM_REQUIRE(lds(R) <= LOWRANK_LDS_MAX, "lowrank_tail_fwd: Co=%d, C=%d, Cc=%d, W=%d need %zu bytes of LDS (60 KB at most)", CO,
+              C, Cc, W, lds(R));
+  const long want = ((long)(R + 1) * W + PX - 1) / PX * TAIL_LPP;
+  int block = want >= 512 ? 512 : (int)((want + 63) / 64 * 64);
+  const dim3 grid((H + R - 1) / R, B);
+  hipLaunchKernelGGL((k_lowrank_tail_fwd<CO, PX>), grid, dim3(block), lds(R), st, (const bf16*)a2, (const bf16*)cat, Wc, Wp, sb,
+                     sa, gain_out, noisy, sigma, sstride, sd, D, Fraw, H, W, C, Cc, R);
+  EDM_CHECK_LAUNCH("lowrank_tail_fwd");
+  return EDM_OK;
+}
+
+extern "C" int edm_lowrank_tail_fwd(const void* a2, const void* cat, const float* Wc, const float* Wp, float sb, float sa,
+                                    const float* gain_out, const float* noisy, const float* sigma, int sigma_stride,
+                                    float sigma_data, float* D, float* Fraw, int B, int H, int W, int C, int Cc, int Co,
+                                    hipStream_t st) {
+  EDM_REQUIRE(a2 && cat && Wc && Wp && gain_out && noisy && sigma && D, "lowrank_tail_fwd: null pointer");
+  EDM_REQUIRE(B > 0 && B <= 65535 && H > 0 && W > 0 && (sigma_stride == 0 || sigma_stride == 1), "lowrank_tail_fwd: bad args");
+  EDM_REQUIRE(edm_lowrank_tail_supported(C, Cc, Co, W), "lowrank_tail_fwd: unsupported shape C=%d Cc=%d Co=%d W=%d", C, Cc, Co, W);
+  EDM_REQUIRE((((uintptr_t)Wc | (uintptr_t)Wp | (uintptr_t)a2 | (uintptr_t)cat) & 15) == 0,
+              "lowrank_tail_fwd: operands must be 16-byte aligned");
+#define CALL(CO_) launch_tail_fwd<CO_>(a2, cat, Wc, Wp, sb, sa, gain_out, noisy, sigma, sigma_stride, sigma_data, D, Fraw, B, \
+                                       H, W, C, Cc, st)
+  EDM_CO_SWITCH(Co, CALL)
+#undef CALL
+}
+
+__global__ __launch_bounds__(256) void k_lowrank_tail_dwout(const float* __restrict__ G, const bf16* __restrict__ wf2,
+                                                            const float* __restrict__ G1, const bf16* __restrict__ wf1,
+                                                            float sb, float sa, float* __restrict__ gwh, int Co, int C,
+                                                            int Cc) {
+  const int lane = threadIdx.x & 63;
+  const int c = blockIdx.x * (blockDim.x >> 6) + (threadIdx.x >> 6);
+  if (c >= C) return;
+  float a9[8] = {0, 0, 0, 0, 0, 0, 0, 0}, a1[8] = {0, 0, 0, 0, 0, 0, 0, 0};
+  for (int t = 0; t < 9; ++t)
+    for (int ci = lane * 8; ci < C; ci += 64 * 8) {
+      float v[8];
+      load8(wf2 + ((long)t * C + c) * C + ci, v);
+#pragma unroll
+      for (int o = 0; o < 8; ++o)
+        if (o < Co) {
+          const float* gp = G + ((long)o * 9 + t) * C + ci;
+#pragma unroll
+          for (int j = 0; j < 8; ++j) a9[o] += v[j] * gp[j];
+        }
+    }
+  if (wf1)
+    for (int cj = lane * 8; cj < Cc; cj += 64 * 8) {
+      float v[8];
+      load8(wf1 + (long)c * Cc + cj, v);
+#pragma unroll
+      for (int o = 0; o < 8; ++o)
+        if (o < Co) {
+          const float* gp = G1 + (long)o * Cc + cj;
+#pragma unroll
+          for (int j = 0; j < 8; ++j) a1[o] += v[j] * gp[j];
+        }
+    }
+#pragma unroll
+  for (int o = 0; o < 8; ++o)
+    if (o < Co) {
+      const float s9 = wave_sum(a9[o]);
+      const float s1 = wf1 ? wave_sum(a1[o]) : G1[(long)o * Cc + c];
+      if (lane == 0) gwh[(long)o * C + c] = sb * s9 + sa * s1;
+    }
+}
+extern "C" int edm_lowrank_tail_dwout_supported(int C, int Cc, int Co, int has1) {
+  return C > 0 && C % 8 == 0 && Cc > 0 && Cc % 8 == 0 && Co >= 1 && Co <= 8 && (has1 || Cc == C);
+}
+extern "C" int edm_lowrank_tail_dwout(const float* G, const void* wf2, const float* G1, const void* wf1, float sb, float sa,
+                                      float* gwh, int Co, int C, int Cc, hipStream_t st) {
+  EDM_REQUIRE(G && wf2 && G1 && gwh, "lowrank_tail_dwout: null pointer");
+  EDM_REQUIRE(edm_lowrank_tail_dwout_supported(C, Cc, Co, wf1 != nullptr), "lowrank_tail_dwout: bad args (C=%d Cc=%d Co=%d)", C, Cc,
+              Co);
+  EDM_REQUIRE((((uintptr_t)wf2 | (uintptr_t)wf1) & 15) == 0, "lowrank_tail_dwout: packs must be 16-byte aligned");
+  hipLaunchKernelGGL(k_lowrank_tail_dwout, dim3((C + 3) / 4), dim3(256), 0, st, G, (const bf16*)wf2, G1, (const bf16*)wf1, sb,
+                     sa, gwh, Co, C, Cc);
+  EDM_CHECK_LAUNCH("lowrank_tail_dwout");
+  return EDM_OK;
+}
+
+__global__ void k_lowrank_gcat_add(const float* __restrict__ dF, const float* __restrict__ Wp, float sa,
+                                   const bf16* __restrict__ t, bf16* __restrict__ gu, bf16* __restrict__ gcs, int HW, int Cc,
+                                   int Ci, int Co, long n8) {
+  const unsigned CL = (unsigned)Cc >> 3, uHW = (unsigned)HW, CiL = (unsigned)Ci >> 3;
+  for (unsigned i = blockIdx.x * blockDim.x + threadIdx.x; i < (unsigned)n8; i += gridDim.x * blockDim.x) {
+    const unsigned p = i / CL, c8 = i - p * CL;
+    const unsigned b = p / uHW, hw = p - b * uHW;
+    float v[8] = {0, 0, 0, 0, 0, 0, 0, 0}, tv[8];
+    load8(t + (long)i * 8, tv);
+    for (int o = 0; o < Co; ++o) {
+      const float df = dF[((long)b * Co + o) * HW + hw];
+      const float* wp = Wp + (long)o * Cc + c8 * 8;
+#pragma unroll
+      for (int j = 0; j < 8; ++j) v[j] += df * wp[j];
+    }
+#pragma unroll
+    for (int j = 0; j < 8; ++j) v[j] = tv[j] + sa * v[j];
+    if (c8 < CiL) store8(gu + ((long)p * Ci + c8 * 8), v);
+    else store8(gcs + ((long)p * (Cc - Ci) + (c8 - CiL) * 8), v);
+  }
+}
+extern "C" int edm_lowrank_gcat_supported(int Cc, int Ci, int Co) {
+  return Cc > 0 && Cc % 8 == 0 && Ci > 0 && Ci % 8 == 0 && Ci <= Cc && Co >= 1 && Co <= 8;
+}
+extern "C" int edm_lowrank_gcat_add(const float* dF, const float* Wp, float sa, const void* t, void* gu, void* gcs, int B,
+                                    int HW, int Cc, int Ci, int Co, hipStream_t st) {
+  EDM_REQUIRE(dF && Wp && t && gu, "lowrank_gcat_add: null pointer");
+  EDM_REQUIRE(B > 0 && HW > 0 && edm_lowrank_gcat_supported(Cc, Ci, Co) && (gcs || Ci == Cc),
+              "lowrank_gcat_add: bad args (Cc=%d Ci=%d Co=%d)", Cc, Ci, Co);
+  const long n8 = (long)B * HW * (Cc / 8);
+  EDM_REQUIRE(n8 < (1L << 31), "lowrank_gcat_add: too many elements");
+  const long blocks = (n8 + 255) / 256;
+  hipLaunchKernelGGL(k_lowrank_gcat_add, dim3((unsigned)(blocks < 8192 ? blocks : 8192)), dim3(256), 0, st, dF, Wp, sa,
+                     (const bf16*)t, (bf16*)gu, (bf16*)gcs, HW, Cc, Ci, Co, n8);
+  EDM_CHECK_LAUNCH("lowrank_gcat_add");
+  return EDM_OK;
+}
diff --git a/tinyedm_amd/networks.py b/tinyedm_amd/networks.py
--- a/tinyedm_amd/networks.py
+++ b/tinyedm_amd/networks.py
@@ -125,6 +125,8 @@
 _w3_pending = {}
 TAIL_LOWRANK = os.environ.get("EDM_TAIL_LOWRANK", "1") != "0"
 _tail_slot = {}
+TAIL_FWD = os.environ.get("EDM_TAIL_FWD", "1") != "0"
+_tail_fwd_slot = {}
 _fin_pending = {}
 
 
@@ -196,6 +198,7 @@
 def _backward_end(key):
     _bwd_end_queued.discard(key)
     _tail_slot.pop(key, None)
+    _tail_fwd_slot.pop(key, None)
     if key in _w3_seen:
         _w3_total[key] = _w3_seen.pop(key)
     _flush_sg(key)
@@ -218,6 +221,7 @@
 
 def reset_backward_state():
     _tail_slot.clear()
+    _tail_fwd_slot.clear()
     if _bwd_end_queued or _w3_pending or _fin_pending or _w1_pending or _sg_pending:
         _bwd_end_queued.clear()
         for items in _sg_pending.values():
@@ -279,12 +283,28 @@
     return mod.finish_grad(ops.conv_wgrad(x, dy, taps), scale=scale)
 
 
-def _wgrad_lowrank(mod, x, dF, wout_hat, scale):
+def _wgrad_lowrank(mod, x, dF, wout_hat, scale, G=None):
     w = mod.weight
     box = []
-    _run_on_side(w.device, lambda: box.append(ops.lowrank_expand_slab(wout_hat, ops.lowrank_wgrad(dF, x, 9)[0], scale)),
-                 (x, dF, wout_hat))
+    if G is not None:
+        _run_on_side(w.device, lambda: box.append(ops.lowrank_expand_slab(wout_hat, G, scale)), (G, wout_hat))
+    else:
+        _run_on_side(w.device, lambda: box.append(ops.lowrank_expand_slab(wout_hat, ops.lowrank_wgrad(dF, x, 9)[0], scale)),
+                     (x, dF, wout_hat))
     return mod.finish_grad(box[0])
+
+
+def _tail_fwd_shapes_ok(u, wf2, wd2, has1, Co, Ci) -> bool:
+    if not (u.dim() == 4 and u.dtype == bf16 and u.is_contiguous() and wf2.dim() == 3 and wd2.dim() == 3):
+        return False
+    if getattr(wf2, "_edm_frag", False) or getattr(wd2, "_edm_frag", False):
+        return False
+    C, Cc, W = wf2.shape[2], u.shape[-1], u.shape[2]
+    if wf2.shape[1] != C or (not has1 and Cc != C) or not 1 <= Co <= ops.LOWRANK_MAX_CO:
+        return False
+    return (ops.lowrank_tail_supported(C, Cc, Co, W) and ops.lowrank_supported(C, Co, W, 9)
+            and ops.lowrank_supported(Cc, Co, W, 1) and ops.lowrank_tail_dwout_supported(C, Cc, Co, has1)
+            and ops.lowrank_gcat_supported(Cc, Ci, Co))
 
 
 PREP_TILE_BYTES = int(os.environ.get("EDM_PREP_TILE_KB", "96")) * 1024
@@ -811,7 +831,7 @@
 
     @staticmethod
     def forward(ctx, u, emb, w1x1, w1, w2, wemb, gain, blk, lin_view, glin_view, token, s_pre=None, alias=False,
-                gm_view=None, skip=None, w_sl1=None, w_sl2=None, pre=None, dest=None, pool=False, gate_pre=None):
+                gm_view=None, skip=None, w_sl1=None, w_sl2=None, pre=None, dest=None, pool=False, gate_pre=None, tail=0):
         enc = blk.is_encoder
         ctx.set_materialize_grads(False)
         has1 = w1x1 is not None
@@ -820,7 +840,8 @@
         wf2, wd2, _ = blk.conv_3x3_2.packs()
         batched = lin_view is not None
         weh = None if batched else blk.embed.packs()[2]
-        wd11 = None
+        wf11 = wd11 = None
+        tail_fwd = False
         ctx.has_skip = skip is not None
         if skip is not None:
             sl = blk.cat_factor
@@ -854,6 +875,9 @@
             fold = False
             if has1:
                 wf11, wd11, _ = blk.conv_1x1.packs()
+            tail_fwd = bool(tail) and _tail_fwd_shapes_ok(u, wf2, wd2, has1, int(tail),
+                                                          ctx.Ci if skip is not None else u.shape[-1])
+            if has1 and not tail_fwd:
                 fold = u.is_contiguous() and ops.conv3x3_fold_supported((*u.shape[:3], wf1.shape[1]), wf2.shape[1], u.shape[-1])
                 if not fold:
                     xres = ops.conv_igemm(u, wf11, 1)
@@ -870,7 +894,10 @@
             a2 = ops.mod_silu_drop_fwd(r1, lin, gain, pdrop, seed, sub, step, dyn=rng.dyn)
         a, b = _mp_coeffs(blk.add_factor)
         Co = wf2.shape[1]
-        if (not enc) and fold:
+        if tail_fwd:
+            _tail_fwd_slot[a2.device.index] = (a2, u, wf2, wd2, wf11, wd11, a, b)
+            out = torch.empty(*a2.shape[:3], 0, device=a2.device, dtype=bf16)
+        elif (not enc) and fold:
             if _dest_ok(dest, a2):
                 out = ops.conv3x3_fold(a2, wf2, u, wf11, b, a, out=_col_block(dest[0], Co), silu_out=_col_block(dest[1], Co))
                 out._edm_cat = dest
@@ -883,6 +910,7 @@
         else:
             out = ops.conv_igemm(a2, wf2, taps, residual=xres, alpha=b, beta=a)
         ctx.blk, ctx.enc, ctx.has1 = blk, enc, has1
+        ctx.tail_fwd = tail_fwd
         ctx.drop = (pdrop, seed, sub, step, rng.dyn)
         ctx.u_marked = U_MARKS and ops.FUSE_MOD and ops.IGEMM_VERSION == 0
         ctx.batched, ctx.glin_view, ctx.gm_view = batched, glin_view, gm_view
@@ -906,8 +934,14 @@
         ggain_out = gp.grad if gdirect else None
         deferred = False
         fused = ops.FUSE_MOD and ops.IGEMM_VERSION == 0 and (gout.shape[1] * gout.shape[2]) % 32 == 0
-        tail = None
-        if blk._tail_last:
+        tail = tfwd = None
+        if ctx.tail_fwd:
+            slot = _tail_slot.pop(gout.device.index, None)
+            if slot is None or len(slot) != 7 or r1 is None:
+                raise RuntimeError("tinyedm_amd: the last block's backward ran without the output end's (TAIL_FWD: its "
+                                   "output is a handle that only _TailOutFn consumes)")
+            tail, tfwd = slot[:2], slot[3:]
+        elif blk._tail_last:
             slot = _tail_slot.pop(gout.device.index, None)
             w2 = blk.conv_3x3_2.weight
             if (slot is not None and slot[2].data_ptr() == gout.data_ptr() and slot[2].shape == gout.shape
@@ -917,7 +951,8 @@
                 tail = slot[:2]
         if tail is not None:
             deferred = ctx.gm_view is not None and gdirect and (fused or MOD_DEFER_UNFUSED)
-            gr1, glin, ggain = ops.lowrank_dgrad3x3_modbwd(tail[0], ops.lowrank_expand_wc(tail[1], wd2), b, r1, lin, gain, pdrop,
+            Wc = tfwd[3] if tfwd is not None else ops.lowrank_expand_wc(tail[1], wd2)
+            gr1, glin, ggain = ops.lowrank_dgrad3x3_modbwd(tail[0], Wc, b, r1, lin, gain, pdrop,
                                                              seed, sub, step, glin_out=glin_out, ggain_out=ggain_out, dyn=dyn,
                                                              gm_out=ctx.gm_view if deferred else None, u_marked=ctx.u_marked)
             if deferred:
@@ -941,7 +976,9 @@
             if not deferred:
                 for hook in getattr(gp, "_edm_hooks", ()):
                     hook(gp)
-        if tail is not None:
+        if tfwd is not None:
+            gw2 = _wgrad_lowrank(blk.conv_3x3_2, a2, tail[0], tail[1], b, G=tfwd[0])
+        elif tail is not None:
             gw2 = _wgrad_lowrank(blk.conv_3x3_2, a2, tail[0], tail[1], b)
         else:
             gw2 = _wgrad(blk.conv_3x3_2, a2, gout, 9, b)
@@ -968,7 +1005,12 @@
                 gu = gx
             g_alias = None
         else:
-            if has1:
+            if tfwd is not None:
+                t = ops.conv3x3_silubwd(gr1, wd1, u) if fuse else ops.silu_bwd(u, gs)
+                gu, gcs = ops.lowrank_gcat_add(tail[0], tfwd[2], a, t, ctx.Ci if ctx.has_skip else None)
+                if has1:
+                    gw11 = _wgrad_lowrank(blk.conv_1x1, None, None, tail[1], a, G=tfwd[1])
+            elif has1:
                 t = ops.conv3x3_silubwd(gr1, wd1, u) if fuse else ops.silu_bwd(u, gs)
                 if ctx.has_skip:
                     Ci = ctx.Ci
@@ -1018,7 +1060,7 @@
         if g_alias is not None:
             gu = ops.axpby(gu, 1.0, g_alias, 1.0)
         return (gu, gemb, gw11, gw1, gw2, gwemb, ggain, None, None, None, gtoken, None, None, None, gskip, gwsl1, gwsl2,
-                None, None, None, None)
+                None, None, None, None, None)
 
 
 _rng_sub_counter = [0]
@@ -1039,15 +1081,15 @@
         self.rng_sub = _rng_sub_counter[0]
 
     def _res(self, u: Tensor, embedding: Tensor, lin=None, s_pre=None, alias=False, skip=None, dest=None, pool=False,
-             gate=None):
+             gate=None, tail=0):
         w11 = self.conv_1x1.weight if isinstance(self.conv_1x1, Conv2d) else None
         has_attn = isinstance(self.attention, CosineAttention)
         sk = ()
-        if skip is not None or dest is not None or pool:
+        if skip is not None or dest is not None or pool or tail:
             cf = self.cat_factor if skip is not None else None
             sk = (skip, cf.layer1.weight if cf is not None else None, cf.layer2.weight if cf is not None else None,
                   getattr(u, "_edm_cat", None) if skip is not None else None, None if has_attn else dest, bool(pool),
-                  gate if skip is not None else None)
+                  gate if skip is not None else None, 0 if has_attn else int(tail))
         if lin is None:
             out = _ResBlockFn.apply(u, embedding, w11, self.conv_3x3_1.weight, self.conv_3x3_2.weight,
                                     self.embed.weight, self.gain, self, None, None, None, s_pre, alias, None, *sk)
@@ -1209,15 +1251,18 @@
         return (FUSE_CAT and SKIP_GATE_FUSED and not isinstance(self.resample, UpSample)
                 and isinstance(self.conv_1x1, Conv2d) and self.cat_factor is not None)
 
-    def forward(self, input: Tensor, embedding: Tensor, skip: Tensor | None = None, _lin=None, _dest=None, _gate=None) -> Tensor:
+    def forward(self, input: Tensor, embedding: Tensor, skip: Tensor | None = None, _lin=None, _dest=None, _gate=None,
+                _tail=0) -> Tensor:
         x, conv = _as_nhwc(input)
+        if conv:
+            _tail = 0
         s_pre = None
         if skip is not None and FUSE_CAT and SKIP_GATE_FUSED and not isinstance(self.resample, UpSample) \
                 and isinstance(self.conv_1x1, Conv2d):
             assert self.cat_factor is not None
             sk, _ = _as_nhwc(skip)
             out = self._res(x, None if _lin is not None else _emb32(embedding, x.shape[0]), _lin, skip=sk, dest=_dest,
-                            gate=_gate)
+                            gate=_gate, tail=_tail)
             return ops.nhwc_bf16_to_nchw(out).to(input.dtype) if conv else _tag(out)
         if skip is not None:
             assert self.cat_factor is not None
@@ -1237,7 +1282,7 @@
             else:
                 x = _ResampleFn.apply(x, True)
                 s_pre = None
-        out = self._res(x, None if _lin is not None else _emb32(embedding, x.shape[0]), _lin, s_pre, dest=_dest)
+        out = self._res(x, None if _lin is not None else _emb32(embedding, x.shape[0]), _lin, s_pre, dest=_dest, tail=_tail)
         return ops.nhwc_bf16_to_nchw(out).to(input.dtype) if conv else _tag(out)
 
     @staticmethod
@@ -1429,6 +1474,52 @@
                 hook(gp)
         gw = ctx.den.conv_out.finish_grad(gwh.view(1, 1, *gwh.shape))
         return gx, gw, gg, None, None, None
+
+
+class _TailOutFn(torch.autograd.Function):
+
+    @staticmethod
+    def forward(ctx, handle, w, gain_out, noisy, sigma, den: "Denoiser", pack):
+        a2, cat, wf2, wd2, wf11, wd11, a, b = pack
+        wh = den.conv_out.packs()[2]
+        Wc = ops.lowrank_expand_wc(wh, wd2)
+        Wp = ops.lowrank_expand_wc(wh, wd11).view(wh.shape[0], -1) if wd11 is not None else wh
+        D, Fraw = ops.lowrank_tail_fwd(a2, cat, Wc, Wp, b, a, gain_out, noisy, sigma, den.sigma_data,
+                                       want_fraw=any(ctx.needs_input_grad))
+        ctx.den, ctx.ab, ctx.hshape = den, (a, b), tuple(handle.shape)
+        ctx.save_for_backward(a2, cat, wh, gain_out, Fraw, sigma, Wc, Wp, wf2, wf11)
+        return D
+
+    @staticmethod
+    def backward(ctx, gD):
+        a2, cat, wh, gain_out, Fraw, sigma, Wc, Wp, wf2, wf11 = ctx.saved_tensors
+        a, b = ctx.ab
+        den = ctx.den
+        gp = den.gain_out
+        gdirect = gp.grad is not None and getattr(gp, "_edm_direct", False) and gp.grad.is_contiguous()
+        w = den.conv_out.weight
+        dD = gD.contiguous().float()
+        dF, aux = ops.lowrank_df(dD, Fraw, gain_out, sigma, den.sigma_data)
+        G1, gg = ops.lowrank_wgrad(dF, cat, 1, aux=aux, aux_out=gp.grad if gdirect else None)
+        if gdirect:
+            gg = None
+            for hook in getattr(gp, "_edm_hooks", ()):
+                hook(gp)
+        box = []
+
+        def reduce_and_contract():
+            G = ops.lowrank_wgrad(dF, a2, 9)[0]
+            box.extend((G, ops.lowrank_tail_dwout(G, wf2, G1, wf11, b, a)))
+        if w.grad is not None and getattr(w, "_edm_direct", False):
+            _run_on_side(w.device, reduce_and_contract, (dF, a2, G1))
+        else:
+            reduce_and_contract()
+        G, gwh = box
+        gx = torch.empty(ctx.hshape, device=dD.device, dtype=bf16)
+        _tail_slot[dD.device.index] = (dF, wh, gx, G, G1, Wp, Wc)
+        _queue_backward_end(dD.device)
+        gw = den.conv_out.finish_grad(gwh.view(1, 1, *gwh.shape))
+        return gx, gw, gg, None, None, None, None
 
 
 class Denoiser(nn.Module):
@@ -1496,6 +1587,29 @@
     def _res_blocks(self):
         return list(self.encoder_blocks) + list(self.decoder_blocks)
 
+    def _conv_out_of(self, x: Tensor, noisy: Tensor, sig: Tensor) -> Tensor:
+        pack = _tail_fwd_slot.pop(x.device.index, None)
+        if pack is not None:
+            return _TailOutFn.apply(x, self.conv_out.weight, self.gain_out, noisy, sig, self, pack)
+        return _ConvOutFn.apply(x, self.conv_out.weight, self.gain_out, noisy, sig, self)
+
+    def _tail_fwd_co(self) -> int:
+        if not (TAIL_FWD and TAIL_LOWRANK) or not len(self.decoder_blocks):
+            return 0
+        blk = self.decoder_blocks[-1]
+        if not (isinstance(blk, DecoderBlock) and blk._tail_last) or isinstance(blk.attention, CosineAttention):
+            return 0
+        for m in (blk, self.conv_out):
+            if m._forward_hooks or m._forward_pre_hooks or m._backward_hooks or m._backward_pre_hooks:
+                return 0
+        if torch.is_grad_enabled():
+            ws = [blk.conv_3x3_2.weight, self.conv_out.weight]
+            if isinstance(blk.conv_1x1, Conv2d):
+                ws.append(blk.conv_1x1.weight)
+            if not all(w.grad is not None and getattr(w, "_edm_direct", False) for w in ws):
+                return 0
+        return int(self.conv_out.weight.shape[0])
+
     def _modfin_table(self, blocks):
         gains = [b.gain for b in blocks]
         if not all(g.grad is not None and getattr(g, "_edm_direct", False) and g.grad.is_contiguous() for g in gains):
@@ -1708,6 +1822,7 @@
         skips.append(x)
         dests = _decoder_dests_impl(dec, skips, x) if FUSE_CAT and SKIP_GATE_FUSED else {}
         gates = self._decoder_gates(dec, skips, dests) if SG_MULTI else {}
+        tail_co = self._tail_fwd_co()
         for i, (block, has_skip) in enumerate(dec):
             skip = skips.pop() if has_skip else None
             dest = dests.get(i)
@@ -1719,8 +1834,9 @@
             cat_pre = getattr(x, "_edm_cat", None)
             if cat_pre is not None:
                 xin._edm_cat = cat_pre
-            x = block(xin, None, _tag(skip) if has_skip else None, _lin=lins[block], _dest=dest, _gate=gates.get(block))
-        D = _ConvOutFn.apply(x, self.conv_out.weight, self.gain_out, noisy, sig, self)
+            last = {"_tail": tail_co} if (tail_co and i + 1 == len(dec)) else {}
+            x = block(xin, None, _tag(skip) if has_skip else None, _lin=lins[block], _dest=dest, _gate=gates.get(block), **last)
+        D = self._conv_out_of(x, noisy, sig)
         if self.training:
             rng.step += 1
         return D.to(noisy_image.dtype)
diff --git a/tinyedm_amd/ops.py b/tinyedm_amd/ops.py
--- a/tinyedm_amd/ops.py
+++ b/tinyedm_amd/ops.py
@@ -847,6 +847,68 @@
     slab = torch.empty(1, taps, O, Ipad, device=G.device, dtype=f32)
     _lib.call("edm_lowrank_expand_slab", _p(wout_hat), _p(G), _p(slab), float(scale), Co, O, I, Ipad, taps, _stream())
     return slab
+
+
+@functools.lru_cache(maxsize=None)
+def lowrank_tail_supported(C, Cc, Co, W):
+    return bool(_lib.lib().edm_lowrank_tail_supported(int(C), int(Cc), int(Co), int(W)))
+
+
+def lowrank_tail_fwd(a2, cat, Wc, Wp, sb, sa, gain_out, noisy, sigma, sigma_data, want_fraw=True):
+    B, H, W, C = _nhwc(a2, "a2")
+    Cc = cat.shape[-1]
+    _chk(cat, bf16, "cat", (B, H, W, Cc))
+    Co = Wc.shape[0]
+    _chk(Wc, f32, "Wc", (Co, 9, C))
+    _chk(Wp, f32, "Wp", (Co, Cc))
+    _chk(noisy, f32, "noisy", (B, Co, H, W))
+    _chk(gain_out, f32, "gain_out")
+    ss = _sigma_arg(sigma, B)
+    D = torch.empty(B, Co, H, W, device=a2.device, dtype=f32)
+    Fraw = torch.empty(B, Co, H, W, device=a2.device, dtype=f32) if want_fraw else None
+    _lib.call("edm_lowrank_tail_fwd", _p(a2), _p(cat), _p(Wc), _p(Wp), float(sb), float(sa), _p(gain_out), _p(noisy),
+              _p(sigma), ss, float(sigma_data), _p(D), _p(Fraw), B, H, W, C, Cc, Co, _stream())
+    return D, Fraw
+
+
+def lowrank_tail_dwout_supported(C, Cc, Co, has1):
+    return bool(_lib.lib().edm_lowrank_tail_dwout_supported(int(C), int(Cc), int(Co), int(bool(has1))))
+
+
+def lowrank_tail_dwout(G, wf2, G1, wf1, sb, sa):
+    _chk(G, f32, "G")
+    Co, _, C = G.shape
+    _chk(G, f32, "G", (Co, 9, C))
+    if wf2.dim() != 3 or getattr(wf2, "_edm_frag", False):
+        raise ValueError("lowrank_tail_dwout: expected a plain (9, O, I) forward pack")
+    _chk(wf2, bf16, "wf2", (9, C, C))
+    Cc = G1.shape[-1]
+    _chk(G1, f32, "G1", (Co, 1, Cc))
+    if wf1 is not None:
+        _chk(wf1, bf16, "wf1", (1, C, Cc))
+    elif Cc != C:
+        raise ValueError("lowrank_tail_dwout: without a 1x1 pack G1 must have the block's channel count")
+    gwh = torch.empty(Co, C, device=G.device, dtype=f32)
+    _lib.call("edm_lowrank_tail_dwout", _p(G), _p(wf2), _p(G1), _p(wf1), float(sb), float(sa), _p(gwh), Co, C, Cc, _stream())
+    return gwh
+
+
+def lowrank_gcat_supported(Cc, Ci, Co):
+    return bool(_lib.lib().edm_lowrank_gcat_supported(int(Cc), int(Ci), int(Co)))
+
+
+def lowrank_gcat_add(dF, Wp, sa, t, Ci=None):
+    B, H, W, Cc = _nhwc(t, "t")
+    _chk(dF, f32, "dF")
+    Co = dF.shape[1]
+    _chk(dF, f32, "dF", (B, Co, H, W))
+    _chk(Wp, f32, "Wp", (Co, Cc))
+    split = Ci is not None and Ci != Cc
+    Ci = Cc if not split else int(Ci)
+    gu = torch.empty(B, H, W, Ci, device=t.device, dtype=bf16)
+    gcs = torch.empty(B, H, W, Cc - Ci, device=t.device, dtype=bf16) if split else None
+    _lib.call("edm_lowrank_gcat_add", _p(dF), _p(Wp), float(sa), _p(t), _p(gu), _p(gcs), B, H * W, Cc, Ci, Co, _stream())
+    return gu, gcs
 
 
 def nchw_to_nhwc_bf16(x):
```

After: 10460 img/s, median of 6. 1.6% higher.
